# neeharperi/FutureDet

Hardware: AMD Instinct MI355X
Metric: sweeps/sec end-to-end (300k pts, 10-sweep voxel) (higher is better)
Workload: dtype f32

## Files before the change

futuredet_amd/backbones.py:

```python
import numpy as np
import torch
from torch import nn

from . import hip_ops, sparse as spconv
from .nn_utils import build_norm_layer
from .registry import BACKBONES
from .sparse import SparseConv3d, SubMConv3d


def conv3x3(in_planes, out_planes, stride=1, indice_key=None, bias=True):
    return spconv.SubMConv3d(in_planes, out_planes, kernel_size=3, stride=stride, padding=1, bias=bias,
                             indice_key=indice_key)


class SparseBasicBlock(spconv.SparseModule):
    expansion = 1

    def __init__(self, inplanes, planes, stride=1, norm_cfg=None, downsample=None, indice_key=None):
        super().__init__()
        if norm_cfg is None:
            norm_cfg = dict(type="BN1d", eps=1e-3, momentum=0.01)
        bias = norm_cfg is not None
        self.conv1 = conv3x3(inplanes, planes, stride, indice_key=indice_key, bias=bias)
        self.bn1 = build_norm_layer(norm_cfg, planes)[1]
        self.relu = nn.ReLU()
        self.conv2 = conv3x3(planes, planes, indice_key=indice_key, bias=bias)
        self.bn2 = build_norm_layer(norm_cfg, planes)[1]
        self.downsample = downsample
        self.stride = stride

    def forward(self, x):
        identity = x
        out = self.conv1(x)
        out.features = self.relu(self.bn1(out.features))
        out = self.conv2(out)
        out.features = self.bn2(out.features)
        if self.downsample is not None:
            identity = self.downsample(x)
        out.features = self.relu(out.features + identity.features)
        return out

    def forward_fused_bn(self, x, bn_act):
        out = self.conv1(x)
        out.features = bn_act(out.features, self.bn1, self.relu)
        out = self.conv2(out)
        identity = x if self.downsample is None else self.downsample(x)
        out.features = bn_act(out.features, self.bn2, self.relu, identity.features)
        return out


@BACKBONES.register_module
class SpMiddleResNetFHD(nn.Module):
    def __init__(self, num_input_features=128, norm_cfg=None, name="SpMiddleResNetFHD", **kwargs):
        super().__init__()
        self.name = name
        if norm_cfg is None:
            norm_cfg = dict(type="BN1d", eps=1e-3, momentum=0.01)
        S = spconv.SparseSequential
        self.conv_input = S(SubMConv3d(num_input_features, 16, 3, bias=False, indice_key="res0"),
                            build_norm_layer(norm_cfg, 16)[1], nn.ReLU(inplace=True))
        self.conv1 = S(SparseBasicBlock(16, 16, norm_cfg=norm_cfg, indice_key="res0"),
                       SparseBasicBlock(16, 16, norm_cfg=norm_cfg, indice_key="res0"))
        self.conv2 = S(SparseConv3d(16, 32, 3, 2, padding=1, bias=False), build_norm_layer(norm_cfg, 32)[1],
                       nn.ReLU(inplace=True), SparseBasicBlock(32, 32, norm_cfg=norm_cfg, indice_key="res1"),
                       SparseBasicBlock(32, 32, norm_cfg=norm_cfg, indice_key="res1"))
        self.conv3 = S(SparseConv3d(32, 64, 3, 2, padding=1, bias=False), build_norm_layer(norm_cfg, 64)[1],
                       nn.ReLU(inplace=True), SparseBasicBlock(64, 64, norm_cfg=norm_cfg, indice_key="res2"),
                       SparseBasicBlock(64, 64, norm_cfg=norm_cfg, indice_key="res2"))
        self.conv4 = S(SparseConv3d(64, 128, 3, 2, padding=[0, 1, 1], bias=False), build_norm_layer(norm_cfg, 128)[1],
                       nn.ReLU(inplace=True), SparseBasicBlock(128, 128, norm_cfg=norm_cfg, indice_key="res3"),
                       SparseBasicBlock(128, 128, norm_cfg=norm_cfg, indice_key="res3"))
        self.extra_conv = S(SparseConv3d(128, 128, (3, 1, 1), (2, 1, 1), bias=False), build_norm_layer(norm_cfg, 128)[1],
                            nn.ReLU())
        self.compute_dtype = torch.float32
        self.dense_channels_last = True
        self.dense_dtype = None
        self.profile_hook = None
        self.fused_bn = False
        self.train_dtype = torch.float32

    def _bn_act(self, features, bn, relu, residual=None):
        if self.fused_bn and spconv.batch_norm_fusable(features, bn):
            return spconv.batch_norm_act(features, bn, residual=residual, relu=True)
        if features.dtype == torch.bfloat16:
            out = bn(features.float())
            if residual is not None:
                out = out + residual.float()
            return spconv.relu_to_bf16(out)
        out = bn(features)
        if residual is not None:
            out = out + residual
        return relu(out)

    def _run_stage(self, seq, x):
        mods = list(seq._modules.values())
        i = 0
        while i < len(mods):
            m = mods[i]
            if isinstance(m, SparseBasicBlock):
                x = m.forward_fused_bn(x, self._bn_act)
            elif isinstance(m, spconv.SparseModule):
                x = m(x)
            elif x.features.shape[0] != 0:
                if isinstance(m, nn.BatchNorm1d) and i + 1 < len(mods) and isinstance(mods[i + 1], nn.ReLU):
                    x.features = self._bn_act(x.features, m, mods[i + 1])
                    i += 1
                else:
                    x.features = m(x.features)
            i += 1
        return x

    def forward_generic(self, voxel_features, coors, batch_size, input_shape):
        sparse_shape = np.array(input_shape[::-1]) + [1, 0, 0]
        ret = spconv.SparseConvTensor(voxel_features, coors.int(), sparse_shape, batch_size)
        stages = (self.conv_input, self.conv1, self.conv2, self.conv3, self.conv4, self.extra_conv)
        mixed = self.train_dtype == torch.bfloat16 and self.training and torch.is_grad_enabled()
        if mixed:
            ret.features = ret.features.to(torch.bfloat16)
        if mixed or (self.fused_bn and self.training and torch.is_grad_enabled()):
            run = [lambda x, seq=seq: self._run_stage(seq, x) for seq in stages]
        else:
            run = stages
        x = run[0](ret)
        x_conv1 = run[1](x)
        x_conv2 = run[2](x_conv1)
        x_conv3 = run[3](x_conv2)
        x_conv4 = run[4](x_conv3)
        ret = run[5](x_conv4).dense()
        if mixed:
            ret = ret.float()
        N, C, D, H, W = ret.shape
        ret = ret.view(N, C * D, H, W)
        return ret, {"conv1": x_conv1, "conv2": x_conv2, "conv3": x_conv3, "conv4": x_conv4}

    def _stages(self):
        return [(self.conv_input[0], self.conv_input[1], [self.conv1[0], self.conv1[1]], True),
                (self.conv2[0], self.conv2[1], [self.conv2[3], self.conv2[4]], False),
                (self.conv3[0], self.conv3[1], [self.conv3[3], self.conv3[4]], False),
                (self.conv4[0], self.conv4[1], [self.conv4[3], self.conv4[4]], False),
                (self.extra_conv[0], self.extra_conv[1], [], False)]

    def build_indexes(self, mark_fn, batch_size, input_shape, device, voxels=None, static=False, expected=None, row_caps=None):
        D, H, W = [int(v) for v in (np.array(input_shape[::-1]) + [1, 0, 0])]
        if voxels is not None:
            geoms = [self._stages()[lvl][0].geometry() for lvl in range(1, 5)]
            return hip_ops.build_pyramid(voxels[0], voxels[1], voxels[2], batch_size, (D, H, W), geoms, device, static=static,
                                         expected=expected, row_caps=row_caps)
        assert not static, "static indexes are built from the voxelizer's device output (voxels=...)"
        counts = torch.zeros((5,), dtype=torch.int32, device=device)
        idx = [hip_ops.SparseIndex(batch_size, D, H, W, device)]
        mark_fn(idx[0])
        idx[0].scan(counts[0:1])
        for lvl in range(1, 5):
            conv = self._stages()[lvl][0]
            ks, st, pd = conv.geometry()
            nxt = idx[-1].downsample(ks, st, pd)
            nxt.scan(counts[lvl:lvl + 1])
            idx.append(nxt)
        host = counts.cpu()
        for i, ix in enumerate(idx):
            ix.finalize(int(host[i]))
        return idx

    def run_fused(self, idx, feats0, dense_out=None, fork=False):
        dt = self.compute_dtype
        stages = self._stages()
        rb_cache = {}

        def rulebook(src, dst, conv):
            ks, st, pd = conv.geometry()
            key = (id(src), id(dst), tuple(ks), tuple(st), tuple(pd))
            if key not in rb_cache:
                rb_cache[key] = src.rulebook(dst, ks, st, pd)
            return rb_cache[key]

        def run(conv, bn, x, src, dst, relu, residual=None):
            wpk, bias, cin_p, cout_p = conv.packed_weight(dt, bn)
            assert x.shape[1] == cin_p, (x.shape, cin_p)
            nbr = rulebook(src, dst, conv)
            fn = lambda: hip_ops.spconv_apply(x, wpk, bias, nbr, dst.n, cout_p, residual=residual, relu=relu)
            if self.profile_hook is not None:
                s = 4 if dt == torch.float32 else 2
                K = nbr.shape[0]
                pairs = lambda: int((nbr[:, : dst.n] >= 0).sum().item())
                return self.profile_hook("spconv_%dx%d_K%d" % (cin_p, cout_p, K),
                                         dict(s=s, K=K, cin=cin_p, cout=cout_p, n_in=src.n, n_out=dst.n, pairs=pairs), fn)
            return fn()

        main, side = None, None
        if fork and feats0.is_cuda:
            main = torch.cuda.current_stream(feats0.device)
            pool = self.__dict__.setdefault("_side_streams", {})
            side = pool.get(main.cuda_stream)
            if side is None:
                side = pool[main.cuda_stream] = torch.cuda.Stream(device=feats0.device)
            side.wait_stream(main)
            with torch.cuda.stream(side):
                made = []
                for lvl, (conv, bn, blocks, is_subm_in) in enumerate(stages):
                    if lvl == 0:
                        continue
                    src_l, dst_l = (idx[lvl] if is_subm_in else idx[lvl - 1]), idx[lvl]
                    made.append(rulebook(src_l, dst_l, conv))
                    for blk in blocks:
                        nbr = rulebook(dst_l, dst_l, blk.conv1)
                        made.append(nbr)
                        cp = spconv.pad_channels(blk.conv1.out_channels)
                        if dt == torch.float32 and nbr.shape[0] == 27 and \
                                hip_ops._lib.load().fd_spconv_wants_balanced_ranges(cp, cp, 0):
                            r = hip_ops.ranges_for(nbr, cp, cp)
                            if r[0] is not None:
                                made.append(r[0])
                for t in made:
                    t.record_stream(main)
        x = feats0
        levels = {}
        for lvl, (conv, bn, blocks, is_subm_in) in enumerate(stages):
            src = idx[lvl] if is_subm_in else idx[lvl - 1]
            dst = idx[lvl]
            if lvl == 1 and side is not None:
                main.wait_stream(side)
            x = run(conv, bn, x, src, dst, relu=True)
            for blk in blocks:
                y = run(blk.conv1, blk.bn1, x, dst, dst, relu=True)
                x = run(blk.conv2, blk.bn2, y, dst, dst, relu=True, residual=x)
            levels[lvl] = (x, dst)
        bev = hip_ops.densify(x, idx[4], out_dtype=self.dense_dtype or dt, channels_last=self.dense_channels_last, out=dense_out)
        return bev, levels

    def forward_static_train(self, feats0, idx):
        if not self.fused_bn:
            raise ValueError("SpMiddleResNetFHD.forward_static_train needs fused_bn = True: torch's BatchNorm1d cannot take its row count "
                             "from the device (set backbone.fused_bn = True)")
        if not (self.training and torch.is_grad_enabled()):
            raise RuntimeError("SpMiddleResNetFHD.forward_static_train is the training path: call .train() and enable gradients")
        if self.train_dtype not in (torch.float32, torch.bfloat16):
            raise ValueError("SpMiddleResNetFHD: train_dtype must be torch.float32 or torch.bfloat16 (got %s)" % (self.train_dtype,))
        B = idx[0].B
        feats = feats0.to(self.train_dtype)
        rulebooks = {}

        def conv(m, x, src, dst):
            ks, st, pd = m.geometry()
            key = (id(src), id(dst), tuple(ks), tuple(st), tuple(pd))
            if key not in rulebooks:
                rulebooks[key] = src.rulebook(dst, ks, st, pd)
            return m._forward_autograd(x, dst, rulebooks[key])

        def bn_act(x, bn, dst, residual=None):
            if dst.n < 2 or not spconv.batch_norm_fusable(x.features, bn):
                raise hip_ops.FutureDetHipError("forward_static_train: BatchNorm over %s %s rows cannot run on the fused kernels"
                                                % (tuple(x.features.shape), x.features.dtype))
            x.features = spconv.batch_norm_act(x.features, bn, residual=residual, relu=True, n_dev=dst.n_dev if dst.static else None)
            return x

        x = spconv.SparseConvTensor(feats, None, idx[0].spatial_shape, B, _index=idx[0])
        for lvl, (head, bn, blocks, is_subm_in) in enumerate(self._stages()):
            src, dst = (idx[lvl] if is_subm_in else idx[lvl - 1]), idx[lvl]
            x = bn_act(conv(head, x, src, dst), bn, dst)
            for blk in blocks:
                y = bn_act(conv(blk.conv1, x, dst, dst), blk.bn1, dst)
                x = bn_act(conv(blk.conv2, y, dst, dst), blk.bn2, dst, residual=x.features)
        ret = x.dense()
        if ret.dtype != torch.float32:
            ret = ret.float()
        N, C, D, H, W = ret.shape
        return ret.view(N, C * D, H, W)

    def forward(self, voxel_features, coors, batch_size, input_shape):
        if self.training:
            if self.train_dtype not in (torch.float32, torch.bfloat16):
                raise ValueError("SpMiddleResNetFHD: train_dtype must be torch.float32 or torch.bfloat16 (got %s)" % (self.train_dtype,))
            if self.train_dtype == torch.float32 and self.compute_dtype != torch.float32 and torch.is_grad_enabled():
                raise NotImplementedError("SpMiddleResNetFHD: with train_dtype = torch.float32 training runs the fp32 sparse convolution only; "
                                          "compute_dtype = %s selects the inference path (set train_dtype = torch.bfloat16 for mixed-precision "
                                          "training, or compute_dtype = torch.float32)" % self.compute_dtype)
            return self.forward_generic(voxel_features, coors, batch_size, input_shape)
        coors = coors.int().contiguous()
        dev = voxel_features.device
        idx = self.build_indexes(lambda i0: i0.mark(coors), batch_size, input_shape, dev)
        row_of = idx[0].lookup(coors)
        feats0 = hip_ops.rows_permute(voxel_features.float().contiguous(), row_of,
                                      spconv.pad_channels(voxel_features.shape[1]), self.compute_dtype, n_rows=idx[0].n)
        bev, levels = self.run_fused(idx, feats0)
        multi = {}
        for name, lvl, c in (("conv1", 0, 16), ("conv2", 1, 32), ("conv3", 2, 64), ("conv4", 3, 128)):
            f, ix = levels[lvl]
            multi[name] = spconv.SparseConvTensor(f[:, :c], None, ix.spatial_shape, batch_size, _index=ix)
        return bev, multi


@BACKBONES.register_module
class PointPillarsScatter(nn.Module):

    def __init__(self, num_input_features=64, norm_cfg=None, name="PointPillarsScatter", **kwargs):
        super().__init__()
        self.name = "PointPillarsScatter"
        self.nchannels = num_input_features
        self.dense_channels_last = True

    def forward(self, voxel_features, coords, batch_size, input_shape, n_dev=None):
        self.nx = int(input_shape[0])
        self.ny = int(input_shape[1])
        coords = coords.int().contiguous()
        if n_dev is None and torch.is_grad_enabled() and voxel_features.requires_grad:
            return _ScatterFn.apply(voxel_features, coords, batch_size, self.ny, self.nx, self.dense_channels_last)
        return hip_ops.pillar_scatter(voxel_features, coords, n_dev, batch_size, self.ny, self.nx,
                                      channels_last=self.dense_channels_last)


    def forward_static(self, voxel_features, coords, counts, batch_size, input_shape):
        self.nx = int(input_shape[0])
        self.ny = int(input_shape[1])
        return _ScatterSegFn.apply(voxel_features, coords.int().contiguous(), counts, batch_size, self.ny, self.nx, self.dense_channels_last)


class _ScatterSegFn(torch.autograd.Function):

    @staticmethod
    def forward(ctx, feats, coords, counts, batch_size, ny, nx, channels_last):
        B = counts.shape[0]
        cap = feats.shape[0] // B
        ctx.coords, ctx.counts, ctx.cap = coords, counts, cap
        canvas = None
        for b in range(B):
            sl = slice(b * cap, (b + 1) * cap)
            canvas = hip_ops.pillar_scatter(feats[sl], coords[sl], counts[b:b + 1], batch_size, ny, nx, channels_last=channels_last,
                                            out=canvas, zero_first=(b == 0))
        return canvas

    @staticmethod
    def backward(ctx, dcanvas):
        coords, counts, cap = ctx.coords, ctx.counts, ctx.cap
        dcanvas = dcanvas.float()
        d = torch.cat([hip_ops.pillar_scatter_backward(dcanvas, coords[b * cap:(b + 1) * cap], n_dev=counts[b:b + 1])
                       for b in range(counts.shape[0])])
        ctx.coords = ctx.counts = None
        return d, None, None, None, None, None, None


class _ScatterFn(torch.autograd.Function):

    @staticmethod
    def forward(ctx, feats, coords, batch_size, ny, nx, channels_last):
        ctx.coords = coords
        return hip_ops.pillar_scatter(feats, coords, None, batch_size, ny, nx, channels_last=channels_last)

    @staticmethod
    def backward(ctx, dcanvas):
        d = hip_ops.pillar_scatter_backward(dcanvas.float(), ctx.coords)
        ctx.coords = None
        return d, None, None, None, None, None
```

futuredet_amd/csrc/fd_common.h:

```cpp
#pragma once
#include <hip/hip_runtime.h>
#include <stdint.h>
#include <stdio.h>

#include <atomic>

#include "../../include/futuredet_hip.h"

namespace fd {

void set_error(const char *fmt, ...);

struct SpconvCall {
    const void *in;
    int64_t n_in;
    const void *wpacked;
    const float *bias;
    const void *residual;
    int relu;
    const int *nbr;
    int64_t nbr_stride;
    const int *ranges;
    int n_ranges;
    int K, n_out;
    const int *n_out_dev;
    int64_t n_expected;
    int cin, cout, dtype;
    void *out;
    hipStream_t stream;
};

constexpr int kSpconvMaxTaps = 27;

struct WeightSection {
    size_t offset, bytes;
};
struct SpconvWeightLayout {
    WeightSection base, c32, pair, win;
    size_t total;
};
inline SpconvWeightLayout spconv_weight_layout(int K, int cin, int cout, int dtype) {
    const size_t elem = dtype == 0 ? 4 : 2, main_bytes = (size_t)K * cin * cout * elem;
    SpconvWeightLayout l{};
    size_t end = 0;
    auto section = [&](bool present, size_t bytes) {
        const WeightSection s{end, present ? bytes : 0};
        end += s.bytes;
        return s;
    };
    l.base = section(true, main_bytes);
    l.c32 = section(dtype == 0 && cin == 32 && cout == 32, main_bytes);
    l.pair = section(dtype == 1 && cin == 16, (size_t)((K + 1) / 2) * 32 * cout * elem);
    l.win = section(dtype == 1 && ((cin == 64 && cout == 64) || (cin == 128 && cout == 128)), main_bytes);
    l.total = end;
    return l;
}
inline SpconvWeightLayout spconv_weight_layout(const SpconvCall &c) { return spconv_weight_layout(c.K, c.cin, c.cout, c.dtype); }

int spconv_f32_res16_dispatch(const SpconvCall &c);
int spconv_f32_c32_dispatch(const SpconvCall &c);
int spconv_f32_compact_dispatch(const SpconvCall &c);
int spconv_bf16_win_dispatch(const SpconvCall &c);
int spconv_bf16_ws_dispatch(const SpconvCall &c);

int wino_pc_launch(const float *x, const void *wp, const float *bias, float *y, int B, int H, int W, int cin, int cout, int relu, int cout_total,
                   int co_off, int wide_items, hipStream_t stream);

__device__ __forceinline__ int device_count(int capacity, const int *count_dev) {
    if (!count_dev) return capacity;
    const int n = *count_dev;
    return n < capacity ? (n > 0 ? n : 0) : capacity;
}

inline int check_launch(const char *what) {
    hipError_t e = hipGetLastError();
    if (e != hipSuccess) {
        set_error("%s: %s", what, hipGetErrorString(e));
        return FD_ELAUNCH;
    }
    return FD_OK;
}

#define FD_REQUIRE(cond, ...)           \
    do {                                \
        if (!(cond)) {                  \
            fd::set_error(__VA_ARGS__); \
            return FD_EINVAL;           \
        }                               \
    } while (0)

inline hipStream_t as_stream(fd_stream_t s) { return reinterpret_cast<hipStream_t>(s); }

int fill_words(void *p, uint32_t value, size_t n_words, hipStream_t stream);
int fill_words3(void *p0, uint32_t v0, size_t n0, void *p1, uint32_t v1, size_t n1, void *p2, uint32_t v2, size_t n2, hipStream_t stream);

constexpr int kMaxDevices = 64;
int current_device();
int device_cu_count();
bool ensure_dynamic_lds(const void *kernel, size_t bytes, std::atomic<uint64_t> &done);
#define FD_TUNE_KNOBS(X)                                                                                                       \
    X(kTuneSpconvRG, "spconv_rg") X(kTuneSpconvV1, "spconv_v1") X(kTuneConvNT, "conv_nt") X(kTuneV2RangesPerCU, "v2_ranges_per_cu") \
    X(kTuneSpconvC32, "spconv_c32") X(kTuneBf16GP, "bf16_gp") X(kTuneBf16RG, "bf16_rg") X(kTuneBf16Depth, "bf16_depth")        \
    X(kTuneBf16NW, "bf16_nw") X(kTuneBf16Win, "bf16_win") X(kTuneF32ResRG, "f32_res_rg") X(kTuneConvStrip, "conv_strip")       \
    X(kTuneF32ResNW, "f32_res_nw")
#define FD_TUNE_ENUM(key, name) key,
enum TuneKey { FD_TUNE_KNOBS(FD_TUNE_ENUM) kTuneCount };
#undef FD_TUNE_ENUM
int tuning(TuneKey key);

inline size_t align_up(size_t v, size_t a) { return (v + a - 1) / a * a; }

struct IndexGeom {
    int B, D, H, W, Ht, Wt;
    __host__ __device__ int64_t num_cols() const { return (int64_t)B * Ht * Wt * 64; }
};
__host__ __device__ inline IndexGeom make_geom(int B, int D, int H, int W) {
    IndexGeom g;
    g.B = B; g.D = D; g.H = H; g.W = W;
    g.Ht = (H + 7) >> 3; g.Wt = (W + 7) >> 3;
    return g;
}
__host__ __device__ inline int64_t col_of(const IndexGeom &g, int b, int y, int x) {
    return ((((int64_t)b * g.Ht + (y >> 3)) * g.Wt + (x >> 3)) << 6) + ((y & 7) << 3) + (x & 7);
}
__device__ inline void col_to_byx(const IndexGeom &g, int64_t col, int &b, int &y, int &x) {
    int in = (int)(col & 63);
    int64_t t = col >> 6;
    int tx = (int)(t % g.Wt);
    t /= g.Wt;
    int ty = (int)(t % g.Ht);
    b = (int)(t / g.Ht);
    y = ty * 8 + (in >> 3);
    x = tx * 8 + (in & 7);
}

__device__ inline unsigned xcd_swizzle(unsigned bid, unsigned nblocks) {
    const unsigned nx = 8;
    unsigned per = nblocks / nx, rem = nblocks % nx;
    unsigned xcd = bid % nx, loc = bid / nx;
    unsigned start = xcd * per + (xcd < rem ? xcd : rem);
    return start + loc;
}

}
```

futuredet_amd/csrc/fd_spconv.hip:

```cpp
#include "fd_spconv_pack.h"

namespace {

typedef float f32x4 __attribute__((ext_vector_type(4)));
typedef short s16x4 __attribute__((ext_vector_type(4)));
typedef __bf16 bf16x8 __attribute__((ext_vector_type(8)));

__device__ inline unsigned short f2bf(float v) {
    unsigned u = __float_as_uint(v);
    u += 0x7fffu + ((u >> 16) & 1u);
    return (unsigned short)(u >> 16);
}
__device__ inline float bf2f(unsigned short h) { return __uint_as_float(((unsigned)h) << 16); }


template <int CIN, int COUT, int RG>
__global__ void __launch_bounds__(256) spconv_f32(const float *__restrict__ in, const float4 *__restrict__ wp,
                                                  const float *__restrict__ bias, const float *__restrict__ residual, int relu,
                                                  const int *__restrict__ nbr, int64_t nbr_stride, int K, int n_out,
                                                  const int *__restrict__ n_out_dev, float *__restrict__ out) {
    constexpr int ROWS_B = 64 * RG;
    constexpr int NB = COUT / 16, NC = CIN / 16;
    __shared__ int s_nbr[fd::kSpconvMaxTaps * ROWS_B];
    const int tile = blockIdx.x;
    const int row0 = tile * ROWS_B;
    n_out = fd::device_count(n_out, n_out_dev);
    if (row0 >= n_out) return;
    for (int t = threadIdx.x; t < K * ROWS_B; t += 256) {
        int k = t / ROWS_B, r = t - k * ROWS_B;
        int64_t o = (int64_t)row0 + r;
        s_nbr[t] = (o < n_out) ? nbr[(int64_t)k * nbr_stride + o] : -1;
    }
    __syncthreads();
    const int lane = threadIdx.x & 63, wave = __builtin_amdgcn_readfirstlane(threadIdx.x >> 6);
    const int lrow = lane & 15, lq = lane >> 4;
    const int wrow = wave * 16 * RG;
    if (row0 + wrow >= n_out) return;

    f32x4 acc[RG][NB];
#pragma unroll
    for (int g = 0; g < RG; ++g)
#pragma unroll
        for (int nb = 0; nb < NB; ++nb) acc[g][nb] = (f32x4){0.f, 0.f, 0.f, 0.f};

    for (int k = 0; k < K; ++k) {
        int idx[RG];
        bool any[RG];
        bool any_all = false;
#pragma unroll
        for (int g = 0; g < RG; ++g) {
            idx[g] = s_nbr[k * ROWS_B + wrow + g * 16 + lrow];
            any[g] = __ballot(idx[g] >= 0) != 0ull;
            any_all = any_all || any[g];
        }
        if (!any_all) continue;
        const float4 *wk = wp + (int64_t)k * NC * NB * 64 + lane;
#pragma unroll
        for (int c = 0; c < NC; ++c) {
            float4 a[RG];
#pragma unroll
            for (int g = 0; g < RG; ++g) {
                a[g] = make_float4(0.f, 0.f, 0.f, 0.f);
                if (idx[g] >= 0) a[g] = *reinterpret_cast<const float4 *>(in + (int64_t)idx[g] * CIN + c * 16 + lq * 4);
            }
#pragma unroll
            for (int nb = 0; nb < NB; ++nb) {
                const float4 b = wk[(c * NB + nb) * 64];
#pragma unroll
                for (int g = 0; g < RG; ++g) {
                    if (any[g]) {
                        acc[g][nb] = __builtin_amdgcn_mfma_f32_16x16x4f32(a[g].x, b.x, acc[g][nb], 0, 0, 0);
                        acc[g][nb] = __builtin_amdgcn_mfma_f32_16x16x4f32(a[g].y, b.y, acc[g][nb], 0, 0, 0);
                        acc[g][nb] = __builtin_amdgcn_mfma_f32_16x16x4f32(a[g].z, b.z, acc[g][nb], 0, 0, 0);
                        acc[g][nb] = __builtin_amdgcn_mfma_f32_16x16x4f32(a[g].w, b.w, acc[g][nb], 0, 0, 0);
                    }
                }
            }
        }
    }
#pragma unroll
    for (int g = 0; g < RG; ++g) {
#pragma unroll
        for (int nb = 0; nb < NB; ++nb) {
            const int col = nb * 16 + lrow;
            const float bv = bias ? bias[col] : 0.0f;
#pragma unroll
            for (int r = 0; r < 4; ++r) {
                const int row = row0 + wrow + g * 16 + lq * 4 + r;
                if (row < n_out) {
                    float v = acc[g][nb][r] + bv;
                    if (residual) v += residual[(int64_t)row * COUT + col];
                    if (relu) v = fmaxf(v, 0.0f);
                    out[(int64_t)row * COUT + col] = v;
                }
            }
        }
    }
}

template <int CIN, int COUT, int RG>
__global__ void __launch_bounds__(256) spconv_bf16(const unsigned short *__restrict__ in, const void *__restrict__ wp_,
                                                   const float *__restrict__ bias, const unsigned short *__restrict__ residual,
                                                   int relu, const int *__restrict__ nbr, int64_t nbr_stride, int K, int n_out,
                                                   const int *__restrict__ n_out_dev, unsigned short *__restrict__ out) {
    constexpr int ROWS_B = 64 * RG;
    constexpr int NB = COUT / 16;
    constexpr bool WIDE = CIN >= 32;
    constexpr int NC = WIDE ? CIN / 32 : 1;
    __shared__ int s_nbr[fd::kSpconvMaxTaps * ROWS_B];
    const int tile = blockIdx.x;
    const int row0 = tile * ROWS_B;
    n_out = fd::device_count(n_out, n_out_dev);
    if (row0 >= n_out) return;
    for (int t = threadIdx.x; t < K * ROWS_B; t += 256) {
        int k = t / ROWS_B, r = t - k * ROWS_B;
        int64_t o = (int64_t)row0 + r;
        s_nbr[t] = (o < n_out) ? nbr[(int64_t)k * nbr_stride + o] : -1;
    }
    __syncthreads();
    const int lane = threadIdx.x & 63, wave = __builtin_amdgcn_readfirstlane(threadIdx.x >> 6);
    const int lrow = lane & 15, lq = lane >> 4;
    const int wrow = wave * 16 * RG;
    if (row0 + wrow >= n_out) return;

    f32x4 acc[RG][NB];
#pragma unroll
    for (int g = 0; g < RG; ++g)
#pragma unroll
        for (int nb = 0; nb < NB; ++nb) acc[g][nb] = (f32x4){0.f, 0.f, 0.f, 0.f};

    for (int k = 0; k < K; ++k) {
        int idx[RG];
        bool any[RG];
        bool any_all = false;
#pragma unroll
        for (int g = 0; g < RG; ++g) {
            idx[g] = s_nbr[k * ROWS_B + wrow + g * 16 + lrow];
            any[g] = __ballot(idx[g] >= 0) != 0ull;
            any_all = any_all || any[g];
        }
        if (!any_all) continue;
        if constexpr (WIDE) {
            const bf16x8 *wk = reinterpret_cast<const bf16x8 *>(wp_) + (int64_t)k * NC * NB * 64 + lane;
#pragma unroll
            for (int c = 0; c < NC; ++c) {
                bf16x8 a[RG];
#pragma unroll
                for (int g = 0; g < RG; ++g) {
                    uint4 raw = make_uint4(0u, 0u, 0u, 0u);
                    if (idx[g] >= 0) raw = *reinterpret_cast<const uint4 *>(in + (int64_t)idx[g] * CIN + c * 32 + lq * 8);
                    a[g] = __builtin_bit_cast(bf16x8, raw);
                }
#pragma unroll
                for (int nb = 0; nb < NB; ++nb) {
                    const bf16x8 b = wk[(c * NB + nb) * 64];
#pragma unroll
                    for (int g = 0; g < RG; ++g)
                        if (any[g]) acc[g][nb] = __builtin_amdgcn_mfma_f32_16x16x32_bf16(a[g], b, acc[g][nb], 0, 0, 0);
                }
            }
        } else {
            const s16x4 *wk = reinterpret_cast<const s16x4 *>(wp_) + (int64_t)k * NB * 64 + lane;
            s16x4 a[RG];
#pragma unroll
            for (int g = 0; g < RG; ++g) {
                uint2 raw = make_uint2(0u, 0u);
                if (idx[g] >= 0) raw = *reinterpret_cast<const uint2 *>(in + (int64_t)idx[g] * CIN + lq * 4);
                a[g] = __builtin_bit_cast(s16x4, raw);
            }
#pragma unroll
            for (int nb = 0; nb < NB; ++nb) {
                const s16x4 b = wk[nb * 64];
#pragma unroll
                for (int g = 0; g < RG; ++g)
                    if (any[g]) acc[g][nb] = __builtin_amdgcn_mfma_f32_16x16x16bf16_1k(a[g], b, acc[g][nb], 0, 0, 0);
            }
        }
    }
#pragma unroll
    for (int g = 0; g < RG; ++g) {
#pragma unroll
        for (int nb = 0; nb < NB; ++nb) {
            const int col = nb * 16 + lrow;
            const float bv = bias ? bias[col] : 0.0f;
#pragma unroll
            for (int r = 0; r < 4; ++r) {
                const int row = row0 + wrow + g * 16 + lq * 4 + r;
                if (row < n_out) {
                    float v = acc[g][nb][r] + bv;
                    if (residual) v += bf2f(residual[(int64_t)row * COUT + col]);
                    if (relu) v = fmaxf(v, 0.0f);
                    out[(int64_t)row * COUT + col] = f2bf(v);
                }
            }
        }
    }
}

template <int CIN, int COUT, int RG>
void launch(const fd::SpconvCall &a) {
    const int rows_b = 64 * RG;
    dim3 grid((unsigned)((a.n_out + rows_b - 1) / rows_b));
    const void *wp = (const char *)a.wpacked + fd::spconv_weight_layout(a).base.offset;
    if (a.dtype == 0)
        hipLaunchKernelGGL((spconv_f32<CIN, COUT, RG>), grid, dim3(256), 0, a.stream, (const float *)a.in, (const float4 *)wp, a.bias,
                           (const float *)a.residual, a.relu, a.nbr, a.nbr_stride, a.K, a.n_out, a.n_out_dev, (float *)a.out);
    else
        hipLaunchKernelGGL((spconv_bf16<CIN, COUT, RG>), grid, dim3(256), 0, a.stream, (const unsigned short *)a.in, wp, a.bias,
                           (const unsigned short *)a.residual, a.relu, a.nbr, a.nbr_stride, a.K, a.n_out, a.n_out_dev, (unsigned short *)a.out);
}

template <int CIN, int COUT>
void launch_rg(const fd::SpconvCall &a, int rg) {
    if (rg >= 4) launch<CIN, COUT, 4>(a);
    else if (rg == 2) launch<CIN, COUT, 2>(a);
    else launch<CIN, COUT, 1>(a);
}

int pick_rg(int64_t n_out, int cin, int cout) {
    const int forced = fd::tuning(fd::kTuneSpconvRG);
    if (forced > 0) return forced;
    const int64_t waves2 = (n_out + 31) / 32;
    int rg = (cin * cout >= 128 * 128) ? 1 : 2;
    if (rg == 2 && waves2 < 256 * 4 * 2) rg = 1;
    return rg;
}

}

extern "C" size_t fd_spconv_packed_weight_bytes(int K, int cin, int cout, int dtype) {
    if (K <= 0 || cin <= 0 || cout <= 0) return 0;
    return fd::spconv_weight_layout(K, cin, cout, dtype).total;
}

extern "C" int fd_spconv_pack_weight(const float *w, int K, int cin, int cout, int dtype, void *dst) {
    if (const int rc = fd::spconv_pack_check("fd_spconv_pack_weight", w, dst, K, cin, cout, dtype, 0)) return rc;
    fd::spconv_pack_weight_host(w, K, cin, cout, dtype, dst);
    return FD_OK;
}

extern "C" int fd_spconv_apply(const void *in_feats, int64_t n_in, const void *wpacked, const float *bias, const void *residual, int relu,
                               const int32_t *nbr, int64_t nbr_stride, const int32_t *ranges, int n_ranges, int K, int64_t n_out,
                               const int32_t *n_out_dev, int64_t n_expected, int cin, int cout, int dtype, void *out_feats, fd_stream_t stream) {
    FD_REQUIRE(K >= 1 && K <= fd::kSpconvMaxTaps, "fd_spconv_apply: K must be in [1,27]");
    FD_REQUIRE(dtype == 0 || dtype == 1, "fd_spconv_apply: dtype must be 0 (f32) or 1 (bf16)");
    FD_REQUIRE(n_out >= 0 && n_out <= nbr_stride && n_out < (1ll << 31), "fd_spconv_apply: n_out out of range");
    FD_REQUIRE(n_ranges >= 0 && (ranges == nullptr || n_ranges >= 1), "fd_spconv_apply: ranges needs n_ranges >= 1");
    if (n_expected <= 0 || n_expected > n_out) n_expected = n_out;
    if (n_out == 0) return FD_OK;
    FD_REQUIRE(in_feats && wpacked && nbr && out_feats, "fd_spconv_apply: null argument");
    const fd::SpconvCall c{in_feats, n_in, wpacked, bias, residual, relu, nbr, nbr_stride, ranges, n_ranges, K, (int)n_out, n_out_dev, n_expected,
                           cin, cout, dtype, out_feats, fd::as_stream(stream)};
    if (dtype == 0 && !fd::tuning(fd::kTuneSpconvV1) && cin == 16 && fd::tuning(fd::kTuneF32ResRG) >= 0) {
        if (fd::spconv_f32_res16_dispatch(c)) return fd::check_launch("fd_spconv_apply(f32 resident)");
    }
    if (dtype == 0 && !fd::tuning(fd::kTuneSpconvV1) && fd::tuning(fd::kTuneSpconvC32) >= 0) {
        if (fd::spconv_f32_c32_dispatch(c)) return fd::check_launch("fd_spconv_apply(c32)");
    }
    if (dtype == 0 && !fd::tuning(fd::kTuneSpconvV1)) {
        if (fd::spconv_f32_compact_dispatch(c)) return fd::check_launch("fd_spconv_apply(compact)");
    }
    if (dtype == 1 && fd::tuning(fd::kTuneBf16GP) >= 0) {
        const bool subm_like = K == 27 && n_in == n_out;
        if (fd::tuning(fd::kTuneBf16Win) >= 0 && subm_like && fd::spconv_bf16_win_dispatch(c)) return fd::check_launch("fd_spconv_apply(bf16 window)");
        if (fd::spconv_bf16_ws_dispatch(c)) return fd::check_launch("fd_spconv_apply(bf16 ws)");
    }
    const int rg = pick_rg(n_expected, cin, cout);
    const int key = cin * 1000 + cout;
    switch (key) {
        case 16016: launch_rg<16, 16>(c, rg); break;
        case 16032: launch_rg<16, 32>(c, rg); break;
        case 32032: launch_rg<32, 32>(c, rg); break;
        case 32064: launch_rg<32, 64>(c, rg); break;
        case 64064: launch_rg<64, 64>(c, rg); break;
        case 64128: launch_rg<64, 128>(c, rg); break;
        case 128128: launch_rg<128, 128>(c, rg); break;
        default:
            fd::set_error("fd_spconv_apply: unsupported channels %d -> %d", cin, cout);
            return FD_EINVAL;
    }
    return fd::check_launch("fd_spconv_apply");
}
```

futuredet_amd/csrc/fd_spconv_c32.hip:

```cpp
#include "fd_spconv_chunk.h"

namespace {

namespace sk = fd::skeleton;
typedef float f32x16 __attribute__((ext_vector_type(16)));
typedef unsigned u32x4 __attribute__((ext_vector_type(4)));
constexpr int TM = 128, COUT = 32, TS = 4, WR = 1;
constexpr sk::Layout L = sk::layout(TM, COUT, TS, 32);
static_assert(((sk::kMaxTaps + TS - 1) / TS) * (TM / WR / 32) <= L.item_slot, "item list slot");

template <int CIN, int DEPTH>
__global__ void __launch_bounds__(256) spconv_f32_c32(const float *__restrict__ in, const float4 *__restrict__ wp, const float *__restrict__ bias,
                                                      const float *__restrict__ residual, int relu, const int *__restrict__ nbr, int64_t nbr_stride,
                                                      int K, int n_out, const int *__restrict__ n_out_dev, float *__restrict__ out, unsigned in_bytes,
                                                      const int *__restrict__ ranges, int rows_per_range) {
    constexpr int NCH = CIN / 8;
    constexpr int kPad = sk::pad_entry(TM);
    extern __shared__ __attribute__((aligned(16))) unsigned char smem[];
    int *s_list = reinterpret_cast<int *>(smem + L.list);
    unsigned short *s_items = reinterpret_cast<unsigned short *>(smem + L.items);
    unsigned char *s_cnt = smem + L.cnt;
    int *s_pad = reinterpret_cast<int *>(smem + L.pad);
    float *s_acc = reinterpret_cast<float *>(smem + L.acc);

    const int tid = threadIdx.x, lane = tid & 63, wave = __builtin_amdgcn_readfirstlane(tid >> 6);
    int r_begin, r_end, n_chunks, chunk_rows;
    sk::resolve_range(n_out, n_out_dev, ranges, rows_per_range, r_begin, r_end);
    if (r_begin >= r_end) return;
    sk::cut_chunks<TM>(r_begin, r_end, n_chunks, chunk_rows);
    int pre[sk::kSliceRegs<TM>];
    sk::fetch_slice<TM>(pre, nbr, nbr_stride, K, r_begin);

    const int ln = lane & 31, lh = lane >> 5;
    const int ts = wave, wr = 0;
    unsigned char *acc_bytes = reinterpret_cast<unsigned char *>(s_acc + ts * L.acc_copy);
    const __amdgpu_buffer_rsrc_t rsrc = __builtin_amdgcn_make_buffer_rsrc(const_cast<float *>(in), 0, (int)in_bytes, 0x00020000);
    unsigned short *items = s_items + wave * L.item_slot;

    for (int chunk = 0; chunk < n_chunks; ++chunk) {
        int row0, n_rows;
        if (!sk::chunk_span(r_begin, r_end, chunk_rows, chunk, row0, n_rows)) break;
        sk::stage_chunk<TM, COUT, TS, 32>(pre, s_list, s_pad, s_acc, bias, residual, K, row0, n_rows);
        __syncthreads();
        sk::compact_taps<TM, WR>(s_list, s_cnt, K);
        __syncthreads();
        if (chunk + 1 < n_chunks) sk::fetch_slice<TM>(pre, nbr, nbr_stride, K, row0 + chunk_rows);
        const int n_items = sk::build_items<TS, 32>(s_cnt, items, K, ts, wr);

        int k_r[DEPTH], row_r[DEPTH];
        u32x4 a_r[DEPTH][NCH];
        auto stage_a0 = [&](int it) -> int { return sk::stage_a0(items, n_items, it); };
        auto stage_a1 = [&](int it, int code_v, int &kk, int &e) { sk::stage_a1<TM, WR, 32>(s_list, s_pad, n_items, wr, ln, it, code_v, kk, e); };
        auto gather_offset = [&](int e) -> unsigned { return sk::entry_row_bytes<CIN>(e) + (unsigned)(lh * 16); };
        auto gather_step = [&](unsigned voff, int c) { return __builtin_amdgcn_raw_buffer_load_b128(rsrc, voff + c * 32, 0, 0); };
        float4 b[NCH];
        auto load_b = [&](int k) {
            const float4 *wk = wp + (int64_t)k * NCH * 64 + lane;
#pragma unroll
            for (int c = 0; c < NCH; ++c) b[c] = wk[c * 64];
        };
        int k_s, e_s, code_s;
#pragma unroll
        for (int d = 0; d < DEPTH - 1; ++d) {
            stage_a1(d, stage_a0(d), k_s, e_s);
            const unsigned vo = gather_offset(e_s);
#pragma unroll
            for (int c = 0; c < NCH; ++c) a_r[d][c] = gather_step(vo, c);
            k_r[d] = k_s;
            row_r[d] = e_s;
        }
        k_r[DEPTH - 1] = -1;
        row_r[DEPTH - 1] = kPad;
        stage_a1(DEPTH - 1, stage_a0(DEPTH - 1), k_s, e_s);
        code_s = stage_a0(DEPTH);
        if (n_items > 0) load_b(k_r[0]);

        for (int i0 = 0; i0 < n_items; i0 += DEPTH) {
#pragma unroll
            for (int d = 0; d < DEPTH; ++d) {
                const unsigned arow = sk::entry_local_row(row_r[d]);
                unsigned aoff[4];
#pragma unroll
                for (int q = 0; q < 4; ++q) aoff[q] = sk::acc_slot_bytes<COUT>(arow, (unsigned)(2 * q + lh));
                f32x16 acc;
#pragma unroll
                for (int q = 0; q < 4; ++q) {
                    const float4 v = *reinterpret_cast<const float4 *>(acc_bytes + aoff[q]);
                    acc[4 * q + 0] = v.x; acc[4 * q + 1] = v.y; acc[4 * q + 2] = v.z; acc[4 * q + 3] = v.w;
                }
                const int dn = (d + DEPTH - 1) % DEPTH;
                {
                    const int it = i0 + d + DEPTH - 1;
                    const unsigned vo = gather_offset(e_s);
                    k_r[dn] = k_s;
                    row_r[dn] = e_s;
#pragma unroll
                    for (int c = 0; c < NCH; ++c) a_r[dn][c] = gather_step(vo, c);
                    stage_a1(it + 1, code_s, k_s, e_s);
                    code_s = stage_a0(it + 2);
                }
                const int knext = k_r[(d + 1) % DEPTH];
                const bool reload = knext >= 0 && knext != k_r[d];
                __builtin_amdgcn_sched_barrier(0);
#pragma unroll
                for (int c = 0; c < NCH; ++c) {
                    const float4 av = __builtin_bit_cast(float4, a_r[d][c]);
                    acc = __builtin_amdgcn_mfma_f32_32x32x2f32(b[c].x, av.x, acc, 0, 0, 0);
                    acc = __builtin_amdgcn_mfma_f32_32x32x2f32(b[c].y, av.y, acc, 0, 0, 0);
                    acc = __builtin_amdgcn_mfma_f32_32x32x2f32(b[c].z, av.z, acc, 0, 0, 0);
                    acc = __builtin_amdgcn_mfma_f32_32x32x2f32(b[c].w, av.w, acc, 0, 0, 0);
                    if (reload) b[c] = (wp + (int64_t)knext * NCH * 64 + lane)[c * 64];
                }
#pragma unroll
                for (int q = 0; q < 4; ++q)
                    *reinterpret_cast<float4 *>(acc_bytes + aoff[q]) = make_float4(acc[4 * q + 0], acc[4 * q + 1], acc[4 * q + 2], acc[4 * q + 3]);
                __builtin_amdgcn_sched_barrier(0);
            }
        }
        __syncthreads();
        sk::epilogue<TM, COUT, TS>(s_acc, bias, residual, relu, out, row0, n_rows);
        __syncthreads();
    }
}

template <int CIN, int DEPTH>
int launch_c32(const fd::SpconvCall &c) {
    const unsigned in_bytes = (unsigned)(c.n_in * CIN * 4);
    int n_ranges = c.n_ranges, rows_per = 0;
    if (!c.ranges) sk::equal_rows_split(c.n_out, TM, c.n_out_dev != nullptr, n_ranges, rows_per);
    static std::atomic<uint64_t> lds_set{0};
    if (!fd::ensure_dynamic_lds(reinterpret_cast<const void *>(spconv_f32_c32<CIN, DEPTH>), (size_t)L.bytes, lds_set)) return 0;
    const void *wp = (const char *)c.wpacked + fd::spconv_weight_layout(c).c32.offset;
    hipLaunchKernelGGL((spconv_f32_c32<CIN, DEPTH>), dim3((unsigned)n_ranges), dim3(256), (size_t)L.bytes, c.stream, (const float *)c.in, (const float4 *)wp,
                       c.bias, (const float *)c.residual, c.relu, c.nbr, c.nbr_stride, c.K, c.n_out, c.n_out_dev, (float *)c.out, in_bytes, c.ranges, rows_per);
    return 1;
}

}

namespace fd {
int spconv_f32_c32_dispatch(const SpconvCall &c) {
    if (c.cout != 32 || c.cin != 32) return 0;
    if (!sk::entries_fit(c.n_in, c.cin)) return 0;
    return launch_c32<32, 3>(c);
}
}
```

futuredet_amd/csrc/fd_spconv_chunk.h:

```cpp
#pragma once
#include "fd_common.h"

namespace fd {
namespace skeleton {

constexpr int kMaxTaps = 27;

constexpr int pad_entry(int tm) { return (int)(0xffffff00u | (unsigned)tm); }
__device__ __forceinline__ int pack_entry(int in_row, int local_row) { return (in_row << 8) | local_row; }
__device__ __forceinline__ unsigned entry_local_row(int e) { return (unsigned)e & 255u; }
template <int CIN>
__device__ __forceinline__ unsigned entry_row_bytes(int e) {
    static_assert(CIN == 16 || CIN == 32 || CIN == 64 || CIN == 128, "shift per CIN");
    const unsigned hi = (unsigned)e & 0xffffff00u;
    return CIN >= 64 ? hi << (CIN == 128 ? 1 : 0) : hi >> (CIN == 32 ? 1 : 2);
}
inline bool entries_fit(int64_t n_in_bound, int cin) { return n_in_bound < (1ll << 23) && n_in_bound * cin * 4 < (1ll << 31); }

struct Layout {
    int list;
    int items;
    int item_slot;
    int cnt;
    int pad;
    int acc;
    int acc_copy;
    int bytes;
};
constexpr int acc_copy_floats(int tm, int cout) { return (tm + 1) * cout; }
constexpr Layout layout(int tm, int cout, int ts, int item) {
    Layout l{};
    l.list = 0;
    l.items = l.list + (int)sizeof(int) * kMaxTaps * tm;
    l.item_slot = item == 16 ? kMaxTaps * (tm / 16) : 32;
    l.cnt = l.items + (int)sizeof(unsigned short) * 4 * l.item_slot;
    l.pad = l.cnt + 112;
    l.acc = l.pad + (int)sizeof(int) * item;
    l.acc_copy = acc_copy_floats(tm, cout);
    l.bytes = l.acc + (int)sizeof(float) * ts * l.acc_copy;
    return l;
}

template <int COUT>
__device__ __forceinline__ unsigned acc_swizzle(unsigned row) {
    static_assert(COUT == 16 || COUT == 32 || COUT == 64 || COUT == 128, "whole bank rows");
    constexpr int kSwzShift = COUT >= 64 ? 0 : COUT == 32 ? 1 : 2;
    constexpr unsigned kSwzMask = COUT >= 64 ? 15u : COUT == 32 ? 7u : 3u;
    return (row >> kSwzShift) & kSwzMask;
}
template <int COUT>
__device__ __forceinline__ int acc_slot(int row, int col) {
    return row * (COUT / 4) + (col ^ (int)acc_swizzle<COUT>((unsigned)row));
}
template <int COUT>
__device__ __forceinline__ unsigned acc_slot_bytes(unsigned row, unsigned col) {
    return row * (COUT * 4) + ((col ^ acc_swizzle<COUT>(row)) << 4);
}

__device__ __forceinline__ void resolve_range(int n_out, const int *n_out_dev, const int *ranges, int rows_per_range,
                                              int &r_begin, int &r_end) {
    if (n_out_dev) n_out = fd::device_count(n_out, n_out_dev);
    if (ranges) {
        r_begin = ranges[blockIdx.x];
        r_end = ranges[blockIdx.x + 1];
    } else {
        if (n_out_dev) rows_per_range = (((n_out + (int)gridDim.x - 1) / (int)gridDim.x) + 15) & ~15;
        const int64_t b = (int64_t)blockIdx.x * rows_per_range;
        r_begin = (int)(b < n_out ? b : n_out);
        r_end = (int)(b + rows_per_range < n_out ? b + rows_per_range : n_out);
    }
    if (r_end > n_out) r_end = n_out;
}
template <int TM>
__device__ __forceinline__ void cut_chunks(int r_begin, int r_end, int &n_chunks, int &chunk_rows) {
    n_chunks = (r_end - r_begin + TM - 1) / TM;
    chunk_rows = (((r_end - r_begin + n_chunks - 1) / n_chunks) + 15) & ~15;
}
__device__ __forceinline__ bool chunk_span(int r_begin, int r_end, int chunk_rows, int chunk, int &row0, int &n_rows) {
    row0 = r_begin + chunk * chunk_rows;
    n_rows = (r_end - row0) < chunk_rows ? (r_end - row0) : chunk_rows;
    return n_rows > 0;
}
inline void equal_rows_split(int n_out, int tm, bool device_count, int &n_ranges, int &rows_per) {
    if (n_ranges <= 0) n_ranges = (n_out + tm - 1) / tm;
    rows_per = (((n_out + n_ranges - 1) / n_ranges) + 15) & ~15;
    if (!device_count) n_ranges = (n_out + rows_per - 1) / rows_per;
}

template <int TM>
constexpr int kSliceRegs = (kMaxTaps * TM + 255) / 256;

template <int TM>
__device__ __forceinline__ void fetch_slice(int (&pre)[kSliceRegs<TM>], const int *nbr, int64_t nbr_stride, int K, int row0) {
    const int tid = threadIdx.x;
#pragma unroll
    for (int i = 0; i < kSliceRegs<TM>; ++i) {
        const int t = tid + i * 256;
        int k = t / TM;
        const int r = t - k * TM;
        k = k < K ? k : K - 1;
        int64_t o = (int64_t)row0 + r;
        o = o < nbr_stride ? o : nbr_stride - 1;
        pre[i] = nbr[(int64_t)k * nbr_stride + o];
    }
}

template <int COUT>
constexpr bool kInitAcc = COUT <= 64;

template <int TM, int COUT, int TS>
__device__ __forceinline__ void init_acc(float *s_acc, const float *bias, const float *residual, int row0, int n_rows) {
    const int tid = threadIdx.x;
    if constexpr (kInitAcc<COUT>) {
        constexpr int C4i = COUT / 4, NINIT = TM * C4i / 256;
        static_assert(TM * C4i % 256 == 0, "whole passes");
        float4 iv[NINIT];
#pragma unroll
        for (int i = 0; i < NINIT; ++i) {
            const int t = tid + i * 256, c4 = t % C4i;
            iv[i] = bias ? reinterpret_cast<const float4 *>(bias)[c4] : make_float4(0.f, 0.f, 0.f, 0.f);
        }
        if (residual) {
            float4 rv[NINIT];
#pragma unroll
            for (int i = 0; i < NINIT; ++i) {
                const int t = tid + i * 256, r = t / C4i, c4 = t - r * C4i;
                const int rr = r < n_rows ? r : n_rows - 1;
                rv[i] = reinterpret_cast<const float4 *>(residual + (int64_t)(row0 + rr) * COUT)[c4];
            }
#pragma unroll
            for (int i = 0; i < NINIT; ++i) { iv[i].x += rv[i].x; iv[i].y += rv[i].y; iv[i].z += rv[i].z; iv[i].w += rv[i].w; }
        }
#pragma unroll
        for (int i = 0; i < NINIT; ++i) {
            const int t = tid + i * 256, r = t / C4i, c4 = t - r * C4i;
            reinterpret_cast<float4 *>(s_acc)[acc_slot<COUT>(r, c4)] = r < n_rows ? iv[i] : make_float4(0.f, 0.f, 0.f, 0.f);
        }
        for (int t = TM * C4i + tid; t < TS * acc_copy_floats(TM, COUT) / 4; t += 256) reinterpret_cast<float4 *>(s_acc)[t] = make_float4(0.f, 0.f, 0.f, 0.f);
    } else {
        for (int t = tid; t < TS * acc_copy_floats(TM, COUT) / 4; t += 256) reinterpret_cast<float4 *>(s_acc)[t] = make_float4(0.f, 0.f, 0.f, 0.f);
    }
}

template <int TM, int COUT, int TS, int ITEM>
__device__ __forceinline__ void stage_chunk(const int (&pre)[kSliceRegs<TM>], int *s_list, int *s_pad, float *s_acc, const float *bias,
                                            const float *residual, int K, int row0, int n_rows) {
    const int tid = threadIdx.x;
    static_assert(256 % TM == 0, "a thread stages the same local row in every pass");
    const bool in_chunk = tid % TM < n_rows;
#pragma unroll
    for (int i = 0; i < kSliceRegs<TM>; ++i) {
        const int t = tid + i * 256;
        if (t < K * TM) s_list[t] = in_chunk ? pre[i] : -1;
    }
    init_acc<TM, COUT, TS>(s_acc, bias, residual, row0, n_rows);
    if (tid < ITEM) s_pad[tid] = pad_entry(TM);
}

template <int TM, int WR>
__device__ __forceinline__ void compact_taps(int *s_list, unsigned char *s_cnt, int K) {
    const int lane = threadIdx.x & 63, wave = __builtin_amdgcn_readfirstlane(threadIdx.x >> 6);
    constexpr int RW = TM / WR, NH = (RW + 63) / 64;
    for (int k = wave; k < K; k += 4) {
#pragma unroll
        for (int wr = 0; wr < WR; ++wr) {
            const int base = k * TM + wr * RW;
            int count = 0;
            int v[NH];
#pragma unroll
            for (int h = 0; h < NH; ++h) {
                const int r = h * 64 + lane;
                v[h] = (r < RW) ? s_list[base + r] : -1;
            }
#pragma unroll
            for (int h = 0; h < NH; ++h) {
                const int r = h * 64 + lane;
                if (r < RW) s_list[base + r] = pad_entry(TM);
            }
#pragma unroll
            for (int h = 0; h < NH; ++h) {
                const int r = h * 64 + lane;
                const unsigned long long m = __ballot(v[h] >= 0);
                const int pos = count + __popcll(m & ((1ull << lane) - 1ull));
                if (v[h] >= 0) s_list[base + pos] = pack_entry(v[h], wr * RW + r);
                count += __popcll(m);
            }
            if (lane == 0) s_cnt[k * 4 + wr] = (unsigned char)count;
        }
    }
}

template <int TS, int ITEM>
__device__ __forceinline__ int build_items(const unsigned char *s_cnt, unsigned short *items, int K, int ts, int wr) {
    const int lane = threadIdx.x & 63;
    const int ng = (lane < K && (lane % TS) == ts) ? ((int)s_cnt[lane * 4 + wr] + ITEM - 1) / ITEM : 0;
    int inc = ng;
#pragma unroll
    for (int off = 1; off < 64; off <<= 1) {
        const int u = __shfl_up(inc, off);
        if (lane >= off) inc += u;
    }
    const int n_items = __builtin_amdgcn_readfirstlane(__shfl(inc, 63));
    for (int g = 0; g < ng; ++g) items[inc - ng + g] = (unsigned short)((lane << 3) | g);
    __builtin_amdgcn_fence(__ATOMIC_RELEASE, "workgroup");
    __builtin_amdgcn_wave_barrier();
    __builtin_amdgcn_fence(__ATOMIC_ACQUIRE, "workgroup");
    return n_items;
}

__device__ __forceinline__ int stage_a0(const unsigned short *items, int n_items, int it) { return (int)items[it < n_items ? it : 0]; }
template <int TM, int WR, int ITEM>
__device__ __forceinline__ void stage_a1(const int *s_list, const int *s_pad, int n_items, int wr, int lp, int it, int code_v, int &kk, int &e) {
    const bool v = it < n_items;
    const int code = __builtin_amdgcn_readfirstlane(code_v);
    const int ks = v ? (code >> 3) : 0;
    kk = v ? ks : -1;
    const int *lst = v ? s_list + ks * TM + wr * (TM / WR) + (code & 7) * ITEM : s_pad;
    e = lst[lp];
}

template <int TM, int COUT, int TS>
__device__ __forceinline__ void epilogue(float *s_acc, const float *bias, const float *residual, int relu,
                                         float *out, int row0, int n_rows) {
    const int tid = threadIdx.x;
    constexpr int C4 = COUT / 4;
    for (int t = tid; t < n_rows * C4; t += 256) {
        const int r = t / C4, c4 = t - r * C4;
        const int row = row0 + r;
        const int slot = acc_slot<COUT>(r, c4);
        float4 v = reinterpret_cast<const float4 *>(s_acc)[slot];
#pragma unroll
        for (int q = 1; q < TS; ++q) {
            const float4 v2 = reinterpret_cast<const float4 *>(s_acc + q * acc_copy_floats(TM, COUT))[slot];
            v.x += v2.x; v.y += v2.y; v.z += v2.z; v.w += v2.w;
        }
        if constexpr (!kInitAcc<COUT>) {
            if (bias) {
                const float4 bv = reinterpret_cast<const float4 *>(bias)[c4];
                v.x += bv.x; v.y += bv.y; v.z += bv.z; v.w += bv.w;
            }
            if (residual) {
                const float4 rv = reinterpret_cast<const float4 *>(residual + (int64_t)row * COUT)[c4];
                v.x += rv.x; v.y += rv.y; v.z += rv.z; v.w += rv.w;
            }
        }
        if (relu) { v.x = fmaxf(v.x, 0.f); v.y = fmaxf(v.y, 0.f); v.z = fmaxf(v.z, 0.f); v.w = fmaxf(v.w, 0.f); }
        reinterpret_cast<float4 *>(out + (int64_t)row * COUT)[c4] = v;
    }
}

}
}
```

futuredet_amd/csrc/fd_spconv_v2.hip:

```cpp
#include "fd_spconv_chunk.h"

namespace {

namespace sk = fd::skeleton;
typedef float f32x4 __attribute__((ext_vector_type(4)));
typedef unsigned u32x4 __attribute__((ext_vector_type(4)));
typedef int i32x4 __attribute__((ext_vector_type(4)));

#ifdef FD_V2_TRACE
__device__ unsigned long long *g_trace;
#define FD_T(i)                                                                                  \
    do {                                                                                         \
        if (threadIdx.x == 0 && g_trace) g_trace[(size_t)blockIdx.x * 16 + (i)] = __builtin_readcyclecounter(); \
    } while (0)
#define FD_TV(i, v)                                                                    \
    do {                                                                               \
        if (threadIdx.x == 0 && g_trace) g_trace[(size_t)blockIdx.x * 16 + (i)] = (v); \
    } while (0)
#else
#define FD_T(i)
#define FD_TV(i, v)
#endif


constexpr int tap_splits(int cout) { return (cout == 32 || cout == 64) ? 2 : 1; }

template <int CIN, int COUT, int TM, int DEPTH>
__global__ void __launch_bounds__(256) spconv_f32_compact(const float *__restrict__ in, const float4 *__restrict__ wp,
                                                          const float *__restrict__ bias, const float *__restrict__ residual, int relu,
                                                          const int *__restrict__ nbr, int64_t nbr_stride, int K, int n_out,
                                                          const int *__restrict__ n_out_dev, float *__restrict__ out, unsigned in_bytes,
                                                          const int *__restrict__ ranges, int rows_per_range) {
    constexpr int NB = COUT / 16, NC = CIN / 16;
    constexpr int WC = NB == 8 ? 4 : (NB >= 2 ? 2 : 1);
    constexpr int NBW = NB / WC;
    constexpr int TS = tap_splits(COUT);
    constexpr int WR = 4 / (WC * TS);
    constexpr int NACC = NBW;
    static_assert((TM == 128 || TM == 64) && TM / WR >= 16, "local row uses 8 bits (0..TM, TM = scratch row)");
    constexpr int kPad = sk::pad_entry(TM);
    constexpr sk::Layout L = sk::layout(TM, COUT, TS, 16);
    extern __shared__ __attribute__((aligned(16))) unsigned char smem[];
    int *s_list = reinterpret_cast<int *>(smem + L.list);
    unsigned short *s_items = reinterpret_cast<unsigned short *>(smem + L.items);
    unsigned char *s_cnt = smem + L.cnt;
    int *s_pad = reinterpret_cast<int *>(smem + L.pad);
    float *s_acc = reinterpret_cast<float *>(smem + L.acc);

    const int tid = threadIdx.x, lane = tid & 63, wave = __builtin_amdgcn_readfirstlane(tid >> 6);
    int r_begin, r_end, n_chunks, chunk_rows;
    sk::resolve_range(n_out, n_out_dev, ranges, rows_per_range, r_begin, r_end);
    if (r_begin >= r_end) return;
    FD_T(0);
    sk::cut_chunks<TM>(r_begin, r_end, n_chunks, chunk_rows);
    int pre[sk::kSliceRegs<TM>];
    sk::fetch_slice<TM>(pre, nbr, nbr_stride, K, r_begin);

    const int lrow = lane & 15, lq = lane >> 4;
    const int wc = wave % WC, wr = TS == 1 ? wave / WC : 0, ts = TS == 1 ? 0 : wave / WC;
    const int cb = wc * NBW * 16;
    unsigned char *acc_bytes = reinterpret_cast<unsigned char *>(s_acc + ts * L.acc_copy);
    const unsigned slot0 = (unsigned)(cb >> 2) + (unsigned)lq;
    const __amdgpu_buffer_rsrc_t rsrc = __builtin_amdgcn_make_buffer_rsrc(const_cast<float *>(in), 0, (int)in_bytes, 0x00020000);
    unsigned short *items = s_items + wave * L.item_slot;

    for (int chunk = 0; chunk < n_chunks; ++chunk) {
    int row0, n_rows;
    if (!sk::chunk_span(r_begin, r_end, chunk_rows, chunk, row0, n_rows)) break;
    sk::stage_chunk<TM, COUT, TS, 16>(pre, s_list, s_pad, s_acc, bias, residual, K, row0, n_rows);
    __syncthreads();
    if (chunk == 0) FD_T(1);
    sk::compact_taps<TM, WR>(s_list, s_cnt, K);
    __syncthreads();
    if (chunk == 0) FD_T(2);
    if (chunk + 1 < n_chunks) sk::fetch_slice<TM>(pre, nbr, nbr_stride, K, row0 + chunk_rows);
    const int n_items = sk::build_items<TS, 16>(s_cnt, items, K, ts, wr);

    int k_r[DEPTH];
    int row_r[DEPTH];
    u32x4 a_r[DEPTH][NC];
    auto stage_a0 = [&](int it) -> int { return sk::stage_a0(items, n_items, it); };
    auto stage_a1 = [&](int it, int code_v, int &kk, int &e) { sk::stage_a1<TM, WR, 16>(s_list, s_pad, n_items, wr, lrow, it, code_v, kk, e); };
    auto gather_offset = [&](int e) -> unsigned { return sk::entry_row_bytes<CIN>(e) + (unsigned)(lq * 16); };
    auto gather_chunk = [&](unsigned voff, int c) { return __builtin_amdgcn_raw_buffer_load_b128(rsrc, voff + c * 64, 0, 0); };
    auto load_b = [&](int k, float4(&dst)[NC][NBW]) {
        const float4 *wk = wp + ((int64_t)k * NC * NB + wc * NBW) * 64 + lane;
#pragma unroll
        for (int c = 0; c < NC; ++c)
#pragma unroll
            for (int nw = 0; nw < NBW; ++nw) dst[c][nw] = wk[(c * NB + nw) * 64];
    };
    float4 b[NC][NBW];
    static_assert(DEPTH >= 2, "the slot freed by the previous item is refilled during the current item's MFMAs");
    int k_s, e_s, code_s;
#pragma unroll
    for (int d = 0; d < DEPTH - 1; ++d) {
        stage_a1(d, stage_a0(d), k_s, e_s);
        const unsigned vo = gather_offset(e_s);
#pragma unroll
        for (int c = 0; c < NC; ++c) a_r[d][c] = gather_chunk(vo, c);
        k_r[d] = k_s;
        row_r[d] = e_s;
    }
    k_r[DEPTH - 1] = -1;
    row_r[DEPTH - 1] = kPad;
    stage_a1(DEPTH - 1, stage_a0(DEPTH - 1), k_s, e_s);
    code_s = stage_a0(DEPTH);
    if (n_items > 0) load_b(k_r[0], b);
    if (chunk == 0) { FD_T(3); FD_TV(8, (unsigned long long)n_items); FD_TV(9, (unsigned long long)n_chunks); FD_TV(10, (unsigned long long)n_rows);
                      FD_TV(11, (unsigned long long)__builtin_amdgcn_s_getreg(4 | (31 << 11))); FD_TV(12, (unsigned long long)__builtin_amdgcn_s_getreg(20 | (31 << 11))); }
    FD_TV(13, (unsigned long long)(g_trace ? g_trace[(size_t)blockIdx.x * 16 + 13] : 0) + (unsigned long long)n_items);

    auto mfma_chunk = [&](const u32x4 &a4, const float4(&bc)[NBW], f32x4(&acc)[NACC]) {
        const float4 av = __builtin_bit_cast(float4, a4);
#pragma unroll
        for (int nw = 0; nw < NBW; ++nw) acc[nw] = __builtin_amdgcn_mfma_f32_16x16x4f32(bc[nw].x, av.x, acc[nw], 0, 0, 0);
#pragma unroll
        for (int nw = 0; nw < NBW; ++nw) acc[nw] = __builtin_amdgcn_mfma_f32_16x16x4f32(bc[nw].y, av.y, acc[nw], 0, 0, 0);
#pragma unroll
        for (int nw = 0; nw < NBW; ++nw) acc[nw] = __builtin_amdgcn_mfma_f32_16x16x4f32(bc[nw].z, av.z, acc[nw], 0, 0, 0);
#pragma unroll
        for (int nw = 0; nw < NBW; ++nw) acc[nw] = __builtin_amdgcn_mfma_f32_16x16x4f32(bc[nw].w, av.w, acc[nw], 0, 0, 0);
    };

    for (int i0 = 0; i0 < n_items; i0 += DEPTH) {
#pragma unroll
        for (int d = 0; d < DEPTH; ++d) {
            const unsigned arow = sk::entry_local_row(row_r[d]);
            unsigned aoff[NBW];
#pragma unroll
            for (int nw = 0; nw < NBW; ++nw) aoff[nw] = sk::acc_slot_bytes<COUT>(arow, slot0 + 4u * nw);
            f32x4 acc[NACC];
#pragma unroll
            for (int nw = 0; nw < NBW; ++nw) acc[nw] = *reinterpret_cast<const f32x4 *>(acc_bytes + aoff[nw]);
            const int dn = (d + DEPTH - 1) % DEPTH;
            unsigned vo;
            {
                const int it = i0 + d + DEPTH - 1;
                vo = gather_offset(e_s);
                k_r[dn] = k_s;
                row_r[dn] = e_s;
                stage_a1(it + 1, code_s, k_s, e_s);
                code_s = stage_a0(it + 2);
            }
            const int knext = k_r[(d + 1) % DEPTH];
            const bool reload = knext >= 0 && knext != k_r[d];
            constexpr bool kSpread = NC * 4 * NBW >= 16;
            if constexpr (!kSpread) {
#pragma unroll
                for (int c = 0; c < NC; ++c) a_r[dn][c] = gather_chunk(vo, c);
            }
            __builtin_amdgcn_sched_barrier(0);
            if (reload) {
                const float4 *wk = wp + ((int64_t)knext * NC * NB + wc * NBW) * 64 + lane;
#pragma unroll
                for (int c = 0; c < NC; ++c) {
                    mfma_chunk(a_r[d][c], b[c], acc);
                    if constexpr (kSpread) a_r[dn][c] = gather_chunk(vo, c);
#pragma unroll
                    for (int nw = 0; nw < NBW; ++nw) b[c][nw] = wk[(c * NB + nw) * 64];
                    __builtin_amdgcn_sched_group_barrier(0x008, 4 * NBW, 0);
                    __builtin_amdgcn_sched_group_barrier(0x020, (kSpread ? 1 : 0) + NBW, 0);
                }
            } else {
#pragma unroll
                for (int c = 0; c < NC; ++c) {
                    mfma_chunk(a_r[d][c], b[c], acc);
                    if constexpr (kSpread) {
                        a_r[dn][c] = gather_chunk(vo, c);
                        __builtin_amdgcn_sched_group_barrier(0x008, 4 * NBW, 0);
                        __builtin_amdgcn_sched_group_barrier(0x020, 1, 0);
                    }
                }
            }
#pragma unroll
            for (int nw = 0; nw < NBW; ++nw) *reinterpret_cast<f32x4 *>(acc_bytes + aoff[nw]) = acc[nw];
            __builtin_amdgcn_sched_barrier(0);
        }
    }
    if (chunk == 0) FD_T(4);
    __syncthreads();
    if (chunk == 0) FD_T(5);
    sk::epilogue<TM, COUT, TS>(s_acc, bias, residual, relu, out, row0, n_rows);
    __syncthreads();
    if (chunk == 0) FD_T(6);
    }
    FD_T(7);
}

inline size_t lds_request(int cin, int cout, int tm) {
    const size_t lds = (size_t)sk::layout(tm, cout, tap_splits(cout), 16).bytes;
    return (cin == 64 && cout == 64 && tm == 128 && lds < 56 * 1024) ? (size_t)56 * 1024 : lds;
}

template <int CIN, int COUT, int TM, int DEPTH>
int launch_compact(const fd::SpconvCall &c) {
    const size_t lds_req = lds_request(CIN, COUT, TM);
    static std::atomic<uint64_t> lds_set{0};
    auto kern = spconv_f32_compact<CIN, COUT, TM, DEPTH>;
    if (!fd::ensure_dynamic_lds(reinterpret_cast<const void *>(kern), lds_req, lds_set)) return 0;
    const unsigned in_bytes = (unsigned)(c.n_in * CIN * 4);
    int n_ranges = c.n_ranges, rows_per = 0;
    if (!c.ranges) sk::equal_rows_split(c.n_out, TM, c.n_out_dev != nullptr, n_ranges, rows_per);
    const void *wp = (const char *)c.wpacked + fd::spconv_weight_layout(c).base.offset;
    hipLaunchKernelGGL(kern, dim3((unsigned)n_ranges), dim3(256), lds_req, c.stream, (const float *)c.in, (const float4 *)wp, c.bias,
                       (const float *)c.residual, c.relu, c.nbr, c.nbr_stride, c.K, c.n_out, c.n_out_dev, (float *)c.out, in_bytes, c.ranges, rows_per);
    return 1;
}

constexpr int kWorkRows = 8;
constexpr int kRowCost = 24;
__global__ void __launch_bounds__(256) block_work_kernel(const int *__restrict__ nbr, int64_t nbr_stride, int K, int n_out,
                                                         const int *__restrict__ n_out_dev, unsigned row_cost, unsigned *__restrict__ work) {
    n_out = fd::device_count(n_out, n_out_dev);
    const int n_blocks = (n_out + kWorkRows - 1) / kWorkRows;
    const int lane = threadIdx.x & 63;
    const int64_t wave = (int64_t)blockIdx.x * 4 + (threadIdx.x >> 6);
    const int64_t o = wave * 64 + lane;
    if (wave * 8 >= n_blocks) return;
    unsigned w = row_cost;
    for (int k = 0; k < K; ++k) {
        const bool v = o < n_out && nbr[(int64_t)k * nbr_stride + o] >= 0;
        const unsigned long long m = __ballot(v);
        const unsigned byte = (unsigned)(m >> (8 * (lane & 7))) & 0xffu;
        w += (unsigned)__popc(byte) * 2u + (byte ? 1u : 0u);
    }
    if (lane < 8 && wave * 8 + lane < n_blocks) work[wave * 8 + lane] = w;
}

__global__ void __launch_bounds__(1024) range_split_kernel(const unsigned *__restrict__ work, int n_out, const int *__restrict__ n_out_dev,
                                                           int n_ranges, int *__restrict__ ranges) {
    n_out = fd::device_count(n_out, n_out_dev);
    const int n_blocks = (n_out + kWorkRows - 1) / kWorkRows;
    __shared__ unsigned long long s_seg[16];
    __shared__ unsigned long long s_total;
    const int tid = threadIdx.x, lane = tid & 63, wave = tid >> 6;
    if (n_blocks == 0) {
        for (int j = tid; j <= n_ranges; j += 1024) ranges[j] = 0;
        return;
    }
    const int seg = (((n_blocks + 15) / 16) + 63) & ~63;
    const int b_lo = wave * seg, b_hi = min(n_blocks, b_lo + seg);
    constexpr int kU = 16;
    unsigned long long sum = 0;
    for (int c0 = b_lo; c0 < b_hi; c0 += 64 * kU) {
        unsigned wv[kU];
#pragma unroll
        for (int u = 0; u < kU; ++u) {
            const int bb = c0 + 64 * u + lane;
            wv[u] = work[bb < b_hi ? bb : b_hi - 1];
        }
#pragma unroll
        for (int u = 0; u < kU; ++u) sum += (c0 + 64 * u + lane < b_hi) ? wv[u] : 0u;
    }
#pragma unroll
    for (int o = 32; o > 0; o >>= 1) sum += __shfl_xor(sum, o);
    if (lane == 0) s_seg[wave] = sum;
    __syncthreads();
    if (tid == 0) {
        unsigned long long run = 0;
        for (int w = 0; w < 16; ++w) { const unsigned long long v = s_seg[w]; s_seg[w] = run; run += v; }
        s_total = run;
    }
    __syncthreads();
    const unsigned long long total = s_total > 0 ? s_total : 1ull;
    const double scale = (double)n_ranges / (2.0 * (double)total);
    auto range_of = [&](unsigned long long ex, unsigned w) -> int {
        const int r = (int)((double)(2ull * ex + w) * scale);
        return r < n_ranges ? r : n_ranges - 1;
    };
    unsigned long long run = s_seg[wave];
    int prev = -1;
    if (b_lo > 0 && b_lo < n_blocks) {
        const unsigned wp = work[b_lo - 1];
        prev = range_of(run - wp, wp);
    }
    constexpr int kB = 8;
    __shared__ unsigned s_buf[16][64 * (kB + 1)];
    unsigned *buf = s_buf[wave];
    for (int c0 = b_lo; c0 < b_hi; c0 += 64 * kB) {
#pragma unroll
        for (int u = 0; u < kB; ++u) {
            const int e = 64 * u + lane, bb = c0 + e;
            buf[(e / kB) * (kB + 1) + e % kB] = bb < b_hi ? work[bb] : 0u;
        }
        __builtin_amdgcn_fence(__ATOMIC_RELEASE, "workgroup");
        __builtin_amdgcn_wave_barrier();
        __builtin_amdgcn_fence(__ATOMIC_ACQUIRE, "workgroup");
        unsigned w[kB];
        unsigned tot = 0;
#pragma unroll
        for (int i = 0; i < kB; ++i) {
            w[i] = buf[lane * (kB + 1) + i];
            tot += w[i];
        }
        unsigned inc = tot;
#pragma unroll
        for (int o = 1; o < 64; o <<= 1) {
            const unsigned u = __shfl_up(inc, o);
            if (lane >= o) inc += u;
        }
        unsigned long long ex = run + (inc - tot);
        const int first = c0 + lane * kB;
        int last_rg = prev;
        {
            unsigned long long e2 = ex;
#pragma unroll
            for (int i = 0; i < kB; ++i) {
                if (first + i < b_hi) last_rg = range_of(e2, w[i]);
                e2 += w[i];
            }
        }
        int before = __shfl_up(last_rg, 1);
        if (lane == 0) before = prev;
        if (first >= b_hi) last_rg = before;
#pragma unroll
        for (int i = 0; i < kB; ++i) {
            const int bb = first + i;
            if (bb < b_hi) {
                const int rg = range_of(ex, w[i]);
                for (int j = before + 1; j <= rg; ++j) ranges[j] = bb * kWorkRows;
                before = rg;
                if (bb == n_blocks - 1)
                    for (int j = rg + 1; j <= n_ranges; ++j) ranges[j] = n_out;
            }
            ex += w[i];
        }
        const int n_valid = min(64 * kB, b_hi - c0);
        prev = __shfl(last_rg, (n_valid - 1) / kB);
        run += __shfl(inc, 63);
        __builtin_amdgcn_wave_barrier();
    }
}

}

#ifdef FD_V2_TRACE
extern "C" int fd_debug_set_trace(void *p) { return hipMemcpyToSymbol(HIP_SYMBOL(g_trace), &p, sizeof(p)) == hipSuccess ? 0 : -1; }
#endif

extern "C" int fd_spconv_num_ranges(int64_t n_out, int cin, int cout, int dtype) {
    if (n_out <= 0 || dtype != 0) return 0;
    const int n_cu = fd::device_cu_count();
    const int64_t tiles = (n_out + 127) / 128;
    const int mult = fd::tuning(fd::kTuneV2RangesPerCU);
    int64_t per_cu;
    if (mult) per_cu = mult;
    else if (cout >= 64) per_cu = (int64_t)((160 * 1024) / lds_request(cin, cout, 128));
    else per_cu = (tiles + n_cu - 1) / n_cu;
    if (per_cu < 1) per_cu = 1;
    return (int)(per_cu * n_cu);
}

extern "C" int fd_spconv_wants_balanced_ranges(int cin, int cout, int dtype) { return dtype == 0 && cout >= 64; }

extern "C" size_t fd_spconv_ranges_workspace_bytes(int64_t n_out) {
    return fd::align_up(sizeof(unsigned) * (size_t)((n_out + kWorkRows - 1) / kWorkRows + 8), 256);
}

extern "C" int fd_spconv_ranges(const int32_t *nbr, int64_t nbr_stride, int K, int64_t n_out, const int32_t *n_out_dev, int n_ranges,
                                int32_t *ranges, void *workspace, size_t workspace_bytes, fd_stream_t stream_) {
    FD_REQUIRE(nbr && ranges && workspace, "fd_spconv_ranges: null argument");
    FD_REQUIRE(n_ranges >= 1 && n_out >= 0 && n_out <= nbr_stride && n_out < (1ll << 31), "fd_spconv_ranges: bad sizes");
    FD_REQUIRE(workspace_bytes >= fd_spconv_ranges_workspace_bytes(n_out), "fd_spconv_ranges: workspace too small");
    hipStream_t stream = fd::as_stream(stream_);
    const int n_blocks = (int)((n_out + kWorkRows - 1) / kWorkRows);
    unsigned *work = (unsigned *)workspace;
    if (n_blocks > 0)
        hipLaunchKernelGGL(block_work_kernel, dim3((unsigned)((n_blocks + 31) / 32)), dim3(256), 0, stream, nbr, nbr_stride, K, (int)n_out, n_out_dev,
                           (unsigned)kRowCost, work);
    hipLaunchKernelGGL(range_split_kernel, dim3(1), dim3(1024), 0, stream, work, (int)n_out, n_out_dev, n_ranges, ranges);
    return fd::check_launch("fd_spconv_ranges");
}

namespace fd {
int spconv_f32_compact_dispatch(const SpconvCall &c) {
    if (!sk::entries_fit(c.n_in, c.cin)) return 0;
    switch (c.cin * 1000 + c.cout) {
        case 16016: return launch_compact<16, 16, 128, 4>(c);
        case 16032: return launch_compact<16, 32, 128, 4>(c);
        case 32032: return launch_compact<32, 32, 128, 4>(c);
        case 32064: return launch_compact<32, 64, 128, 4>(c);
        case 64064: return launch_compact<64, 64, 128, 3>(c);
        case 64128: return launch_compact<64, 128, 128, 3>(c);
        case 128128: return launch_compact<128, 128, 128, 2>(c);
        case 32016: return launch_compact<32, 16, 128, 4>(c);
        case 64032: return launch_compact<64, 32, 128, 4>(c);
        case 128064: return launch_compact<128, 64, 128, 2>(c);
    }
    return 0;
}
}
```

futuredet_amd/hip_ops.py:

```python
import ctypes
import threading

import numpy as np
import torch

from . import lib as _lib
from .lib import DecodeCfg, FutureDetHipError, MapView, check


_raw_stream = getattr(torch._C, "_cuda_getCurrentRawStream", None)


def _stream():
    if _raw_stream is not None:
        return ctypes.c_void_p(_raw_stream(torch.cuda.current_device()))
    return ctypes.c_void_p(torch.cuda.current_stream().cuda_stream)


def _dev(t, name, dtype=None):
    if not isinstance(t, torch.Tensor) or not t.is_cuda:
        raise FutureDetHipError("%s must be a tensor on the HIP device (got %s); this path has no CPU implementation"
                                % (name, "cpu tensor" if isinstance(t, torch.Tensor) else type(t)))
    if dtype is not None and t.dtype != dtype:
        raise FutureDetHipError("%s must be %s, got %s" % (name, dtype, t.dtype))
    if not t.is_contiguous():
        raise FutureDetHipError("%s must be contiguous" % name)
    return t


def _p(t):
    return ctypes.c_void_p(t.data_ptr()) if t is not None else None


class _Workspace(object):

    def __init__(self):
        self._bufs = {}
        self._scope = threading.local()

    def scope(self, token):
        ws = self

        class _Scope(object):
            def __enter__(self_):
                self_.prev = getattr(ws._scope, "token", None)
                ws._scope.token = token

            def __exit__(self_, *exc):
                ws._scope.token = self_.prev

        return _Scope()

    def release(self, token):
        for key in [k for k in self._bufs if k[2] == ("scope", token)]:
            del self._bufs[key]

    def get(self, tag, nbytes, device):
        token = getattr(self._scope, "token", None)
        key = (tag, device.index, ("scope", token) if token is not None else _stream().value)
        buf = self._bufs.get(key)
        if buf is None or buf.numel() < nbytes:
            buf = torch.empty(max(int(nbytes), 256), dtype=torch.uint8, device=device)
            self._bufs[key] = buf
        return buf


workspace = _Workspace()
_DT = {torch.float32: 0, torch.bfloat16: 1}


def set_tuning(name, value):
    check(_lib.load().fd_tuning_set(name.encode(), int(value)), "fd_tuning_set")


def voxelize(points, voxel_size, coors_range, max_points, max_voxels, batch_idx=0, want_voxels=True, want_mean=False,
             mean_stride=None, coor_cols=3, out=None, n_points_dev=None):
    L = _lib.load()
    points = _dev(points, "points", torch.float32)
    n, ndim = points.shape
    dev = points.device
    rng = (ctypes.c_float * 6)(*[float(np.float32(v)) for v in coors_range])
    vs = (ctypes.c_float * 3)(*[float(np.float32(v)) for v in voxel_size])
    out = dict(out or {})
    if want_voxels and "voxels" not in out:
        out["voxels"] = torch.empty((max_voxels, max_points, ndim), dtype=torch.float32, device=dev)
    if want_mean and "mean" not in out:
        out["mean"] = torch.empty((max_voxels, mean_stride or ndim), dtype=torch.float32, device=dev)
    if "coors" not in out:
        out["coors"] = torch.empty((max_voxels, coor_cols), dtype=torch.int32, device=dev)
    if "num_points" not in out:
        out["num_points"] = torch.empty((max_voxels,), dtype=torch.int32, device=dev)
    if "num_voxels" not in out:
        out["num_voxels"] = torch.zeros((1,), dtype=torch.int32, device=dev)
    mean = out.get("mean") if want_mean else None
    voxels = out.get("voxels") if want_voxels else None
    ws_bytes = L.fd_voxelize_workspace_bytes(n, max_voxels)
    ws = workspace.get("voxelize", ws_bytes, dev)
    check(L.fd_voxelize(_p(points), n, _p(n_points_dev), ndim, rng, vs, int(max_points), int(max_voxels), int(batch_idx), _p(voxels), _p(mean),
                        int(mean.shape[1]) if mean is not None else 0, _p(out["coors"]), int(out["coors"].shape[1]),
                        _p(out["num_points"]), _p(out["num_voxels"]), _p(ws), ws.numel(), _stream()), "fd_voxelize")
    return out


class SparseIndex(object):

    def __init__(self, B, D, H, W, device, words=None, prefix=None):
        L = _lib.load()
        self.B, self.D, self.H, self.W = int(B), int(D), int(H), int(W)
        self.ncols = L.fd_index_num_cols(self.B, self.H, self.W)
        self.words = torch.zeros((self.ncols,), dtype=torch.int64, device=device) if words is None else words
        self.prefix = torch.empty((self.ncols,), dtype=torch.int32, device=device) if prefix is None else prefix
        self.n_dev = None
        self.n = None
        self.coords = None
        self.device = device
        self.static = False
        self.n_expected = 0

    @property
    def spatial_shape(self):
        return [self.D, self.H, self.W]

    def mark(self, coords, n_dev=None, n_max=None):
        L = _lib.load()
        coords = _dev(coords, "coords", torch.int32)
        n_max = coords.shape[0] if n_max is None else n_max
        check(L.fd_index_mark(_p(coords), _p(n_dev), n_max, self.B, self.D, self.H, self.W, _p(self.words), _stream()),
              "fd_index_mark")

    def scan(self, n_dev):
        L = _lib.load()
        ws = workspace.get("index_scan", L.fd_index_workspace_bytes(self.ncols), self.device)
        self.n_dev = n_dev
        check(L.fd_index_scan(_p(self.words), self.ncols, _p(self.prefix), _p(n_dev), _p(ws), ws.numel(), _stream()),
              "fd_index_scan")

    def downsample(self, ksize, stride, pad):
        L = _lib.load()
        od = [(i + 2 * p - (k - 1) - 1) // s + 1 for i, k, s, p in zip(self.spatial_shape, ksize, stride, pad)]
        out = SparseIndex(self.B, od[0], od[1], od[2], self.device)
        check(L.fd_index_downsample(_p(self.words), self.B, self.D, self.H, self.W, (ctypes.c_int * 3)(*ksize),
                                    (ctypes.c_int * 3)(*stride), (ctypes.c_int * 3)(*pad), _p(out.words), _stream()),
              "fd_index_downsample")
        return out

    def finalize(self, n):
        L = _lib.load()
        self.n = int(n)
        self.coords = torch.empty((max(self.n, 1), 4), dtype=torch.int32, device=self.device)[: self.n]
        if self.n:
            check(L.fd_index_coords(_p(self.words), _p(self.prefix), self.B, self.D, self.H, self.W, _p(self.coords),
                                    _stream()), "fd_index_coords")

    def lookup(self, coords, n_dev=None):
        L = _lib.load()
        coords = _dev(coords, "coords", torch.int32)
        row_of = torch.empty((coords.shape[0],), dtype=torch.int32, device=self.device)
        check(L.fd_index_lookup(_p(self.words), _p(self.prefix), self.B, self.D, self.H, self.W, _p(coords), _p(n_dev),
                                coords.shape[0], _p(row_of), _stream()), "fd_index_lookup")
        return row_of

    def rulebook(self, out_index, ksize, stride, pad):
        L = _lib.load()
        assert out_index.n is not None
        K = int(ksize[0] * ksize[1] * ksize[2])
        nstride = max(64, (out_index.n + 63) // 64 * 64)
        nbr = torch.empty((K, nstride), dtype=torch.int32, device=self.device)
        static = getattr(out_index, "static", False)
        if out_index.n == 0:
            nbr.fill_(-1)
            return nbr
        check(L.fd_rulebook(_p(self.words), _p(self.prefix), self.B, self.D, self.H, self.W, _p(out_index.coords), out_index.n,
                            _p(out_index.n_dev), nstride, 0 if static else 1, (ctypes.c_int * 3)(*ksize), (ctypes.c_int * 3)(*stride),
                            (ctypes.c_int * 3)(*pad), _p(nbr), _stream()), "fd_rulebook")
        nbr.n_out = out_index.n
        nbr.n_dev = out_index.n_dev if static else None
        nbr.n_expected = out_index.n_expected if static else 0
        src_static = getattr(self, "static", False)
        nbr.n_in_dev = self.n_dev if src_static else None
        nbr.n_in_expected = self.n_expected if src_static else 0
        return nbr


class _PyramidPlan(object):

    def __init__(self, B, shape0, geoms, device):
        L = _lib.load()
        self.B, self.geoms, self.device = int(B), geoms, device
        self.shapes = [tuple(int(v) for v in shape0)]
        for ks, st, pd in geoms:
            self.shapes.append(tuple((i + 2 * p - (k - 1) - 1) // s + 1 for i, k, s, p in zip(self.shapes[-1], ks, st, pd)))
        self.ncols = [L.fd_index_num_cols(self.B, sh[1], sh[2]) for sh in self.shapes]
        self.ws_bytes = L.fd_index_workspace_bytes(sum(self.ncols) + 2048 * len(self.ncols))

    def row_caps(self, cap0):
        caps = [min(int(cap0), self.B * int(np.prod(self.shapes[0])))]
        for (ks, st, pd), sh in zip(self.geoms, self.shapes[1:]):
            fan = int(np.prod([-(-k // s) for k, s in zip(ks, st)]))
            caps.append(min(caps[-1] * fan, self.B * int(np.prod(sh))))
        return caps


_pyramid_plans = {}


def build_pyramid(coors, nvox, n_max, B, shape0, geoms, device, static=False, expected=None, row_caps=None):
    L = _lib.load()
    key = (int(B), tuple(int(v) for v in shape0), tuple((tuple(k), tuple(s), tuple(p)) for k, s, p in geoms), str(device))
    plan = _pyramid_plans.get(key)
    if plan is None:
        plan = _pyramid_plans[key] = _PyramidPlan(B, shape0, geoms, device)
    shapes, ncols = plan.shapes, plan.ncols
    words_all = torch.empty((sum(ncols),), dtype=torch.int64, device=device)
    prefix_all = torch.empty((sum(ncols),), dtype=torch.int32, device=device)
    counts = torch.empty((len(shapes),), dtype=torch.int32, device=device)
    idx, off = [], 0
    levels = (_lib.IndexLevel * len(shapes))()
    wp, pp = words_all.data_ptr(), prefix_all.data_ptr()
    for l, (sh, nc) in enumerate(zip(shapes, ncols)):
        ix = SparseIndex.__new__(SparseIndex)
        ix.B, ix.D, ix.H, ix.W, ix.ncols, ix.device = plan.B, sh[0], sh[1], sh[2], nc, device
        ix.words, ix.prefix = words_all[off:off + nc], prefix_all[off:off + nc]
        ix.n_dev, ix.n, ix.coords = counts[l:l + 1], None, None
        ix.level_counts = counts
        ix.static, ix.n_expected = False, 0
        lv = levels[l]
        lv.D, lv.H, lv.W = sh
        if l:
            ks, st, pd = geoms[l - 1]
            lv.ksize[:], lv.stride[:], lv.pad[:] = list(ks), list(st), list(pd)
        lv.words, lv.prefix, lv.coords = wp + 8 * off, pp + 4 * off, None
        idx.append(ix)
        off += nc
    ws = workspace.get("index_scan", plan.ws_bytes, device)

    def size_coords(host):
        total = sum(host)
        coords_all = torch.empty((max(total, 1), 4), dtype=torch.int32, device=device)
        o = 0
        for l, ix in enumerate(idx):
            ix.n = int(host[l])
            ix.coords = coords_all[o:o + ix.n]
            levels[l].coords = (coords_all.data_ptr() + 16 * o) if ix.n else None
            levels[l].coords_rows = ix.n
            o += ix.n

    if static:
        host = plan.row_caps(int(B) * int(n_max))
        if row_caps is not None:
            host = [min(int(a), int(b)) for a, b in zip(host, row_caps)]
        for l, ix in enumerate(idx):
            ix.static = True
            ix.n_expected = int(expected[l]) if expected is not None else 0
        size_coords(host)
        fused = all(int(h) > 0 for h in host)
        check(L.fd_index_pyramid(_p(coors), _p(nvox), int(n_max), plan.B, len(shapes), levels, _p(counts), _p(ws), ws.numel(), _stream()),
              "fd_index_pyramid")
        if not fused:
            check(L.fd_index_pyramid_coords(plan.B, len(shapes), levels, _stream()), "fd_index_pyramid_coords")
        return idx
    check(L.fd_index_pyramid(_p(coors), _p(nvox), int(n_max), plan.B, len(shapes), levels, _p(counts), _p(ws), ws.numel(), _stream()),
          "fd_index_pyramid")
    size_coords(counts.tolist())
    check(L.fd_index_pyramid_coords(plan.B, len(shapes), levels, _stream()), "fd_index_pyramid_coords")
    return idx


def ranges_for(nbr, cin, cout):
    cached = getattr(nbr, "ranges", None)
    if cached is not None:
        return cached
    L = _lib.load()
    n_out = getattr(nbr, "n_out", None)
    if not n_out:
        return None, 0
    K, nstride = nbr.shape
    n = int(L.fd_spconv_num_ranges(getattr(nbr, "n_expected", 0) or n_out, cin, cout, 0))
    if n <= 0:
        return None, 0
    ranges = torch.empty((n + 1,), dtype=torch.int32, device=nbr.device)
    ws = workspace.get("spconv_ranges", L.fd_spconv_ranges_workspace_bytes(n_out), nbr.device)
    check(L.fd_spconv_ranges(_p(nbr), nstride, K, n_out, _p(getattr(nbr, "n_dev", None)), n, _p(ranges), _p(ws), ws.numel(), _stream()),
          "fd_spconv_ranges")
    nbr.ranges = (ranges, n)
    return nbr.ranges


def rows_permute(src, row_of, c_dst, dtype=torch.float32, n_rows=None, n_dev=None):
    L = _lib.load()
    src = _dev(src, "src", torch.float32)
    row_of = _dev(row_of, "row_of", torch.int32)
    n_rows = src.shape[0] if n_rows is None else n_rows
    dst = torch.zeros((max(n_rows, 1), c_dst), dtype=dtype, device=src.device)[:n_rows]
    if src.shape[0]:
        check(L.fd_rows_permute(_p(src), src.shape[1], _p(row_of), _p(n_dev), src.shape[0], _p(dst), c_dst,
                                _DT[dtype], _stream()), "fd_rows_permute")
    return dst


def rows_place(index, coords, src, c_dst, dtype=torch.float32, n_dev=None, out=None):
    L = _lib.load()
    coords = _dev(coords, "coords", torch.int32)
    src = _dev(src, "src", torch.float32)
    if out is None:
        out = torch.zeros((max(index.n, 1), c_dst), dtype=dtype, device=src.device)[: index.n]
    _dev(out, "out", dtype)
    if coords.dim() != 2 or coords.shape[1] != 4:
        raise FutureDetHipError("rows_place: coords must be [n, 4] (b, z, y, x), got %s" % (tuple(coords.shape),))
    if src.dim() != 2 or src.shape[0] < coords.shape[0]:
        raise FutureDetHipError("rows_place: src must be [n, c_src] with a row per coordinate")
    if out.dim() != 2 or out.shape[1] != c_dst or index.n is None or out.shape[0] < index.n:
        raise FutureDetHipError("rows_place: out must be [rows >= index.n, %d] (finalised index), got %s" % (c_dst, tuple(out.shape)))
    check(L.fd_rows_place(_p(index.words), _p(index.prefix), index.B, index.D, index.H, index.W, _p(coords), _p(n_dev),
                          coords.shape[0], _p(src), src.shape[1], _p(out), c_dst, _DT[dtype], _stream()), "fd_rows_place")
    return out


def pack_spconv_weight(w_kio, dtype=torch.float32):
    L = _lib.load()
    dev = w_kio.device
    w = w_kio.detach().to("cpu", torch.float32).contiguous()
    K, cin, cout = w.shape
    nbytes = L.fd_spconv_packed_weight_bytes(K, cin, cout, _DT[dtype])
    host = torch.empty((nbytes,), dtype=torch.uint8)
    check(L.fd_spconv_pack_weight(ctypes.c_void_p(w.data_ptr()), K, cin, cout, _DT[dtype], ctypes.c_void_p(host.data_ptr())),
          "fd_spconv_pack_weight")
    return host.to(dev)


PACK_PLAIN, PACK_TRANSPOSED, PACK_FLIPPED_TRANSPOSED = 0, 1, 2
_PACK_DEVICE = {torch.float32: "fd_spconv_pack_weight_device", torch.bfloat16: "fd_spconv_pack_weight_device_bf16"}
_WGRAD = {torch.float32: ("fd_spconv_wgrad", "fd_spconv_wgrad_workspace_bytes", "spconv_wgrad"),
          torch.bfloat16: ("fd_spconv_wgrad_bf16", "fd_spconv_wgrad_bf16_workspace_bytes", "spconv_wgrad_bf16")}


def pack_spconv_weight_device(w_kio, mode=PACK_PLAIN, dtype=torch.float32):
    L = _lib.load()
    if dtype not in _DT:
        raise FutureDetHipError("pack_spconv_weight_device: dtype must be float32 or bfloat16 (got %s)" % (dtype,))
    w = _dev(w_kio.detach(), "w_kio", torch.float32)
    K, cin, cout = w.shape
    ci, co = (cout, cin) if mode else (cin, cout)
    out = torch.empty((L.fd_spconv_packed_weight_bytes(K, ci, co, _DT[dtype]),), dtype=torch.uint8, device=w.device)
    name = _PACK_DEVICE[dtype]
    check(getattr(L, name)(_p(w), K, cin, cout, int(mode), _p(out), _stream()), name)
    return out


def spconv_wgrad(feats, dy, nbr, n_out):
    L = _lib.load()
    if feats.dtype != dy.dtype or feats.dtype not in _DT:
        raise FutureDetHipError("spconv_wgrad: feats and dy must both be float32 or both bfloat16 (got %s and %s)" % (feats.dtype, dy.dtype))
    feats = _dev(feats, "feats")
    dy = _dev(dy, "dy")
    K, nstride = nbr.shape
    cin, cout = feats.shape[1], dy.shape[1]
    assert dy.shape[0] >= n_out
    dw = torch.empty((K, cin, cout), dtype=torch.float32, device=feats.device)
    name, ws_bytes, tag = _WGRAD[feats.dtype]
    ws = workspace.get(tag, getattr(L, ws_bytes)(K, n_out, cin, cout), feats.device)
    check(getattr(L, name)(_p(feats), feats.shape[0], _p(dy), _p(_dev(nbr, "nbr", torch.int32)), nstride, K, n_out,
                           _p(getattr(nbr, "n_dev", None)), cin, cout, _p(dw), _p(ws), ws.numel(), _stream()), name)
    return dw


def assign_targets(boxes, counts, classes, trajectory, cfg, out):
    L = _lib.load()
    boxes = _dev(boxes, "boxes", torch.float32)
    B = boxes.shape[0]
    assert tuple(boxes.shape) == (B, cfg.T, cfg.n_max, 12), (tuple(boxes.shape), cfg.T, cfg.n_max)
    assert tuple(counts.shape) == (B, cfg.T) and tuple(classes.shape) == (B, cfg.T, cfg.n_max)
    assert (trajectory is None) == (cfg.n_sets == 1)
    if trajectory is not None:
        assert tuple(trajectory.shape) == (B, cfg.T, cfg.n_max)
        trajectory = _dev(trajectory, "trajectory", torch.int32)
    U = cfg.n_tasks + (2 if cfg.n_sets == 3 else 0)
    ws = workspace.get("targets", L.fd_targets_workspace_bytes(B, cfg.T, U, cfg.max_objs), boxes.device)
    check(L.fd_assign_targets(_p(boxes), _p(_dev(counts, "counts", torch.int32)), _p(_dev(classes, "classes", torch.int32)), _p(trajectory), B,
                              ctypes.byref(cfg), _p(_dev(out["hm"], "hm", torch.float32)), _p(_dev(out["ind"], "ind", torch.int64)),
                              _p(_dev(out["mask"], "mask", torch.uint8)), _p(_dev(out["cat"], "cat", torch.int64)),
                              _p(_dev(out["anno_box"], "anno_box", torch.float32)), _p(_dev(out["gt_boxes_and_cls"], "gt_boxes_and_cls", torch.float32)),
                              _p(_dev(out["status"], "status", torch.int32)), _p(ws), ws.numel(), _stream()), "fd_assign_targets")
    return out


def rulebook_transpose(nbr, n_out, n_in):
    L = _lib.load()
    K, nstride = nbr.shape
    istride = max(64, (n_in + 63) // 64 * 64)
    inv = torch.empty((K, istride), dtype=torch.int32, device=nbr.device)
    check(L.fd_rulebook_transpose(_p(_dev(nbr, "nbr", torch.int32)), nstride, K, n_out, _p(getattr(nbr, "n_dev", None)), n_in, _p(inv),
                                  istride, _stream()), "fd_rulebook_transpose")
    return inv


def dense_gather(grad, index, c):
    L = _lib.load()
    if not (isinstance(grad, torch.Tensor) and grad.is_cuda and grad.dtype == torch.float32):
        raise FutureDetHipError("dense_gather: grad must be a float32 tensor on the HIP device")
    n = int(index.n)
    feats = torch.empty((max(n, 1), c), dtype=torch.float32, device=grad.device)[:n]
    sb, sc, sy, sx = grad.stride()
    check(L.fd_dense_gather(_p(grad), sb, sc, sy, sx, index.D, _p(index.coords), n, _p(index.n_dev if index.static else None), c,
                            _p(feats), _stream()), "fd_dense_gather")
    return feats


def spconv_apply(feats, wpacked, bias, nbr, n_out, cout, residual=None, relu=False, out=None, balanced=None):
    L = _lib.load()
    feats = _dev(feats, "feats")
    dt = _DT[feats.dtype]
    cin = feats.shape[1]
    out_dtype, out_cols = feats.dtype, cout
    K, nstride = nbr.shape
    if out is None:
        out = torch.empty((max(n_out, 1), out_cols), dtype=out_dtype, device=feats.device)[:n_out]
    if residual is not None:
        _dev(residual, "residual", out_dtype)
    ranges, n_ranges = None, 0
    n_dev, n_expected = getattr(nbr, "n_dev", None), getattr(nbr, "n_expected", 0)
    if dt == 0 and n_out > 0:
        if balanced is None:
            balanced = K == 27 and cin == cout and bool(L.fd_spconv_wants_balanced_ranges(cin, cout, 0))
        if balanced == "tiles":
            n_ranges = 0
        elif balanced:
            ranges, n_ranges = ranges_for(nbr, cin, cout)
        else:
            n_ranges = int(L.fd_spconv_num_ranges(n_expected or n_out, cin, cout, 0))
    check(L.fd_spconv_apply(_p(feats), feats.shape[0], _p(_dev(wpacked, "wpacked")), _p(bias), _p(residual), int(bool(relu)),
                            _p(_dev(nbr, "nbr", torch.int32)), nstride, _p(ranges), n_ranges, K, n_out, _p(n_dev), int(n_expected or 0),
                            cin, cout, dt, _p(out), _stream()),
          "fd_spconv_apply")
    return out


def densify(feats, index, out_dtype=None, channels_last=False, out=None):
    L = _lib.load()
    feats = _dev(feats, "feats")
    C = feats.shape[1]
    shape = (index.B, C * index.D, index.H, index.W)
    if out is None:
        out_dtype = out_dtype or feats.dtype
        out = torch.empty(shape, dtype=out_dtype, device=feats.device,
                          memory_format=torch.channels_last if channels_last else torch.contiguous_format)
    else:
        assert tuple(out.shape) == shape and out.is_cuda
        out_dtype = out.dtype
    sb, sc, sy, sx = out.stride()
    check(L.fd_densify(_p(feats), C, _DT[feats.dtype], _p(index.words), _p(index.prefix), index.B, index.D, index.H,
                       index.W, _p(out), _DT[out_dtype], sb, sc, sy, sx, int(feats.shape[0]), _stream()), "fd_densify")
    return out


def pack_conv2d_weight(w_oihw):
    L = _lib.load()
    dev = w_oihw.device
    w = w_oihw.detach().to("cpu", torch.float32).contiguous()
    cout, cin, ks, _ = w.shape
    nbytes = L.fd_conv2d_packed_weight_bytes(cout, cin, ks)
    if nbytes == 0:
        raise FutureDetHipError("fd_conv2d: unsupported weight shape %s" % (tuple(w.shape),))
    host = torch.empty((nbytes,), dtype=torch.uint8)
    check(L.fd_conv2d_pack_weight(ctypes.c_void_p(w.data_ptr()), cout, cin, ks, ctypes.c_void_p(host.data_ptr())),
          "fd_conv2d_pack_weight")
    return host.to(dev)


def conv2d_nhwc_bf16(x, wpk, bias, cout, ks, stride=1, relu=True, out=None, co_off=0, osy=1, osx=1, ooy=0, oox=0):
    L = _lib.load()
    x = _dev(x, "x", torch.bfloat16)
    B, H, W, cin = x.shape
    pad = 1 if ks == 3 else 0
    Ho, Wo = (H + 2 * pad - ks) // stride + 1, (W + 2 * pad - ks) // stride + 1
    if out is None:
        out = torch.empty((B, Ho * osy, Wo * osx, cout), dtype=torch.bfloat16, device=x.device)
    _dev(out, "out", torch.bfloat16)
    check(L.fd_conv2d_nhwc_bf16(_p(x), B, H, W, cin, _p(wpk), _p(bias), cout, ks, stride, pad, int(bool(relu)), _p(out),
                                out.shape[3], co_off, osy, osx, ooy, oox, _stream()), "fd_conv2d_nhwc_bf16")
    return out


def pack_conv2d_weight_device(w, transposed=False):
    L = _lib.load()
    w = _dev(w.detach(), "w", torch.float32)
    if w.dim() != 4 or w.shape[2] != w.shape[3]:
        raise FutureDetHipError("pack_conv2d_weight_device: need a [Cout, Cin, k, k] weight (got %s)" % (tuple(w.shape),))
    cout, cin, ks, _ = w.shape
    if transposed and cout % 32:
        raise FutureDetHipError("pack_conv2d_weight_device: the transposed weights need Cout %% 32 == 0 (got %s)" % (tuple(w.shape),))
    nbytes = L.fd_conv2d_packed_weight_bytes(cin, cout, ks) if transposed else L.fd_conv2d_packed_weight_bytes(cout, cin, ks)
    if nbytes == 0:
        raise FutureDetHipError("fd_conv2d: unsupported weight shape %s" % (tuple(w.shape),))
    out = torch.empty((nbytes,), dtype=torch.uint8, device=w.device)
    check(L.fd_conv2d_pack_weight_dev(_p(w), cout, cin, ks, int(bool(transposed)), _p(out), _stream()), "fd_conv2d_pack_weight_dev")
    return out


def conv2d_wgrad_bf16_chunk():
    return int(_lib.load().fd_conv2d_wgrad_bf16_chunk())


def conv2d_wgrad_bf16(x_nhwc, dy_nhwc, ks):
    L = _lib.load()
    x = _dev(x_nhwc, "x_nhwc", torch.bfloat16)
    dy = _dev(dy_nhwc, "dy_nhwc", torch.bfloat16)
    if x.dim() != 4 or dy.dim() != 4 or x.shape[:3] != dy.shape[:3]:
        raise FutureDetHipError("conv2d_wgrad_bf16: x [B,H,W,Cin] and dy [B,H,W,Cout] must cover the same pixels (got %s and %s)"
                                % (tuple(x.shape), tuple(dy.shape)))
    B, H, W, cin = x.shape
    cout = dy.shape[3]
    nbytes = L.fd_conv2d_wgrad_bf16_workspace_bytes(B, H, W, cin, cout, ks)
    if nbytes == 0:
        raise FutureDetHipError("conv2d_wgrad_bf16: unsupported problem %s -> %d channels, ks %s" % (tuple(x.shape), cout, ks))
    ws = torch.empty((nbytes,), dtype=torch.uint8, device=x.device)
    dw = torch.empty((cout, cin, ks, ks), dtype=torch.float32, device=x.device)
    check(L.fd_conv2d_wgrad_bf16(_p(x), _p(dy), B, H, W, cin, cout, ks, _p(ws), ws.numel(), _p(dw), _stream()), "fd_conv2d_wgrad_bf16")
    return dw


def _map4(t, name):
    t = _dev(t, name, torch.bfloat16)
    if t.dim() != 4:
        raise FutureDetHipError("%s must be a [B, H, W, C] map (got %s)" % (name, tuple(t.shape)))
    return t


def _out_map(out, shape, like, name):
    if out is None:
        return torch.empty(shape, dtype=torch.bfloat16, device=like.device)
    _dev(out, name, torch.bfloat16)
    if tuple(out.shape) != tuple(shape):
        raise FutureDetHipError("%s must be %s (got %s)" % (name, tuple(shape), tuple(out.shape)))
    return out


def conv2d_s2_dgrad_bf16(dy_nhwc, wpk_t, H, W, cin, out=None):
    L = _lib.load()
    dy = _map4(dy_nhwc, "dy_nhwc")
    B, Ho, Wo, cout = dy.shape
    if H < 1 or W < 1 or (Ho, Wo) != ((H - 1) // 2 + 1, (W - 1) // 2 + 1):
        raise FutureDetHipError("conv2d_s2_dgrad_bf16: dy %s is not the stride-2 map of %d x %d" % (tuple(dy.shape), H, W))
    _dev(wpk_t, "wpk_t", torch.uint8)
    if wpk_t.numel() != L.fd_conv2d_packed_weight_bytes(cin, cout, 3) or wpk_t.numel() == 0:
        raise FutureDetHipError("conv2d_s2_dgrad_bf16: wpk_t is not the transposed pack of a [%d, %d, 3, 3] weight" % (cout, cin))
    out = _out_map(out, (B, H, W, cin), dy, "out")
    check(L.fd_conv2d_s2_dgrad_bf16(_p(dy), B, H, W, cin, cout, _p(wpk_t), _p(out), _stream()), "fd_conv2d_s2_dgrad_bf16")
    return out


def conv2d_wgrad_s2_bf16(x_nhwc, dy_nhwc):
    L = _lib.load()
    x, dy = _map4(x_nhwc, "x_nhwc"), _map4(dy_nhwc, "dy_nhwc")
    B, H, W, cin = x.shape
    cout = dy.shape[3]
    if tuple(dy.shape[:3]) != (B, (H - 1) // 2 + 1, (W - 1) // 2 + 1):
        raise FutureDetHipError("conv2d_wgrad_s2_bf16: dy %s is not the stride-2 map of x %s" % (tuple(dy.shape), tuple(x.shape)))
    nbytes = L.fd_conv2d_wgrad_s2_bf16_workspace_bytes(B, H, W, cin, cout)
    if nbytes == 0:
        raise FutureDetHipError("conv2d_wgrad_s2_bf16: unsupported problem %s -> %d channels" % (tuple(x.shape), cout))
    ws = torch.empty((nbytes,), dtype=torch.uint8, device=x.device)
    dw = torch.empty((cout, cin, 3, 3), dtype=torch.float32, device=x.device)
    check(L.fd_conv2d_wgrad_s2_bf16(_p(x), _p(dy), B, H, W, cin, cout, _p(ws), ws.numel(), _p(dw), _stream()), "fd_conv2d_wgrad_s2_bf16")
    return dw


PACK_UP2, PACK_DOWN2 = 0, 1


def pack_conv2d_weight_2x2_device(w, kind, fine_major=False):
    L = _lib.load()
    w = _dev(w.detach(), "w", torch.float32)
    if w.dim() != 4 or tuple(w.shape[2:]) != (2, 2) or kind not in (PACK_UP2, PACK_DOWN2):
        raise FutureDetHipError("pack_conv2d_weight_2x2_device: need a [Ccoarse, Cfine, 2, 2] weight and kind PACK_UP2 or PACK_DOWN2 (got %s, %r)"
                                % (tuple(w.shape), kind))
    cc, cf = (w.shape[1], w.shape[0]) if fine_major else (w.shape[0], w.shape[1])
    nbytes = L.fd_conv2d_packed_weight_2x2_bytes(cc, cf, kind)
    if nbytes == 0:
        raise FutureDetHipError("pack_conv2d_weight_2x2_device: unsupported weight shape %s for kind %d" % (tuple(w.shape), kind))
    out = torch.empty((nbytes,), dtype=torch.uint8, device=w.device)
    check(L.fd_conv2d_pack_weight_2x2_dev(_p(w), cc, cf, kind, int(bool(fine_major)), _p(out), _stream()), "fd_conv2d_pack_weight_2x2_dev")
    return out


def conv2d_up2_bf16(x_nhwc, wpk4, c_fine, out=None):
    x = _map4(x_nhwc, "x_nhwc")
    B, H, W, cc = x.shape
    _dev(wpk4, "wpk4", torch.uint8)
    per = _lib.load().fd_conv2d_packed_weight_bytes(c_fine, cc, 1)
    if per == 0 or wpk4.numel() != 4 * per:
        raise FutureDetHipError("conv2d_up2_bf16: wpk4 is not the PACK_UP2 pack of a [%d, %d, 2, 2] weight" % (cc, c_fine))
    out = _out_map(out, (B, 2 * H, 2 * W, c_fine), x, "out")
    for tap in range(4):
        conv2d_nhwc_bf16(x, wpk4[tap * per:(tap + 1) * per], None, c_fine, 1, stride=1, relu=False, out=out, osy=2, osx=2, ooy=tap >> 1, oox=tap & 1)
    return out


def conv2d_down2_bf16(x_nhwc, wpk, c_coarse, out=None):
    L = _lib.load()
    x = _map4(x_nhwc, "x_nhwc")
    B, H, W, cf = x.shape
    _dev(wpk, "wpk", torch.uint8)
    if wpk.numel() != L.fd_conv2d_packed_weight_2x2_bytes(c_coarse, cf, PACK_DOWN2) or wpk.numel() == 0:
        raise FutureDetHipError("conv2d_down2_bf16: wpk is not the PACK_DOWN2 pack of a [%d, %d, 2, 2] weight" % (c_coarse, cf))
    out = _out_map(out, (B, H // 2, W // 2, c_coarse), x, "out")
    check(L.fd_conv2d_down2_bf16(_p(x), B, H, W, cf, _p(wpk), c_coarse, _p(out), _stream()), "fd_conv2d_down2_bf16")
    return out


def conv2d_wgrad_2x2_bf16(coarse_nhwc, fine_nhwc, fine_major=False):
    L = _lib.load()
    co, fi = _map4(coarse_nhwc, "coarse_nhwc"), _map4(fine_nhwc, "fine_nhwc")
    B, H, W, cf = fi.shape
    cc = co.shape[3]
    if tuple(co.shape[:3]) != (B, H // 2, W // 2):
        raise FutureDetHipError("conv2d_wgrad_2x2_bf16: coarse %s is not the 2 x 2 / stride 2 map of fine %s" % (tuple(co.shape), tuple(fi.shape)))
    nbytes = L.fd_conv2d_wgrad_2x2_bf16_workspace_bytes(B, H, W, cc, cf)
    if nbytes == 0:
        raise FutureDetHipError("conv2d_wgrad_2x2_bf16: unsupported problem %s, %s" % (tuple(co.shape), tuple(fi.shape)))
    ws = torch.empty((nbytes,), dtype=torch.uint8, device=fi.device)
    dw = torch.empty((cf, cc, 2, 2) if fine_major else (cc, cf, 2, 2), dtype=torch.float32, device=fi.device)
    check(L.fd_conv2d_wgrad_2x2_bf16(_p(co), _p(fi), B, H, W, cc, cf, int(bool(fine_major)), _p(ws), ws.numel(), _p(dw), _stream()),
          "fd_conv2d_wgrad_2x2_bf16")
    return dw


def head_tail_max_groups():
    return int(_lib.load().fd_head_tail_bf16_max_groups())


def head_tail_wgrad_chunk():
    return int(_lib.load().fd_head_tail_wgrad_bf16_chunk())


def _head_tail_group(what, x, c0, w, bias, y):
    x = _dev(x, what + ": x", torch.bfloat16)
    w = _dev(w, what + ": weight", torch.float32)
    y = _dev(y, what + ": y", torch.float32)
    if bias is not None:
        bias = _dev(bias, what + ": bias", torch.float32)
    if x.dim() != 4 or w.dim() != 4 or tuple(w.shape[2:]) != (3, 3) or y.dim() != 4:
        raise FutureDetHipError("%s: needs x [B, H, W, C], a [k, cin, 3, 3] weight and y [B, k, H, W] (got %s, %s, %s)"
                                % (what, tuple(x.shape), tuple(w.shape), tuple(y.shape)))
    k, cin = int(w.shape[0]), int(w.shape[1])
    B, H, W, C = x.shape
    if tuple(y.shape) != (B, k, H, W) or (bias is not None and tuple(bias.shape) != (k,)):
        raise FutureDetHipError("%s: y must be [%d, %d, %d, %d] and the bias [%d] (got %s, %s)"
                                % (what, B, k, H, W, k, tuple(y.shape), None if bias is None else tuple(bias.shape)))
    if c0 < 0 or c0 % 8 or c0 + cin > C:
        raise FutureDetHipError("%s: channels %d .. %d are no 16-byte aligned slice of the %d channels of x" % (what, c0, c0 + cin - 1, C))
    rec = _lib.HeadTailGroup(x.data_ptr() + 2 * c0, w.data_ptr(), bias.data_ptr() if bias is not None else None, y.data_ptr(), C, cin, k)
    return rec, (B, H, W)


def _head_tail_launch(what, entry, records, with_workspace=False):
    L = _lib.load()
    shapes = set(s for _, s in records)
    if len(shapes) != 1:
        raise FutureDetHipError("%s: needs at least one group, all over the same B x H x W pixels (got %s)" % (what, sorted(shapes)))
    B, H, W = shapes.pop()
    step = head_tail_max_groups()
    for i in range(0, len(records), step):
        part = [r for r, _ in records[i:i + step]]
        arr = (_lib.HeadTailGroup * len(part))(*part)
        if with_workspace:
            nbytes = L.fd_head_tail_wgrad_bf16_workspace_bytes(B, H, W, sum(r.cin for r in part))
            if nbytes == 0:
                raise FutureDetHipError("%s: unsupported problem %d x %d x %d, cin %s" % (what, B, H, W, [r.cin for r in part]))
            ws = workspace.get("head_tail_wgrad", nbytes, torch.device("cuda", torch.cuda.current_device()))
            check(getattr(L, entry)(arr, len(part), B, H, W, _p(ws), ws.numel(), _stream()), entry)
        else:
            check(getattr(L, entry)(arr, len(part), B, H, W, _stream()), entry)


def head_tail_forward(groups):
    recs, ys = [], []
    for x, c0, w, bias in groups:
        x = _dev(x, "head_tail_forward: x", torch.bfloat16)
        w = _dev(w, "head_tail_forward: weight", torch.float32)
        if x.dim() != 4 or w.dim() != 4:
            raise FutureDetHipError("head_tail_forward: needs x [B, H, W, C] and a [k, cin, 3, 3] weight (got %s, %s)" % (tuple(x.shape), tuple(w.shape)))
        if bias is None:
            raise FutureDetHipError("head_tail_forward: every group needs a bias")
        y = torch.empty((x.shape[0], w.shape[0], x.shape[1], x.shape[2]), dtype=torch.float32, device=x.device)
        recs.append(_head_tail_group("head_tail_forward", x, c0, w, bias, y))
        ys.append(y)
    _head_tail_launch("head_tail_forward", "fd_head_tail_forward_bf16", recs)
    return ys


def head_tail_dgrad(groups):
    recs = [_head_tail_group("head_tail_dgrad", dx, c0, w, None, dy) for dx, c0, w, dy in groups]
    _head_tail_launch("head_tail_dgrad", "fd_head_tail_dgrad_bf16", recs)


def head_tail_wgrad(groups):
    recs, out = [], []
    for x, c0, cin, dy in groups:
        dy = _dev(dy, "head_tail_wgrad: dy", torch.float32)
        if dy.dim() != 4:
            raise FutureDetHipError("head_tail_wgrad: dy must be [B, k, H, W] (got %s)" % (tuple(dy.shape),))
        dw = torch.empty((dy.shape[1], cin, 3, 3), dtype=torch.float32, device=dy.device)
        db = torch.empty((dy.shape[1],), dtype=torch.float32, device=dy.device)
        recs.append(_head_tail_group("head_tail_wgrad", x, c0, dw, db, dy))
        out.append((dw, db))
    _head_tail_launch("head_tail_wgrad", "fd_head_tail_wgrad_bf16", recs, with_workspace=True)
    return out


def pack_conv2d_weight_f32(w_oihw):
    L = _lib.load()
    dev = w_oihw.device
    w = w_oihw.detach().to("cpu", torch.float32).contiguous()
    cout, cin, ks, _ = w.shape
    nbytes = L.fd_conv2d_f32_packed_weight_bytes(cout, cin, ks)
    if nbytes == 0:
        raise FutureDetHipError("fd_conv2d_f32: unsupported weight shape %s" % (tuple(w.shape),))
    host = torch.empty((nbytes,), dtype=torch.uint8)
    check(L.fd_conv2d_f32_pack_weight(ctypes.c_void_p(w.data_ptr()), cout, cin, ks, ctypes.c_void_p(host.data_ptr())),
          "fd_conv2d_f32_pack_weight")
    return host.to(dev)


def conv2d_nhwc_f32(x, wpk, bias, cout, ks, stride=1, relu=True, out=None, co_off=0, osy=1, osx=1, ooy=0, oox=0, tile=0):
    L = _lib.load()
    x = _dev(x, "x", torch.float32)
    B, H, W, cin = x.shape
    pad = 1 if ks == 3 else 0
    Ho, Wo = (H + 2 * pad - ks) // stride + 1, (W + 2 * pad - ks) // stride + 1
    if out is None:
        out = torch.empty((B, Ho * osy, Wo * osx, cout), dtype=torch.float32, device=x.device)
    _dev(out, "out", torch.float32)
# ... 1067 lines not shown
```

futuredet_amd/lib.py:

```python
import ctypes
import os

_HERE = os.path.dirname(os.path.abspath(__file__))
LIB_PATH = os.environ.get("FD_LIB_PATH") or os.path.join(_HERE, "libfuturedet_hip.so")
_lib = None

c_void_p = ctypes.c_void_p
c_int = ctypes.c_int
c_i64 = ctypes.c_int64
c_size_t = ctypes.c_size_t
c_float = ctypes.c_float


class MapView(ctypes.Structure):
    _fields_ = [("data", ctypes.c_void_p), ("group_stride", ctypes.c_int64), ("channel_stride", ctypes.c_int64), ("cell_stride", ctypes.c_int64),
                ("dtype", ctypes.c_int)]


ABI_VERSION = 8


class DecodeCfg(ctypes.Structure):
    _fields_ = [("H", c_int), ("W", c_int), ("out_size_factor", c_float), ("voxel_x", c_float), ("voxel_y", c_float),
                ("pc_x", c_float), ("pc_y", c_float), ("score_threshold", c_float), ("center_range", c_float * 6),
                ("nms_iou_threshold", c_float), ("nms_pre_max", c_int), ("nms_post_max", c_int), ("hm_channels", c_int),
                ("nms_kind", c_int), ("n_radius", c_int), ("circle_radius", c_float * 16)]


class IndexLevel(ctypes.Structure):
    _fields_ = [("D", ctypes.c_int32), ("H", ctypes.c_int32), ("W", ctypes.c_int32), ("ksize", ctypes.c_int32 * 3),
                ("stride", ctypes.c_int32 * 3), ("pad", ctypes.c_int32 * 3), ("words", c_void_p), ("prefix", c_void_p),
                ("coords", c_void_p), ("coords_rows", ctypes.c_int64)]


class ForecastBuffers(ctypes.Structure):
    _fields_ = [(n, c_void_p) for n in ("center", "quat", "velocity", "size", "fwd_idx", "fwd_ok", "bwd_idx", "bwd_ok", "match_idx", "cv_centers",
                                        "status", "traj_kind", "traj_src", "traj_first", "traj_group", "n_traj")]


class TargetsCfg(ctypes.Structure):
    _fields_ = [("H", c_int), ("W", c_int), ("T", c_int), ("n_max", c_int), ("max_objs", c_int), ("n_sets", c_int), ("n_tasks", c_int),
                ("task_classes", c_int * 16), ("radius_mult", c_int), ("min_radius", c_int), ("out_size_factor", c_float), ("voxel_x", c_float),
                ("voxel_y", c_float), ("pc_x", c_float), ("pc_y", c_float), ("gaussian_overlap", ctypes.c_double)]


class OptimTable(ctypes.Structure):
    _fields_ = [(n, c_void_p) for n in ("params", "numel", "offset", "flags", "step", "coef", "chunks", "partials", "norm", "grad", "exp_avg",
                                        "exp_avg_sq")] + [("total", c_i64), ("n_tensors", ctypes.c_int32), ("n_chunks", ctypes.c_int32),
                                                          ("chunk", ctypes.c_int32)]


class LossCfg(ctypes.Structure):
    _fields_ = [(n, ctypes.c_int32) for n in ("B", "H", "W", "M", "n_tasks", "dense", "T", "D", "row_stride")] + [
        ("col", ctypes.c_int32 * 14), ("code_weights", ctypes.c_double * 14), ("code_weights_forecast", ctypes.c_double * 14),
        ("weight", ctypes.c_double)]


class LossTask(ctypes.Structure):
    _fields_ = [("hm", c_void_p), ("hm_target", c_void_p), ("ind", c_void_p), ("cat", c_void_p), ("mask", c_void_p * 7), ("maps", c_void_p * 7),
                ("anno_box", c_void_p * 7), ("C", ctypes.c_int32), ("sig", c_void_p), ("d_hm", c_void_p), ("d_maps", c_void_p * 7)]


class HeadTailGroup(ctypes.Structure):
    _fields_ = [("x", c_void_p), ("w", c_void_p), ("bias", c_void_p), ("y", c_void_p), ("x_stride", c_i64), ("cin", c_int), ("k", c_int)]


class DenseBnNhwcGroup(ctypes.Structure):
    _fields_ = [("gamma", c_void_p), ("beta", c_void_p), ("running_mean", c_void_p), ("running_var", c_void_p), ("num_batches_tracked", c_void_p),
                ("c", c_int), ("eps", c_float), ("momentum", ctypes.c_double)]


class AugmentRecord(ctypes.Structure):
    _fields_ = [("flip_a", ctypes.c_int32), ("flip_b", ctypes.c_int32), ("c", c_float), ("s", c_float), ("rot", c_float), ("scale", c_float),
                ("tx", ctypes.c_double), ("ty", ctypes.c_double), ("tz", ctypes.c_double)]


SIGNATURES = {
    "fd_abi_version": (c_int, []),
    "fd_last_error": (ctypes.c_char_p, []),
    "fd_tuning_set": (c_int, [ctypes.c_char_p, c_int]),
    "fd_voxelize_workspace_bytes": (c_size_t, [c_i64, c_i64]),
    "fd_voxelize": (c_int, [c_void_p, c_i64, c_void_p, c_int, c_void_p, c_void_p, c_int, c_i64, c_int, c_void_p, c_void_p, c_int,
                            c_void_p, c_int, c_void_p, c_void_p, c_void_p, c_size_t, c_void_p]),
    "fd_index_num_cols": (c_i64, [c_int, c_int, c_int]),
    "fd_index_workspace_bytes": (c_size_t, [c_i64]),
    "fd_index_mark": (c_int, [c_void_p, c_void_p, c_i64, c_int, c_int, c_int, c_int, c_void_p, c_void_p]),
    "fd_index_downsample": (c_int, [c_void_p, c_int, c_int, c_int, c_int, c_void_p, c_void_p, c_void_p, c_void_p, c_void_p]),
    "fd_index_scan": (c_int, [c_void_p, c_i64, c_void_p, c_void_p, c_void_p, c_size_t, c_void_p]),
    "fd_index_coords": (c_int, [c_void_p, c_void_p, c_int, c_int, c_int, c_int, c_void_p, c_void_p]),
    "fd_index_lookup": (c_int, [c_void_p, c_void_p, c_int, c_int, c_int, c_int, c_void_p, c_void_p, c_i64, c_void_p, c_void_p]),
    "fd_rows_permute": (c_int, [c_void_p, c_int, c_void_p, c_void_p, c_i64, c_void_p, c_int, c_int, c_void_p]),
    "fd_rulebook": (c_int, [c_void_p, c_void_p, c_int, c_int, c_int, c_int, c_void_p, c_i64, c_void_p, c_i64, c_int, c_void_p, c_void_p,
                            c_void_p, c_void_p, c_void_p]),
    "fd_spconv_packed_weight_bytes": (c_size_t, [c_int, c_int, c_int, c_int]),
    "fd_spconv_pack_weight": (c_int, [c_void_p, c_int, c_int, c_int, c_int, c_void_p]),
    "fd_spconv_apply": (c_int, [c_void_p, c_i64, c_void_p, c_void_p, c_void_p, c_int, c_void_p, c_i64, c_void_p, c_int, c_int, c_i64,
                                c_void_p, c_i64, c_int, c_int, c_int, c_void_p, c_void_p]),
    "fd_spconv_num_ranges": (c_int, [c_i64, c_int, c_int, c_int]),
    "fd_spconv_wants_balanced_ranges": (c_int, [c_int, c_int, c_int]),
    "fd_spconv_ranges_workspace_bytes": (c_size_t, [c_i64]),
    "fd_spconv_ranges": (c_int, [c_void_p, c_i64, c_int, c_i64, c_void_p, c_int, c_void_p, c_void_p, c_size_t, c_void_p]),
    "fd_densify": (c_int, [c_void_p, c_int, c_int, c_void_p, c_void_p, c_int, c_int, c_int, c_int, c_void_p, c_int, c_i64,
                           c_i64, c_i64, c_i64, c_i64, c_void_p]),
    "fd_conv2d_packed_weight_bytes": (c_size_t, [c_int, c_int, c_int]),
    "fd_conv2d_pack_weight": (c_int, [c_void_p, c_int, c_int, c_int, c_void_p]),
    "fd_conv2d_nhwc_bf16": (c_int, [c_void_p, c_int, c_int, c_int, c_int, c_void_p, c_void_p, c_int, c_int, c_int, c_int, c_int,
                                    c_void_p, c_int, c_int, c_int, c_int, c_int, c_int, c_void_p]),
    "fd_conv2d_f32_packed_weight_bytes": (c_size_t, [c_int, c_int, c_int]),
    "fd_conv2d_f32_pack_weight": (c_int, [c_void_p, c_int, c_int, c_int, c_void_p]),
    "fd_conv2d_f32_num_tiles": (c_int, []),
    "fd_conv2d_nhwc_f32": (c_int, [c_void_p, c_int, c_int, c_int, c_int, c_void_p, c_void_p, c_int, c_int, c_int, c_int, c_int,
                                   c_void_p, c_int, c_int, c_int, c_int, c_int, c_int, c_int, c_void_p]),
    "fd_conv2d_shuffle_nhwc_f32": (c_int, [c_void_p, c_int, c_int, c_int, c_int, c_void_p, c_void_p, c_int, c_int, c_int, c_void_p, c_int, c_int, c_int,
                                           c_void_p]),
    "fd_conv2d_grouped_nhwc_f32": (c_int, [c_void_p, c_int, c_int, c_int, c_int, c_int, c_void_p, c_void_p, c_void_p, c_int, c_void_p, c_int, c_int,
                                           c_int, c_void_p]),
    "fd_conv2d_wino_f32_num_tiles": (c_int, []),
    "fd_conv2d_wino_f32_packed_weight_bytes": (c_size_t, [c_int, c_int]),
    "fd_conv2d_wino_f32_pack_weight": (c_int, [c_void_p, c_int, c_int, c_void_p]),
    "fd_conv2d_wino_nhwc_f32": (c_int, [c_void_p, c_int, c_int, c_int, c_int, c_void_p, c_void_p, c_int, c_int, c_void_p, c_int, c_int, c_int,
                                        c_void_p]),
    "fd_decode_workspace_bytes": (c_size_t, [c_int, ctypes.POINTER(DecodeCfg)]),
    "fd_centerpoint_decode": (c_int, [c_void_p, c_i64, c_void_p, c_i64, c_void_p, c_i64, c_void_p, c_i64, c_void_p, c_i64,
                                      c_int, ctypes.POINTER(DecodeCfg), c_void_p, c_void_p, c_void_p, c_void_p, c_void_p,
                                      c_size_t, c_void_p]),
    "fd_centerpoint_decode_maps": (c_int, [ctypes.POINTER(MapView)] * 5 + [c_int, ctypes.POINTER(DecodeCfg), c_void_p, c_void_p, c_void_p, c_void_p,
                                           c_void_p, c_size_t, c_void_p]),
    "fd_centerpoint_decode_packed": (c_int, [ctypes.POINTER(MapView)] * 6 + [c_int, c_int, ctypes.POINTER(DecodeCfg), c_int, c_void_p, c_void_p, c_void_p,
                                             c_void_p, c_void_p, c_void_p, c_void_p, c_void_p, c_void_p, c_void_p, c_size_t, c_void_p]),
    "fd_assemble_detections": (c_int, [c_void_p, c_void_p, c_void_p, c_void_p, ctypes.POINTER(MapView), c_int, c_int, c_int, c_void_p, c_void_p,
                                       c_void_p, c_void_p, c_void_p, c_void_p]),
    "fd_nms_workspace_bytes": (c_size_t, [c_int]),
    "fd_rotated_nms": (c_int, [c_void_p, c_int, c_float, c_void_p, c_void_p, c_void_p, c_size_t, c_void_p]),
    "fd_boxes_iou_bev": (c_int, [c_void_p, c_int, c_void_p, c_int, c_void_p, c_void_p]),
    "fd_pillar_encode": (c_int, [c_void_p, c_void_p, c_void_p, c_void_p, c_i64, c_int, c_int, c_int, c_float, c_float, c_float,
                                 c_float, c_void_p, c_void_p, c_void_p, c_int, c_void_p, c_void_p, c_void_p, c_int, c_int,
                                 c_void_p, c_int, c_void_p]),
    "fd_pillar_scatter": (c_int, [c_void_p, c_int, c_int, c_int, c_void_p, c_void_p, c_i64, c_int, c_int, c_int, c_void_p, c_int,
                                  c_i64, c_i64, c_i64, c_i64, c_int, c_void_p]),
    "fd_forecast_chains": (c_int, [c_void_p, c_void_p, c_void_p, c_void_p, c_int, c_int, ctypes.c_double, c_void_p, c_void_p,
                                   c_void_p, c_void_p, c_void_p, c_void_p, c_void_p, c_void_p]),
    "fd_det_to_global_boxes": (c_int, [c_void_p, c_int, c_void_p, c_void_p, c_void_p, c_void_p, c_void_p, c_void_p, c_void_p, c_void_p, c_void_p]),
    "fd_forecast_groups": (c_int, [c_void_p, c_int, ctypes.c_double, c_void_p, c_void_p]),
    "fd_forecast_from_detections": (c_int, [c_void_p, c_void_p, c_int, c_int, c_int, c_int, c_void_p, c_void_p, ctypes.c_double, ctypes.c_double,
                                            ctypes.POINTER(ForecastBuffers), c_void_p]),
    "fd_nearest_rows": (c_int, [c_void_p, c_int, c_void_p, c_int, c_int, c_void_p, c_void_p]),
    "fd_index_pyramid": (c_int, [c_void_p, c_void_p, c_i64, c_int, c_int, ctypes.POINTER(IndexLevel), c_void_p, c_void_p, c_size_t,
                                 c_void_p]),
    "fd_index_pyramid_coords": (c_int, [c_int, c_int, ctypes.POINTER(IndexLevel), c_void_p]),
    "fd_rows_place": (c_int, [c_void_p, c_void_p, c_int, c_int, c_int, c_int, c_void_p, c_void_p, c_i64, c_void_p, c_int, c_void_p,
                              c_int, c_int, c_void_p]),
    "fd_sweep_assemble_workspace_bytes": (c_size_t, [c_i64]),
    "fd_sweep_assemble": (c_int, [c_void_p, c_int, c_int, c_i64, c_void_p, c_int, c_float, c_void_p, c_void_p, c_void_p,
                                  c_size_t, c_void_p]),
    "fd_deform_adapt_packed_weight_bytes": (c_size_t, [c_int]),
    "fd_deform_adapt_pack_weight": (c_int, [c_void_p, c_void_p, c_int, c_void_p]),
    "fd_deform_adapt_nhwc": (c_int, [c_void_p, c_int, c_int, c_int, c_int, c_int, c_void_p, c_void_p, c_void_p, c_void_p, c_void_p, c_void_p]),
    "fd_deform_adapt_backward_workspace_bytes": (c_size_t, [c_int, c_int, c_int]),
    "fd_deform_adapt_backward": (c_int, [c_void_p, c_void_p, c_void_p, c_void_p, c_void_p, c_void_p, c_int, c_int, c_int, c_int, c_void_p, c_void_p,
                                         c_void_p, c_void_p, c_size_t, c_void_p]),
    "fd_deform_adapt_pack_weight_device": (c_int, [c_void_p, c_void_p, c_void_p, c_void_p]),
    "fd_spconv_wgrad_workspace_bytes": (c_size_t, [c_int, c_i64, c_int, c_int]),
    "fd_spconv_wgrad": (c_int, [c_void_p, c_i64, c_void_p, c_void_p, c_i64, c_int, c_i64, c_void_p, c_int, c_int, c_void_p, c_void_p, c_size_t,
                                c_void_p]),
    "fd_rulebook_transpose": (c_int, [c_void_p, c_i64, c_int, c_i64, c_void_p, c_i64, c_void_p, c_i64, c_void_p]),
    "fd_spconv_pack_weight_device": (c_int, [c_void_p, c_int, c_int, c_int, c_int, c_void_p, c_void_p]),
    "fd_spconv_wgrad_bf16_workspace_bytes": (c_size_t, [c_int, c_i64, c_int, c_int]),
    "fd_spconv_wgrad_bf16": (c_int, [c_void_p, c_i64, c_void_p, c_void_p, c_i64, c_int, c_i64, c_void_p, c_int, c_int, c_void_p, c_void_p, c_size_t,
                                     c_void_p]),
    "fd_spconv_pack_weight_device_bf16": (c_int, [c_void_p, c_int, c_int, c_int, c_int, c_void_p, c_void_p]),
    "fd_conv2d_pack_weight_dev": (c_int, [c_void_p, c_int, c_int, c_int, c_int, c_void_p, c_void_p]),
    "fd_conv2d_wgrad_bf16_chunk": (c_int, []),
    "fd_conv2d_wgrad_bf16_workspace_bytes": (c_size_t, [c_int, c_int, c_int, c_int, c_int, c_int]),
    "fd_conv2d_wgrad_bf16": (c_int, [c_void_p, c_void_p, c_int, c_int, c_int, c_int, c_int, c_int, c_void_p, c_size_t, c_void_p, c_void_p]),
    "fd_conv2d_s2_dgrad_bf16": (c_int, [c_void_p, c_int, c_int, c_int, c_int, c_int, c_void_p, c_void_p, c_void_p]),
    "fd_conv2d_wgrad_s2_bf16_workspace_bytes": (c_size_t, [c_int, c_int, c_int, c_int, c_int]),
    "fd_conv2d_wgrad_s2_bf16": (c_int, [c_void_p, c_void_p, c_int, c_int, c_int, c_int, c_int, c_void_p, c_size_t, c_void_p, c_void_p]),
    "fd_conv2d_down2_bf16": (c_int, [c_void_p, c_int, c_int, c_int, c_int, c_void_p, c_int, c_void_p, c_void_p]),
    "fd_conv2d_packed_weight_2x2_bytes": (c_size_t, [c_int, c_int, c_int]),
    "fd_conv2d_pack_weight_2x2_dev": (c_int, [c_void_p, c_int, c_int, c_int, c_int, c_void_p, c_void_p]),
    "fd_conv2d_wgrad_2x2_bf16_workspace_bytes": (c_size_t, [c_int, c_int, c_int, c_int, c_int]),
    "fd_conv2d_wgrad_2x2_bf16": (c_int, [c_void_p, c_void_p, c_int, c_int, c_int, c_int, c_int, c_int, c_void_p, c_size_t, c_void_p, c_void_p]),
    "fd_head_tail_bf16_max_groups": (c_int, []),
    "fd_head_tail_wgrad_bf16_chunk": (c_int, []),
    "fd_head_tail_wgrad_bf16_workspace_bytes": (c_size_t, [c_int, c_int, c_int, c_int]),
    "fd_head_tail_forward_bf16": (c_int, [ctypes.POINTER(HeadTailGroup), c_int, c_int, c_int, c_int, c_void_p]),
    "fd_head_tail_dgrad_bf16": (c_int, [ctypes.POINTER(HeadTailGroup), c_int, c_int, c_int, c_int, c_void_p]),
    "fd_head_tail_wgrad_bf16": (c_int, [ctypes.POINTER(HeadTailGroup), c_int, c_int, c_int, c_int, c_void_p, c_size_t, c_void_p]),
    "fd_dense_gather": (c_int, [c_void_p, c_i64, c_i64, c_i64, c_i64, c_int, c_void_p, c_i64, c_void_p, c_int, c_void_p, c_void_p]),
    "fd_pillar_train_workspace_bytes": (c_size_t, [c_i64, c_int]),
    "fd_pillar_train_forward": (c_int, [c_void_p, c_void_p, c_void_p, c_i64, c_int, c_int, c_int, c_float, c_float, c_float, c_float,
                                        c_void_p, c_void_p, c_void_p, c_int, c_float, c_void_p, c_void_p, c_void_p, c_int, c_float,
                                        c_void_p, c_void_p, c_void_p, c_void_p, c_void_p, c_void_p, c_size_t, c_void_p]),
    "fd_pillar_train_backward": (c_int, [c_void_p, c_void_p, c_void_p, c_i64, c_int, c_int, c_int, c_float, c_float, c_float, c_float,
                                         c_void_p, c_void_p, c_void_p, c_int, c_void_p, c_void_p, c_void_p, c_int, c_void_p,
                                         c_void_p, c_void_p, c_void_p, c_void_p, c_void_p, c_void_p, c_void_p, c_size_t, c_void_p]),
    "fd_pillar_train_forward_dev": (c_int, [c_void_p, c_void_p, c_void_p, c_void_p, c_int, c_i64, c_int, c_int, c_int, c_float, c_float,
                                            c_float, c_float, c_void_p, c_void_p, c_void_p, c_int, c_float, c_void_p, c_void_p, c_void_p,
                                            c_int, c_float, c_void_p, c_void_p, c_void_p, c_void_p, c_void_p, c_void_p, c_size_t, c_void_p]),
    "fd_pillar_train_backward_dev": (c_int, [c_void_p, c_void_p, c_void_p, c_void_p, c_int, c_i64, c_int, c_int, c_int, c_float, c_float,
                                             c_float, c_float, c_void_p, c_void_p, c_void_p, c_int, c_void_p, c_void_p, c_void_p, c_int,
                                             c_void_p, c_void_p, c_void_p, c_void_p, c_void_p, c_void_p, c_void_p, c_void_p, c_size_t,
                                             c_void_p]),
    "fd_pillar_train_running_stats_dev": (c_int, [c_void_p, c_void_p, c_int, ctypes.c_double, c_void_p, c_int, c_i64, c_int, c_void_p,
                                                  c_void_p, c_void_p, c_void_p]),
    "fd_targets_workspace_bytes": (c_size_t, [c_int, c_int, c_int, c_int]),
    "fd_assign_targets": (c_int, [c_void_p, c_void_p, c_void_p, c_void_p, c_int, ctypes.POINTER(TargetsCfg), c_void_p, c_void_p, c_void_p, c_void_p,
                                  c_void_p, c_void_p, c_void_p, c_void_p, c_size_t, c_void_p]),
    "fd_optim_chunk": (c_int, []),
    "fd_optim_zero_grad": (c_int, [ctypes.POINTER(OptimTable), c_void_p]),
    "fd_optim_adam_step": (c_int, [ctypes.POINTER(OptimTable)] + [ctypes.c_double] * 6 + [c_void_p]),
    "fd_optim_adam_step_dev": (c_int, [ctypes.POINTER(OptimTable), c_void_p, c_int, c_void_p, c_void_p]),
    "fd_rows_colsum_chunk": (c_int, []),
    "fd_rows_colsum_workspace_bytes": (c_size_t, [c_i64, c_int]),
    "fd_rows_colsum": (c_int, [c_void_p, c_i64, c_void_p, c_int, c_int, c_void_p, c_void_p, c_size_t, c_void_p]),
    "fd_levels_overflow": (c_int, [c_void_p, c_void_p, c_int, c_void_p, c_void_p]),
    "fd_augment_points": (c_int, [c_void_p, c_i64, c_int, c_void_p, c_void_p, c_void_p, c_void_p]),
    "fd_augment_boxes": (c_int, [c_void_p, c_void_p, c_void_p, c_void_p, c_int, c_int, c_int, c_void_p]),
    "fd_loss_chunk": (c_int, []),
    "fd_centerhead_loss_terms": (c_size_t, [ctypes.POINTER(LossCfg)]),
    "fd_centerhead_loss_workspace_bytes": (c_size_t, [ctypes.POINTER(LossCfg), c_int]),
    "fd_centerhead_loss_forward": (c_int, [ctypes.POINTER(LossCfg), ctypes.POINTER(LossTask), c_void_p, c_void_p, c_size_t, c_void_p]),
    "fd_centerhead_loss_backward": (c_int, [ctypes.POINTER(LossCfg), ctypes.POINTER(LossTask), c_void_p, c_void_p, c_void_p, c_size_t, c_void_p]),
    "fd_sparse_bn_chunk": (c_int, []),
    "fd_sparse_bn_workspace_bytes": (c_size_t, [c_i64, c_int]),
    "fd_sparse_bn_train_forward": (c_int, [c_void_p, c_void_p, c_void_p, c_void_p, c_i64, c_void_p, c_int, c_int, c_float, ctypes.c_double,
                                           c_void_p, c_void_p, c_void_p, c_void_p, c_void_p, c_void_p, c_size_t, c_void_p]),
    "fd_sparse_bn_train_backward": (c_int, [c_void_p, c_void_p, c_void_p, c_void_p, c_void_p, c_i64, c_void_p, c_int, c_int,
                                            c_void_p, c_void_p, c_void_p, c_void_p, c_void_p, c_size_t, c_void_p]),
    "fd_dense_bn_chunk": (c_int, []),
    "fd_dense_bn_workspace_bytes": (c_size_t, [c_i64, c_int, c_i64]),
    "fd_dense_bn_train_forward": (c_int, [c_void_p, c_void_p, c_void_p, c_i64, c_int, c_i64, c_int, c_float, ctypes.c_double,
                                          c_void_p, c_void_p, c_void_p, c_void_p, c_void_p, c_void_p, c_size_t, c_void_p]),
    "fd_dense_bn_train_backward": (c_int, [c_void_p, c_void_p, c_void_p, c_void_p, c_void_p, c_i64, c_int, c_i64, c_int,
                                           c_void_p, c_void_p, c_void_p, c_void_p, c_size_t, c_void_p]),
    "fd_dense_bn_nhwc_chunk": (c_int, []),
    "fd_dense_bn_nhwc_stat_groups": (c_int, []),
    "fd_dense_bn_nhwc_apply_blocks": (c_int, []),
    "fd_dense_bn_nhwc_workspace_bytes": (c_size_t, [c_i64, c_int]),
    "fd_dense_bn_nhwc_train_forward_bf16": (c_int, [c_void_p, ctypes.POINTER(DenseBnNhwcGroup), c_int, c_i64, c_int, c_int, c_void_p, c_void_p,
                                                    c_void_p, c_size_t, c_void_p]),
    "fd_dense_bn_nhwc_train_backward_bf16": (c_int, [c_void_p, c_void_p, c_void_p, c_void_p, ctypes.POINTER(DenseBnNhwcGroup), c_int, c_i64, c_int,
                                                     c_int, c_void_p, c_void_p, c_void_p, c_void_p, c_size_t, c_void_p]),
}
for _name in ("fd_sparse_bn_train_forward", "fd_sparse_bn_train_backward"):
    SIGNATURES[_name + "_bf16"] = SIGNATURES[_name]



class FutureDetHipError(RuntimeError):
    pass


def load():
    global _lib
    if _lib is None:
        if not os.path.isfile(LIB_PATH):
            raise FutureDetHipError(
                "libfuturedet_hip.so is not built (%s). Run `python -c 'import __graft_entry__ as g; g.build()'` "
                "or `python futuredet_amd/build.py`; there is no CPU fallback for this path." % LIB_PATH)
        L = ctypes.CDLL(LIB_PATH)
        for name, (res, args) in SIGNATURES.items():
            fn = getattr(L, name)
            fn.restype = res
            fn.argtypes = args
        if L.fd_abi_version() != ABI_VERSION:
            raise FutureDetHipError("%s reports ABI %d, these bindings are written for %d: rebuild it (python futuredet_amd/build.py --force)"
                                    % (LIB_PATH, L.fd_abi_version(), ABI_VERSION))
        _lib = L
    return _lib


def check(status, what):
    if status != 0:
        msg = load().fd_last_error()
        raise FutureDetHipError("%s failed (%d): %s" % (what, status, msg.decode() if msg else "?"))
```

futuredet_amd/sparse.py:

```python
import math

import numpy as np
import torch
from torch import nn

from . import hip_ops

CH_ALIGN = 16


def _triple(v):
    if isinstance(v, (list, tuple, np.ndarray)):
        assert len(v) == 3
        return [int(x) for x in v]
    return [int(v)] * 3


def pad_channels(c):
    return max(CH_ALIGN, (c + CH_ALIGN - 1) // CH_ALIGN * CH_ALIGN)


class SparseConvTensor(object):
    def __init__(self, features, indices, spatial_shape, batch_size, grid=None, _index=None):
        self.spatial_shape = [int(v) for v in spatial_shape]
        self.batch_size = int(batch_size)
        self.indice_dict = {}
        self.grid = grid
        if _index is not None:
            self.index = _index
            self.features = features
            return
        indices = indices.int().contiguous()
        D, H, W = self.spatial_shape
        idx = hip_ops.SparseIndex(self.batch_size, D, H, W, features.device)
        n_dev = torch.zeros((1,), dtype=torch.int32, device=features.device)
        idx.mark(indices)
        idx.scan(n_dev)
        idx.finalize(int(n_dev.cpu()[0]))
        row_of = idx.lookup(indices)
        self.index = idx
        self._true_channels = features.shape[1]
        src = features.float().contiguous()
        if torch.is_grad_enabled() and src.requires_grad:
            self.features = _RowsPermute.apply(src, row_of, idx.n)
        else:
            self.features = hip_ops.rows_permute(src, row_of, features.shape[1], torch.float32, n_rows=idx.n)

    @property
    def indices(self):
        return self.index.coords

    def find_indice_pair(self, key):
        return self.indice_dict.get(key) if key is not None else None

    def dense(self, channels_first=True):
        feats = self.features.contiguous()
        if torch.is_grad_enabled() and feats.requires_grad:
            out = _Densify.apply(feats, self.index)
        else:
            out = hip_ops.densify(feats, self.index)
        B, C, D = self.batch_size, feats.shape[1], self.index.D
        out = out.view(B, C, D, self.index.H, self.index.W)
        if not channels_first:
            out = out.permute(0, 2, 3, 4, 1).contiguous()
        return out


class SparseModule(nn.Module):
    pass


class _RowsPermute(torch.autograd.Function):

    @staticmethod
    def forward(ctx, src, row_of, n_rows):
        ctx.save_for_backward(row_of)
        return hip_ops.rows_permute(src, row_of, src.shape[1], torch.float32, n_rows=n_rows)

    @staticmethod
    def backward(ctx, grad):
        (row_of,) = ctx.saved_tensors
        keep = row_of >= 0
        g = grad[row_of.long().clamp(min=0)]
        return g * keep[:, None].to(g.dtype), None, None


class _Densify(torch.autograd.Function):

    @staticmethod
    def forward(ctx, feats, index):
        ctx.index, ctx.dtype = index, feats.dtype
        return hip_ops.densify(feats, index)

    @staticmethod
    def backward(ctx, grad):
        g = hip_ops.dense_gather(grad.float(), ctx.index, grad.shape[1] // ctx.index.D)
        return (g if ctx.dtype == torch.float32 else g.to(ctx.dtype)), None


class _ReluToBf16(torch.autograd.Function):

    @staticmethod
    def forward(ctx, x):
        y = torch.relu(x).to(torch.bfloat16)
        ctx.save_for_backward(y)
        return y

    @staticmethod
    def backward(ctx, dy):
        (y,) = ctx.saved_tensors
        return dy.float() * (y > 0)


def relu_to_bf16(x):
    return _ReluToBf16.apply(x)


class _SparseConvFunction(torch.autograd.Function):

    @staticmethod
    def forward(ctx, feats, weight, bias, nbr, n_out, subm):
        wpk = hip_ops.pack_spconv_weight_device(weight, hip_ops.PACK_PLAIN, feats.dtype)
        out = hip_ops.spconv_apply(feats, wpk, bias, nbr, n_out, weight.shape[2])
        ctx.save_for_backward(feats, weight)
        ctx.nbr, ctx.n_out, ctx.subm, ctx.has_bias = nbr, n_out, subm, bias is not None
        return out

    @staticmethod
    def backward(ctx, dy):
        feats, weight = ctx.saved_tensors
        nbr, n_out = ctx.nbr, ctx.n_out
        n_in, cin_p = feats.shape
        dt = feats.dtype
        dy = dy.to(dt).contiguous()
        dx = dw = db = None
        if ctx.needs_input_grad[0]:
            if ctx.subm:
                wt = hip_ops.pack_spconv_weight_device(weight, hip_ops.PACK_FLIPPED_TRANSPOSED, dt)
                dx = hip_ops.spconv_apply(dy, wt, None, nbr, n_in, cin_p)
            else:
                inv = getattr(nbr, "inv", None)
                if inv is None:
                    inv = nbr.inv = hip_ops.rulebook_transpose(nbr, n_out, n_in)
                    if getattr(nbr, "n_in_dev", None) is not None:
                        inv.n_dev, inv.n_expected = nbr.n_in_dev, nbr.n_in_expected
                wt = hip_ops.pack_spconv_weight_device(weight, hip_ops.PACK_TRANSPOSED, dt)
                dx = hip_ops.spconv_apply(dy, wt, None, inv, n_in, cin_p)
        if ctx.needs_input_grad[1]:
            dw = hip_ops.spconv_wgrad(feats, dy, nbr, n_out)
        if ctx.has_bias and ctx.needs_input_grad[2]:
            if getattr(nbr, "n_dev", None) is not None:
                db = hip_ops.rows_colsum(dy[:n_out], nbr.n_dev)
            else:
                db = dy[:n_out].sum(0) if dt == torch.float32 else dy[:n_out].float().sum(0)
        return dx, dw, db, None, None, None


class _SparseBatchNormFunction(torch.autograd.Function):

    @staticmethod
    def forward(ctx, x, gamma, beta, residual, bn, relu, n_dev=None):
        y, saved = hip_ops.sparse_bn_train_forward(x, gamma, beta, bn.running_mean, bn.running_var, bn.num_batches_tracked, bn.eps,
                                                   bn.momentum, residual=residual, relu=relu, n_dev=n_dev)
        for buf in (bn.running_mean, bn.running_var, bn.num_batches_tracked):
            torch.autograd.graph.increment_version(buf)
        ctx.save_for_backward(x, y, gamma, saved)
        ctx.relu, ctx.n_dev = relu, n_dev
        return y

    @staticmethod
    @torch.autograd.function.once_differentiable
    def backward(ctx, dy):
        x, y, gamma, saved = ctx.saved_tensors
        want_res = ctx.needs_input_grad[3]
        dx, dres, dgamma, dbeta = hip_ops.sparse_bn_train_backward(dy.to(x.dtype).contiguous(), x, y, gamma, saved, relu=ctx.relu,
                                                                   want_residual=want_res, n_dev=ctx.n_dev)
        return dx, dgamma, dbeta, dres, None, None, None


def batch_norm_fusable(features, bn):
    return (isinstance(bn, nn.BatchNorm1d) and bn.training and torch.is_grad_enabled() and bn.affine and bn.track_running_stats
            and bn.momentum is not None and bn.running_mean is not None and features.is_cuda and features.dtype in (torch.float32, torch.bfloat16)
            and bn.weight.dtype == torch.float32 and bn.weight.device == features.device and features.dim() == 2
            and features.shape[0] >= 2 and hip_ops.sparse_bn_channels_ok(features.shape[1]))


def batch_norm_act(features, bn, residual=None, relu=True, n_dev=None):
    if not batch_norm_fusable(features, bn):
        raise hip_ops.FutureDetHipError("batch_norm_act: needs a training-mode affine BatchNorm1d with running statistics and a momentum, "
                                        "gradients enabled and fp32 or bf16 device features [n >= 2, C], C a multiple of 16 up to 128 (got %s %s)"
                                        % (tuple(features.shape), features.dtype))
    if residual is not None:
        residual = residual.to(features.dtype).contiguous()
    if n_dev is None:
        return _SparseBatchNormFunction.apply(features.contiguous(), bn.weight, bn.bias, residual, bn, bool(relu))
    return _SparseBatchNormFunction.apply(features.contiguous(), bn.weight, bn.bias, residual, bn, bool(relu), n_dev)


class SparseConvolution(SparseModule):
    def __init__(self, ndim, in_channels, out_channels, kernel_size=3, stride=1, padding=0, dilation=1, groups=1,
                 bias=True, subm=False, indice_key=None):
        super().__init__()
        assert ndim == 3 and groups == 1 and _triple(dilation) == [1, 1, 1]
        self.in_channels, self.out_channels = in_channels, out_channels
        self.kernel_size = _triple(kernel_size)
        self.stride = _triple(stride)
        self.padding = _triple(padding)
        self.subm = subm
        self.indice_key = indice_key
        self.weight = nn.Parameter(torch.Tensor(*self.kernel_size, in_channels, out_channels))
        if bias:
            self.bias = nn.Parameter(torch.Tensor(out_channels))
        else:
            self.register_parameter("bias", None)
        self.reset_parameters()
        self._packed = {}
        self.register_load_state_dict_post_hook(lambda m, keys: m._packed.clear())

    def reset_parameters(self):
        nn.init.kaiming_uniform_(self.weight, a=math.sqrt(5))
        if self.bias is not None:
            fan_in = self.in_channels * int(np.prod(self.kernel_size))
            bound = 1 / math.sqrt(fan_in)
            nn.init.uniform_(self.bias, -bound, bound)

    def geometry(self):
        if self.subm:
            return self.kernel_size, [1, 1, 1], [k // 2 for k in self.kernel_size]
        return self.kernel_size, self.stride, self.padding

    def packed_weight(self, dtype, bn=None):
        key = (dtype, id(bn), self.weight.device)
        ver = self.weight._version + (self.bias._version if self.bias is not None else 0)
        if bn is not None:
            ver += bn.weight._version + bn.bias._version + bn.running_mean._version + bn.running_var._version
        hit = self._packed.get(key)
        if hit is not None and hit[0] == ver:
            return hit[1]
        K = int(np.prod(self.kernel_size))
        w = self.weight.detach().float().reshape(K, self.in_channels, self.out_channels)
        b = self.bias.detach().float() if self.bias is not None else None
        if bn is not None:
            from .nn_utils import fold_bn

            w, b = fold_bn(w, b, bn, 2)
        cin_p, cout_p = pad_channels(self.in_channels), pad_channels(self.out_channels)
        wp = torch.zeros((K, cin_p, cout_p), dtype=torch.float32, device=w.device)
        wp[:, : self.in_channels, : self.out_channels] = w
        bp = None
        if b is not None:
            bp = torch.zeros((cout_p,), dtype=torch.float32, device=w.device)
            bp[: self.out_channels] = b
            bp = bp.contiguous()
        packed = (hip_ops.pack_spconv_weight(wp, dtype), bp, cin_p, cout_p)
        self._packed[key] = (ver, packed)
        return packed

    def rulebook_for(self, x):
        data = x.find_indice_pair(self.indice_key)
        if data is not None:
            return data
        ks, st, pd = self.geometry()
        if self.subm:
            out_index = x.index
        else:
            out_index = x.index.downsample(ks, st, pd)
            n_dev = torch.zeros((1,), dtype=torch.int32, device=x.features.device)
            out_index.scan(n_dev)
            out_index.finalize(int(n_dev.cpu()[0]))
        nbr = x.index.rulebook(out_index, ks, st, pd)
        data = (out_index, nbr)
        if self.indice_key is not None:
            x.indice_dict[self.indice_key] = data
        return data

    def forward(self, x):
        assert isinstance(x, SparseConvTensor)
        out_index, nbr = self.rulebook_for(x)
        params = [self.weight] + ([self.bias] if self.bias is not None else [])
        if torch.is_grad_enabled() and (x.features.requires_grad or (self.training and any(p.requires_grad for p in params))):
            return self._forward_autograd(x, out_index, nbr)
        feats = x.features
        if feats.dtype not in (torch.float32, torch.bfloat16):
            raise NotImplementedError("sparse convolution takes fp32 or bf16 features (features are %s)" % feats.dtype)
        wpk, bias, cin_p, cout_p = self.packed_weight(feats.dtype)
        if feats.shape[1] != cin_p:
            feats = torch.nn.functional.pad(feats, (0, cin_p - feats.shape[1]))
        out = hip_ops.spconv_apply(feats.contiguous(), wpk, bias, nbr, out_index.n, cout_p)
        if cout_p != self.out_channels:
            out = out[:, : self.out_channels].contiguous()
        y = SparseConvTensor(out, None, out_index.spatial_shape, x.batch_size, grid=x.grid, _index=out_index)
        y.indice_dict = x.indice_dict
        return y


    def _forward_autograd(self, x, out_index, nbr):
        if x.features.dtype not in (torch.float32, torch.bfloat16):
            raise NotImplementedError("sparse convolution training takes fp32 or bf16 features (features are %s)" % x.features.dtype)
        K = int(np.prod(self.kernel_size))
        cin_p, cout_p = pad_channels(self.in_channels), pad_channels(self.out_channels)
        F = torch.nn.functional
        w = F.pad(self.weight.float().reshape(K, self.in_channels, self.out_channels),
                  (0, cout_p - self.out_channels, 0, cin_p - self.in_channels)).contiguous()
        b = F.pad(self.bias.float(), (0, cout_p - self.out_channels)).contiguous() if self.bias is not None else None
        feats = x.features
        if feats.shape[1] != cin_p:
            feats = F.pad(feats, (0, cin_p - feats.shape[1]))
        out = _SparseConvFunction.apply(feats.contiguous(), w, b, nbr, out_index.n, self.subm)
        if cout_p != self.out_channels:
            out = out[:, : self.out_channels]
        y = SparseConvTensor(out, None, out_index.spatial_shape, x.batch_size, grid=x.grid, _index=out_index)
        y.indice_dict = x.indice_dict
        return y


class SparseConv3d(SparseConvolution):
    def __init__(self, in_channels, out_channels, kernel_size, stride=1, padding=0, dilation=1, groups=1, bias=True,
                 indice_key=None):
        super().__init__(3, in_channels, out_channels, kernel_size, stride, padding, dilation, groups, bias,
                         indice_key=indice_key)


class SubMConv3d(SparseConvolution):
    def __init__(self, in_channels, out_channels, kernel_size, stride=1, padding=0, dilation=1, groups=1, bias=True,
                 indice_key=None):
        super().__init__(3, in_channels, out_channels, kernel_size, stride, padding, dilation, groups, bias, subm=True,
                         indice_key=indice_key)


class SparseSequential(SparseModule):

    def __init__(self, *args, **kwargs):
        super().__init__()
        for i, m in enumerate(args):
            self.add_module(str(i), m)
        for k, m in kwargs.items():
            self.add_module(k, m)

    def __getitem__(self, idx):
        return list(self._modules.values())[idx]

    def __len__(self):
        return len(self._modules)

    def add(self, module, name=None):
        self.add_module(str(len(self._modules)) if name is None else name, module)

    def forward(self, x):
        for m in self._modules.values():
            if isinstance(m, SparseModule):
                x = m(x)
            elif isinstance(x, SparseConvTensor):
                if x.features.shape[0] != 0:
                    x.features = m(x.features)
            else:
                x = m(x)
        return x
```

include/futuredet_hip.h:

```cpp
#ifndef FUTUREDET_HIP_H
#define FUTUREDET_HIP_H

#include <stddef.h>
#include <stdint.h>

#ifdef __cplusplus
extern "C" {
#endif

#define FD_OK 0
#define FD_EINVAL (-1)
#define FD_EWORKSPACE (-2)
#define FD_ELAUNCH (-3)

typedef void *fd_stream_t;

int fd_abi_version(void);
const char *fd_last_error(void);
int fd_tuning_set(const char *name, int value);

size_t fd_voxelize_workspace_bytes(int64_t n_points, int64_t max_voxels);
int fd_voxelize(const float *points, int64_t n_points, const int32_t *n_points_dev, int ndim, const float *range6_host,
                const float *voxel_size3_host, int max_points, int64_t max_voxels, int batch_idx,
                float *out_voxels, float *out_mean, int mean_stride, int32_t *out_coors, int coor_cols,
                int32_t *out_num_points, int32_t *out_num_voxels, void *workspace, size_t workspace_bytes,
                fd_stream_t stream);

int64_t fd_index_num_cols(int B, int H, int W);
size_t fd_index_workspace_bytes(int64_t num_cols);
int fd_index_mark(const int32_t *coords , const int32_t *n_dev ,
                  int64_t n_max, int B, int D, int H, int W, uint64_t *words, fd_stream_t stream);
int fd_index_downsample(const uint64_t *in_words, int B, int D, int H, int W, const int *ksize3,
                        const int *stride3, const int *pad3, uint64_t *out_words, fd_stream_t stream);
int fd_index_scan(const uint64_t *words, int64_t num_cols, int32_t *prefix, int32_t *n_active_dev,
                  void *workspace, size_t workspace_bytes, fd_stream_t stream);
int fd_index_coords(const uint64_t *words, const int32_t *prefix, int B, int D, int H, int W,
                    int32_t *coords , fd_stream_t stream);
int fd_index_lookup(const uint64_t *words, const int32_t *prefix, int B, int D, int H, int W,
                    const int32_t *coords_in, const int32_t *n_dev, int64_t n_max, int32_t *row_of,
                    fd_stream_t stream);
int fd_rows_permute(const float *src, int c_src, const int32_t *row_of, const int32_t *n_dev, int64_t n_max,
                    void *dst, int c_dst, int dst_bf16, fd_stream_t stream);
int fd_rulebook(const uint64_t *in_words, const int32_t *in_prefix, int B, int Din, int Hin, int Win,
                const int32_t *out_coords, int64_t out_rows, const int32_t *n_out_dev, int64_t nbr_stride, int fill_tail, const int *ksize3,
                const int *stride3, const int *pad3, int32_t *nbr, fd_stream_t stream);

size_t fd_spconv_packed_weight_bytes(int K, int cin, int cout, int dtype);
int fd_spconv_pack_weight(const float *w_kio_host, int K, int cin, int cout, int dtype, void *wpacked_host);
int fd_spconv_apply(const void *in_feats, int64_t n_in, const void *wpacked, const float *bias, const void *residual,
                    int relu, const int32_t *nbr, int64_t nbr_stride, const int32_t *ranges ,
                    int n_ranges, int K, int64_t n_out, const int32_t *n_out_dev ,
                    int64_t n_expected ,
                    int cin, int cout, int dtype, void *out_feats, fd_stream_t stream);
int fd_spconv_num_ranges(int64_t n_out, int cin, int cout, int dtype);
int fd_spconv_wants_balanced_ranges(int cin, int cout, int dtype);
size_t fd_spconv_ranges_workspace_bytes(int64_t n_out);
int fd_spconv_ranges(const int32_t *nbr, int64_t nbr_stride, int K, int64_t n_out, const int32_t *n_out_dev, int n_ranges,
                     int32_t *ranges , void *workspace, size_t workspace_bytes, fd_stream_t stream);

int fd_densify(const void *feats, int c, int dtype, const uint64_t *words, const int32_t *prefix, int B, int D,
               int H, int W, void *out, int out_dtype, int64_t stride_b, int64_t stride_c, int64_t stride_y,
               int64_t stride_x, int64_t n_rows ,
               fd_stream_t stream);

size_t fd_conv2d_packed_weight_bytes(int cout, int cin, int ks);
int fd_conv2d_pack_weight(const float *w_oihw_host, int cout, int cin, int ks, void *wpacked_host);
int fd_conv2d_nhwc_bf16(const void *x, int B, int H, int W, int cin, const void *wpacked, const float *bias, int cout,
                        int ks, int stride, int pad, int relu, void *y, int cout_total, int co_off, int osy, int osx,
                        int ooy, int oox, fd_stream_t stream);
size_t fd_conv2d_f32_packed_weight_bytes(int cout, int cin, int ks);
int fd_conv2d_f32_pack_weight(const float *w_oihw_host, int cout, int cin, int ks, void *wpacked_host);
int fd_conv2d_f32_num_tiles(void);
int fd_conv2d_nhwc_f32(const float *x, int B, int H, int W, int cin, const void *wpacked, const float *bias, int cout, int ks,
                       int stride, int pad, int relu, float *y, int cout_total, int co_off, int osy, int osx, int ooy, int oox,
                       int tile , fd_stream_t stream);
int fd_conv2d_shuffle_nhwc_f32(const float *x, int B, int H, int W, int cin, const void *wpacked, const float *bias, int cout_sub, int k,
                               int relu, float *y, int cout_total, int co_off, int tile, fd_stream_t stream);
int fd_conv2d_grouped_nhwc_f32(const float *x, int B, int H, int W, int groups, int cin_g, const void *wpacked, const float *bias,
                               const int *counts_host, int relu, float *y, int cout_total, int co_off, int tile, fd_stream_t stream);
int fd_conv2d_wino_f32_num_tiles(void);
size_t fd_conv2d_wino_f32_packed_weight_bytes(int cout, int cin);
int fd_conv2d_wino_f32_pack_weight(const float *w_oihw_host, int cout, int cin, void *wpacked_host);
int fd_conv2d_wino_nhwc_f32(const float *x, int B, int H, int W, int cin, const void *wpacked, const float *bias, int cout, int relu,
                            float *y, int cout_total, int co_off, int tile , fd_stream_t stream);

typedef struct fd_decode_cfg {
    int H, W;
    float out_size_factor, voxel_x, voxel_y, pc_x, pc_y;
    float score_threshold;
    float center_range[6];
    float nms_iou_threshold;
    int nms_pre_max, nms_post_max;
    int hm_channels;
    int nms_kind;
    int n_radius;
    float circle_radius[16];
} fd_decode_cfg;

typedef struct fd_map_view {
    const void *data;
    int64_t group_stride, channel_stride, cell_stride;
    int dtype;
} fd_map_view;

size_t fd_decode_workspace_bytes(int G, const fd_decode_cfg *cfg);
int fd_centerpoint_decode_maps(const fd_map_view *hm, const fd_map_view *reg, const fd_map_view *height, const fd_map_view *dim,
                               const fd_map_view *rot, int G, const fd_decode_cfg *cfg_host, float *out_boxes7, float *out_scores,
                               int32_t *out_cell, int32_t *out_count, void *workspace, size_t workspace_bytes, fd_stream_t stream);
int fd_assemble_detections(const float *boxes7, const float *scores, const int32_t *cell, const int32_t *count, const fd_map_view *vel,
                           int B, int post_max, int S, const int32_t *step_group, const int32_t *step_vel_channel,
                           const int32_t *step_label, float *packed, int32_t *counts_out, fd_stream_t stream);
int fd_centerpoint_decode_packed(const fd_map_view *hm, const fd_map_view *reg, const fd_map_view *height, const fd_map_view *dim,
                                 const fd_map_view *rot, const fd_map_view *vel, int G, int B, const fd_decode_cfg *cfg_host, int S,
                                 const int32_t *step_group, const int32_t *step_vel_channel, const int32_t *step_label, float *out_boxes7,
                                 float *out_scores, int32_t *out_cell, int32_t *out_count, float *packed, int32_t *counts_out, void *workspace,
                                 size_t workspace_bytes, fd_stream_t stream);
int fd_centerpoint_decode(const float *hm, int64_t hm_gstride, const float *reg, int64_t reg_gstride,
                          const float *height, int64_t height_gstride, const float *dim, int64_t dim_gstride,
                          const float *rot, int64_t rot_gstride, int G, const fd_decode_cfg *cfg_host,
                          float *out_boxes7, float *out_scores, int32_t *out_cell, int32_t *out_count,
                          void *workspace, size_t workspace_bytes, fd_stream_t stream);

size_t fd_nms_workspace_bytes(int n);
int fd_rotated_nms(const float *boxes7, int n, float thresh, int64_t *keep, int32_t *out_count,
                   void *workspace, size_t workspace_bytes, fd_stream_t stream);
int fd_boxes_iou_bev(const float *a7, int na, const float *b7, int nb, float *out, fd_stream_t stream);

#define FD_SWEEP_HAS_TRANSFORM 1
#define FD_SWEEP_REMOVE_CLOSE 2
typedef struct fd_sweep_desc {
    double m[16];
    int64_t row_begin, row_end;
    float time;
    int32_t flags;
} fd_sweep_desc;
size_t fd_sweep_assemble_workspace_bytes(int64_t n_rows);
int fd_sweep_assemble(const float *raw, int raw_cols, int keep_cols, int64_t n_rows, const fd_sweep_desc *sweeps_dev,
                      int n_sweeps, float min_distance, float *out_points, int32_t *out_count, void *workspace,
                      size_t workspace_bytes, fd_stream_t stream);

int fd_pillar_encode(const float *voxels, const int32_t *num_points, const int32_t *coors4, const int32_t *n_dev,
                     int64_t m_max, int max_points, int ndim, int with_distance, float vx, float vy, float x_offset,
                     float y_offset, const float *w1, const float *scale1, const float *shift1, int units1,
                     const float *w2, const float *scale2, const float *shift2, int units2, int out_dtype, void *out,
                     int out_stride, fd_stream_t stream);

int fd_pillar_scatter(const void *feats, int c, int feat_stride, int dtype, const int32_t *coors4, const int32_t *n_dev,
                      int64_t m_max, int B, int H, int W, void *out, int out_dtype, int64_t stride_b, int64_t stride_c,
                      int64_t stride_y, int64_t stride_x, int zero_first, fd_stream_t stream);


int fd_forecast_chains(const double *centers, const double *velocity, const int32_t *counts, const double *time_dev, int T,
                       int n_max, double reject_thresh, int32_t *fwd_idx, int32_t *fwd_ok, int32_t *bwd_idx, int32_t *bwd_ok,
                       int32_t *match_idx, double *cv_centers, int32_t *status, fd_stream_t stream);

int fd_det_to_global_boxes(const float *box3d9, int n, const double *cs_rotation4_host, const double *cs_translation3_host,
                           const double *pose_rotation4_host, const double *pose_translation3_host, double *center,
                           double *quat, double *velocity, float *size, fd_stream_t stream);
int fd_forecast_groups(const double *centers3, int n, double match_thresh, int32_t *ids, fd_stream_t stream);

typedef struct fd_forecast_buffers {
    double *center, *quat, *velocity;
    float *size;
    int32_t *fwd_idx, *fwd_ok, *bwd_idx, *bwd_ok, *match_idx;
    double *cv_centers;
    int32_t *status;
    int32_t *traj_kind, *traj_src, *traj_first, *traj_group, *n_traj;
} fd_forecast_buffers;
int fd_forecast_from_detections(const float *packed, const int32_t *counts, int B, int T, int post, int row_floats,
                                const double *records_dev, const double *time_dev, double reject_thresh, double match_thresh,
                                const fd_forecast_buffers *out, fd_stream_t stream);

int fd_nearest_rows(const double *library, int n_library, const double *queries, int n_queries, int dim, int32_t *idx, fd_stream_t stream);

typedef struct fd_index_level {
    int32_t D, H, W;
    int32_t ksize[3], stride[3], pad[3];
    uint64_t *words;
    int32_t *prefix;
    int32_t *coords;
    int64_t coords_rows;
} fd_index_level;
int fd_index_pyramid(const int32_t *coords, const int32_t *n_dev, int64_t n_max_per_sample, int B, int n_levels,
                     const fd_index_level *levels_host, int32_t *counts_dev, void *workspace, size_t workspace_bytes,
                     fd_stream_t stream);
int fd_index_pyramid_coords(int B, int n_levels, const fd_index_level *levels_host, fd_stream_t stream);

int fd_rows_place(const uint64_t *words, const int32_t *prefix, int B, int D, int H, int W, const int32_t *coords_in,
                  const int32_t *n_dev, int64_t n_max, const float *src, int c_src, void *dst, int c_dst, int dst_bf16,
                  fd_stream_t stream);

size_t fd_deform_adapt_packed_weight_bytes(int bf16);
int fd_deform_adapt_pack_weight(const float *w_cls_oihw_host, const float *w_reg_oihw_host, int bf16, void *wpacked_host);
int fd_deform_adapt_nhwc(const void *x, int B, int H, int W, int C, int bf16, const float *off_w, const float *off_b, const float *offsets,
                         const void *wpacked, void *y, fd_stream_t stream);

size_t fd_deform_adapt_backward_workspace_bytes(int B, int H, int W);
int fd_deform_adapt_backward(const float *x, const float *offsets, const float *w_cls_oihw, const float *w_reg_oihw, const float *y, const float *dy,
                             int B, int H, int W, int C, float *dx, float *doffsets, float *dw, void *workspace, size_t workspace_bytes,
                             fd_stream_t stream);
int fd_deform_adapt_pack_weight_device(const float *w_cls_oihw, const float *w_reg_oihw, void *wpacked, fd_stream_t stream);

size_t fd_spconv_wgrad_workspace_bytes(int K, int64_t n_out, int cin, int cout);
int fd_spconv_wgrad(const float *in_feats, int64_t n_in, const float *dy, const int32_t *nbr, int64_t nbr_stride, int K, int64_t n_out,
                    const int32_t *n_out_dev, int cin, int cout, float *dw, void *workspace, size_t workspace_bytes, fd_stream_t stream);
int fd_rulebook_transpose(const int32_t *nbr, int64_t nbr_stride, int K, int64_t n_out, const int32_t *n_out_dev, int64_t n_in, int32_t *inv,
                          int64_t inv_stride, fd_stream_t stream);
int fd_spconv_pack_weight_device(const float *w_kio, int K, int cin, int cout, int mode, void *wpacked, fd_stream_t stream);
int fd_dense_gather(const float *dense, int64_t stride_b, int64_t stride_c, int64_t stride_y, int64_t stride_x, int D, const int32_t *coords,
                    int64_t n_rows, const int32_t *n_dev, int c, float *feats, fd_stream_t stream);

size_t fd_spconv_wgrad_bf16_workspace_bytes(int K, int64_t n_out, int cin, int cout);
int fd_spconv_wgrad_bf16(const void *in_feats, int64_t n_in, const void *dy, const int32_t *nbr, int64_t nbr_stride, int K, int64_t n_out,
                         const int32_t *n_out_dev, int cin, int cout, float *dw, void *workspace, size_t workspace_bytes, fd_stream_t stream);
int fd_spconv_pack_weight_device_bf16(const float *w_kio, int K, int cin, int cout, int mode, void *wpacked, fd_stream_t stream);

int fd_conv2d_pack_weight_dev(const float *w_oihw, int cout, int cin, int ks, int mode, void *wpacked, fd_stream_t stream);
int fd_conv2d_wgrad_bf16_chunk(void);
size_t fd_conv2d_wgrad_bf16_workspace_bytes(int B, int H, int W, int cin, int cout, int ks);
int fd_conv2d_wgrad_bf16(const void *x, const void *dy, int B, int H, int W, int cin, int cout, int ks, void *workspace,
                         size_t workspace_bytes, float *dw, fd_stream_t stream);

typedef struct fd_head_tail_group {
    void *x;
    float *w;
    float *bias;
    void *y;
    int64_t x_stride;
    int cin;
    int k;
} fd_head_tail_group;
int fd_head_tail_bf16_max_groups(void);
int fd_head_tail_wgrad_bf16_chunk(void);
size_t fd_head_tail_wgrad_bf16_workspace_bytes(int B, int H, int W, int cin_sum);
int fd_head_tail_forward_bf16(const fd_head_tail_group *groups, int n_groups, int B, int H, int W, fd_stream_t stream);
int fd_head_tail_dgrad_bf16(const fd_head_tail_group *groups, int n_groups, int B, int H, int W, fd_stream_t stream);
int fd_head_tail_wgrad_bf16(const fd_head_tail_group *groups, int n_groups, int B, int H, int W, void *workspace, size_t workspace_bytes,
                            fd_stream_t stream);

#define FD_TARGETS_MAX_TASKS 16
typedef struct fd_targets_cfg {
    int H, W;
    int T, n_max, max_objs;
    int n_sets;
    int n_tasks;
    int task_classes[FD_TARGETS_MAX_TASKS];
    int radius_mult;
    int min_radius;
    float out_size_factor, voxel_x, voxel_y, pc_x, pc_y;
    double gaussian_overlap;
} fd_targets_cfg;
size_t fd_targets_workspace_bytes(int B, int T, int maps_per_step, int max_objs);
int fd_assign_targets(const float *boxes, const int32_t *counts, const int32_t *classes, const int32_t *trajectory, int B,
                      const fd_targets_cfg *cfg, float *hm, int64_t *ind, uint8_t *mask, int64_t *cat, float *anno_box,
                      float *gt_boxes_and_cls, int32_t *status, void *workspace, size_t workspace_bytes, fd_stream_t stream);

size_t fd_pillar_train_workspace_bytes(int64_t m, int max_points);
int fd_pillar_train_forward(const float *voxels, const int32_t *num_points, const int32_t *coors4, int64_t m, int max_points, int ndim,
                            int with_distance, float vx, float vy, float x_offset, float y_offset, const float *w1, const float *gamma1,
                            const float *beta1, int units1, float eps1, const float *w2, const float *gamma2, const float *beta2, int units2,
                            float eps2, float *out, float *mean1, float *var1, float *mean2, float *var2, void *workspace,
                            size_t workspace_bytes, fd_stream_t stream);
int fd_pillar_train_backward(const float *voxels, const int32_t *num_points, const int32_t *coors4, int64_t m, int max_points, int ndim,
                             int with_distance, float vx, float vy, float x_offset, float y_offset, const float *w1, const float *gamma1,
                             const float *beta1, int units1, const float *w2, const float *gamma2, const float *beta2, int units2,
                             const float *dout, float *dw1, float *dgamma1, float *dbeta1, float *dw2, float *dgamma2, float *dbeta2,
                             void *workspace, size_t workspace_bytes, fd_stream_t stream);

int fd_pillar_train_forward_dev(const float *voxels, const int32_t *num_points, const int32_t *coors4, const int32_t *seg_counts, int n_seg,
                                int64_t seg_stride, int max_points, int ndim, int with_distance, float vx, float vy, float x_offset,
                                float y_offset, const float *w1, const float *gamma1, const float *beta1, int units1, float eps1,
                                const float *w2, const float *gamma2, const float *beta2, int units2, float eps2, float *out, float *mean1,
                                float *var1, float *mean2, float *var2, void *workspace, size_t workspace_bytes, fd_stream_t stream);
int fd_pillar_train_backward_dev(const float *voxels, const int32_t *num_points, const int32_t *coors4, const int32_t *seg_counts, int n_seg,
                                 int64_t seg_stride, int max_points, int ndim, int with_distance, float vx, float vy, float x_offset,
                                 float y_offset, const float *w1, const float *gamma1, const float *beta1, int units1, const float *w2,
                                 const float *gamma2, const float *beta2, int units2, const float *dout, float *dw1, float *dgamma1,
                                 float *dbeta1, float *dw2, float *dgamma2, float *dbeta2, void *workspace, size_t workspace_bytes,
                                 fd_stream_t stream);
int fd_pillar_train_running_stats_dev(const float *mean, const float *var, int channels, double momentum, const int32_t *seg_counts, int n_seg,
                                      int64_t seg_stride, int max_points, float *running_mean, float *running_var,
                                      int64_t *num_batches_tracked, fd_stream_t stream);

#define FD_OPTIM_CHUNK 4096
#define FD_OPTIM_DECAY 1
#define FD_OPTIM_HAS_GRAD 2
typedef struct fd_optim_table {
    const void *params;
    const void *numel, *offset;
    const void *flags;
    void *step;
    void *coef;
    const void *chunks;
    void *partials;
    void *norm;
    float *grad, *exp_avg, *exp_avg_sq;
    int64_t total;
    int32_t n_tensors, n_chunks, chunk;
} fd_optim_table;
int fd_optim_chunk(void);
int fd_optim_zero_grad(const fd_optim_table *table, fd_stream_t stream);
int fd_optim_adam_step(const fd_optim_table *table, double lr, double beta1, double beta2, double eps, double wd, double max_norm,
                       fd_stream_t stream);
int fd_optim_adam_step_dev(const fd_optim_table *table, const double *hyper, int clip, const int32_t *skip, fd_stream_t stream);

#define FD_ROWS_COLSUM_CHUNK 512
int fd_rows_colsum_chunk(void);
size_t fd_rows_colsum_workspace_bytes(int64_t n, int C);
int fd_rows_colsum(const void *x, int64_t n, const int32_t *n_dev, int C, int dtype, float *out, void *workspace, size_t workspace_bytes,
                   fd_stream_t stream);
int fd_levels_overflow(const int32_t *counts, const int32_t *caps, int n_levels, int32_t *flag, fd_stream_t stream);

#define FD_AUGMENT_MAX_ROWS (1 << 28)
typedef struct fd_augment_record {
    int32_t flip_a, flip_b;
    float c, s, rot, scale;
    double tx, ty, tz;
} fd_augment_record;
int fd_augment_points(const float *src, int64_t n_rows, int ndim, const int32_t *perm, const fd_augment_record *rec, float *dst,
                      fd_stream_t stream);
int fd_augment_boxes(const float *boxes, const int32_t *counts, const fd_augment_record *recs, float *out, int B, int T, int n_max,
                     fd_stream_t stream);

#define FD_LOSS_CHUNK 2048
#define FD_LOSS_MAX_TASKS 16
#define FD_LOSS_MAX_STEPS 7
#define FD_LOSS_MAX_OBJS 2048
typedef struct fd_loss_cfg {
    int32_t B;
    int32_t H;
    int32_t W;
    int32_t M;
    int32_t n_tasks;
    int32_t dense;
    int32_t T;
    int32_t D;
    int32_t row_stride;
    int32_t col[14];
    double code_weights[14];
    double code_weights_forecast[14];
    double weight;
} fd_loss_cfg;
typedef struct fd_loss_task {
    const float *hm;
    const float *hm_target;
    const int64_t *ind;
    const int64_t *cat;
    const void *mask[7];
    const float *maps[7];
    const float *anno_box[7];
    int32_t C;
    float *sig;
    float *d_hm;
    float *d_maps[7];
} fd_loss_task;
int fd_loss_chunk(void);
size_t fd_centerhead_loss_terms(const fd_loss_cfg *cfg);
size_t fd_centerhead_loss_workspace_bytes(const fd_loss_cfg *cfg, int max_classes);
int fd_centerhead_loss_forward(const fd_loss_cfg *cfg, const fd_loss_task *tasks, float *terms, void *workspace, size_t workspace_bytes,
                               fd_stream_t stream);
int fd_centerhead_loss_backward(const fd_loss_cfg *cfg, const fd_loss_task *tasks, const float *terms, const float *go, void *workspace,
// ... 67 lines not shown
```

Measured before the change: 282.1.

## Precompute compacted per-chunk tap lists for f32 SubM convs on side stream

Adds a chunk-plan kernel that precomputes each 128-row chunk's compacted neighbor lists and per-tap counts once per rulebook. The f32 compact and c32 spconv kernels gain a PLAN variant that loads these lists directly, skipping the in-kernel compact_taps pass and one barrier per chunk. The plan is built on the side stream alongside rulebooks and cached on the nbr tensor, so the two SubM convs in each block reuse it. It costs an extra plan buffer, a build kernel, and more template instantiations. Training paths opt out.

```diff
diff --git a/futuredet_amd/backbones.py b/futuredet_amd/backbones.py
--- a/futuredet_amd/backbones.py
+++ b/futuredet_amd/backbones.py
@@ -211,6 +211,9 @@
                             r = hip_ops.ranges_for(nbr, cp, cp)
                             if r[0] is not None:
                                 made.append(r[0])
+                        if dt == torch.float32 and nbr.shape[0] == 27 and dst_l.n > 0 and \
+                                hip_ops._lib.load().fd_spconv_plan_wanted(cp, cp, 0):
+                            made.append(hip_ops.plan_for(nbr, dst_l.n, *hip_ops.row_split(nbr, dst_l.n, cp, cp))[0])
                 for t in made:
                     t.record_stream(main)
         x = feats0
diff --git a/futuredet_amd/csrc/fd_common.h b/futuredet_amd/csrc/fd_common.h
--- a/futuredet_amd/csrc/fd_common.h
+++ b/futuredet_amd/csrc/fd_common.h
@@ -28,6 +28,8 @@
     int cin, cout, dtype;
     void *out;
     hipStream_t stream;
+    const int *plan;
+    int64_t plan_stride;
 };
 
 constexpr int kSpconvMaxTaps = 27;
@@ -102,7 +104,7 @@
     X(kTuneSpconvRG, "spconv_rg") X(kTuneSpconvV1, "spconv_v1") X(kTuneConvNT, "conv_nt") X(kTuneV2RangesPerCU, "v2_ranges_per_cu") \
     X(kTuneSpconvC32, "spconv_c32") X(kTuneBf16GP, "bf16_gp") X(kTuneBf16RG, "bf16_rg") X(kTuneBf16Depth, "bf16_depth")        \
     X(kTuneBf16NW, "bf16_nw") X(kTuneBf16Win, "bf16_win") X(kTuneF32ResRG, "f32_res_rg") X(kTuneConvStrip, "conv_strip")       \
-    X(kTuneF32ResNW, "f32_res_nw")
+    X(kTuneF32ResNW, "f32_res_nw") X(kTuneSpconvPlan, "spconv_plan")
 #define FD_TUNE_ENUM(key, name) key,
 enum TuneKey { FD_TUNE_KNOBS(FD_TUNE_ENUM) kTuneCount };
 #undef FD_TUNE_ENUM
diff --git a/futuredet_amd/csrc/fd_spconv.hip b/futuredet_amd/csrc/fd_spconv.hip
--- a/futuredet_amd/csrc/fd_spconv.hip
+++ b/futuredet_amd/csrc/fd_spconv.hip
@@ -239,9 +239,10 @@
     return FD_OK;
 }
 
-extern "C" int fd_spconv_apply(const void *in_feats, int64_t n_in, const void *wpacked, const float *bias, const void *residual, int relu,
-                               const int32_t *nbr, int64_t nbr_stride, const int32_t *ranges, int n_ranges, int K, int64_t n_out,
-                               const int32_t *n_out_dev, int64_t n_expected, int cin, int cout, int dtype, void *out_feats, fd_stream_t stream) {
+namespace {
+int spconv_apply(const void *in_feats, int64_t n_in, const void *wpacked, const float *bias, const void *residual, int relu, const int32_t *nbr,
+                 int64_t nbr_stride, const int32_t *ranges, int n_ranges, int K, int64_t n_out, const int32_t *n_out_dev, int64_t n_expected, int cin,
+                 int cout, int dtype, void *out_feats, fd_stream_t stream, const int32_t *plan, int64_t plan_stride) {
     FD_REQUIRE(K >= 1 && K <= fd::kSpconvMaxTaps, "fd_spconv_apply: K must be in [1,27]");
     FD_REQUIRE(dtype == 0 || dtype == 1, "fd_spconv_apply: dtype must be 0 (f32) or 1 (bf16)");
     FD_REQUIRE(n_out >= 0 && n_out <= nbr_stride && n_out < (1ll << 31), "fd_spconv_apply: n_out out of range");
@@ -250,7 +251,7 @@
     if (n_out == 0) return FD_OK;
     FD_REQUIRE(in_feats && wpacked && nbr && out_feats, "fd_spconv_apply: null argument");
     const fd::SpconvCall c{in_feats, n_in, wpacked, bias, residual, relu, nbr, nbr_stride, ranges, n_ranges, K, (int)n_out, n_out_dev, n_expected,
-                           cin, cout, dtype, out_feats, fd::as_stream(stream)};
+                           cin, cout, dtype, out_feats, fd::as_stream(stream), plan, plan_stride};
     if (dtype == 0 && !fd::tuning(fd::kTuneSpconvV1) && cin == 16 && fd::tuning(fd::kTuneF32ResRG) >= 0) {
         if (fd::spconv_f32_res16_dispatch(c)) return fd::check_launch("fd_spconv_apply(f32 resident)");
     }
@@ -281,3 +282,24 @@
     }
     return fd::check_launch("fd_spconv_apply");
 }
+}
+
+extern "C" int fd_spconv_apply(const void *in_feats, int64_t n_in, const void *wpacked, const float *bias, const void *residual, int relu,
+                               const int32_t *nbr, int64_t nbr_stride, const int32_t *ranges, int n_ranges, int K, int64_t n_out,
+                               const int32_t *n_out_dev, int64_t n_expected, int cin, int cout, int dtype, void *out_feats, fd_stream_t stream) {
+    return spconv_apply(in_feats, n_in, wpacked, bias, residual, relu, nbr, nbr_stride, ranges, n_ranges, K, n_out, n_out_dev, n_expected, cin, cout,
+                        dtype, out_feats, stream, nullptr, 0);
+}
+
+extern "C" int fd_spconv_apply_plan(const void *in_feats, int64_t n_in, const void *wpacked, const float *bias, const void *residual, int relu,
+                                    const int32_t *nbr, int64_t nbr_stride, const int32_t *ranges, int n_ranges, int K, int64_t n_out,
+                                    const int32_t *n_out_dev, int64_t n_expected, int cin, int cout, int dtype, void *out_feats,
+                                    const int32_t *plan, int64_t plan_stride, fd_stream_t stream) {
+    if (plan) {
+        FD_REQUIRE(K == fd::kSpconvMaxTaps && dtype == 0 && cin == cout, "fd_spconv_apply_plan: a chunk plan belongs to an fp32 SubM layer (K = 27)");
+        FD_REQUIRE(plan_stride >= fd_spconv_plan_stride(n_out), "fd_spconv_apply_plan: plan_stride below fd_spconv_plan_stride(n_out)");
+        if (!fd_spconv_plan_wanted(cin, cout, dtype)) plan = nullptr;
+    }
+    return spconv_apply(in_feats, n_in, wpacked, bias, residual, relu, nbr, nbr_stride, ranges, n_ranges, K, n_out, n_out_dev, n_expected, cin, cout,
+                        dtype, out_feats, stream, plan, plan_stride);
+}
diff --git a/futuredet_amd/csrc/fd_spconv_c32.hip b/futuredet_amd/csrc/fd_spconv_c32.hip
--- a/futuredet_amd/csrc/fd_spconv_c32.hip
+++ b/futuredet_amd/csrc/fd_spconv_c32.hip
@@ -9,7 +9,7 @@
 constexpr sk::Layout L = sk::layout(TM, COUT, TS, 32);
 static_assert(((sk::kMaxTaps + TS - 1) / TS) * (TM / WR / 32) <= L.item_slot, "item list slot");
 
-template <int CIN, int DEPTH>
+template <int CIN, int DEPTH, bool PLAN>
 __global__ void __launch_bounds__(256) spconv_f32_c32(const float *__restrict__ in, const float4 *__restrict__ wp, const float *__restrict__ bias,
                                                       const float *__restrict__ residual, int relu, const int *__restrict__ nbr, int64_t nbr_stride,
                                                       int K, int n_out, const int *__restrict__ n_out_dev, float *__restrict__ out, unsigned in_bytes,
@@ -29,7 +29,8 @@
     if (r_begin >= r_end) return;
     sk::cut_chunks<TM>(r_begin, r_end, n_chunks, chunk_rows);
     int pre[sk::kSliceRegs<TM>];
-    sk::fetch_slice<TM>(pre, nbr, nbr_stride, K, r_begin);
+    const int k_fetch = PLAN ? sk::kPlanRows : K;
+    sk::fetch_slice<TM>(pre, nbr, nbr_stride, k_fetch, r_begin);
 
     const int ln = lane & 31, lh = lane >> 5;
     const int ts = wave, wr = 0;
@@ -40,11 +41,15 @@
     for (int chunk = 0; chunk < n_chunks; ++chunk) {
         int row0, n_rows;
         if (!sk::chunk_span(r_begin, r_end, chunk_rows, chunk, row0, n_rows)) break;
-        sk::stage_chunk<TM, COUT, TS, 32>(pre, s_list, s_pad, s_acc, bias, residual, K, row0, n_rows);
+        if constexpr (PLAN) {
+            sk::stage_plan_chunk<TM, COUT, TS, 32>(pre, s_list, s_cnt, s_pad, s_acc, bias, residual, row0, n_rows);
+        } else {
+            sk::stage_chunk<TM, COUT, TS, 32>(pre, s_list, s_pad, s_acc, bias, residual, K, row0, n_rows);
+            __syncthreads();
+            sk::compact_taps<TM, WR>(s_list, s_cnt, K);
+        }
         __syncthreads();
-        sk::compact_taps<TM, WR>(s_list, s_cnt, K);
-        __syncthreads();
-        if (chunk + 1 < n_chunks) sk::fetch_slice<TM>(pre, nbr, nbr_stride, K, row0 + chunk_rows);
+        if (chunk + 1 < n_chunks) sk::fetch_slice<TM>(pre, nbr, nbr_stride, k_fetch, row0 + chunk_rows);
         const int n_items = sk::build_items<TS, 32>(s_cnt, items, K, ts, wr);
 
         int k_r[DEPTH], row_r[DEPTH];
@@ -123,16 +128,16 @@
     }
 }
 
-template <int CIN, int DEPTH>
+template <int CIN, int DEPTH, bool PLAN>
 int launch_c32(const fd::SpconvCall &c) {
     const unsigned in_bytes = (unsigned)(c.n_in * CIN * 4);
     int n_ranges = c.n_ranges, rows_per = 0;
     if (!c.ranges) sk::equal_rows_split(c.n_out, TM, c.n_out_dev != nullptr, n_ranges, rows_per);
     static std::atomic<uint64_t> lds_set{0};
-    if (!fd::ensure_dynamic_lds(reinterpret_cast<const void *>(spconv_f32_c32<CIN, DEPTH>), (size_t)L.bytes, lds_set)) return 0;
+    if (!fd::ensure_dynamic_lds(reinterpret_cast<const void *>(spconv_f32_c32<CIN, DEPTH, PLAN>), (size_t)L.bytes, lds_set)) return 0;
     const void *wp = (const char *)c.wpacked + fd::spconv_weight_layout(c).c32.offset;
-    hipLaunchKernelGGL((spconv_f32_c32<CIN, DEPTH>), dim3((unsigned)n_ranges), dim3(256), (size_t)L.bytes, c.stream, (const float *)c.in, (const float4 *)wp,
-                       c.bias, (const float *)c.residual, c.relu, c.nbr, c.nbr_stride, c.K, c.n_out, c.n_out_dev, (float *)c.out, in_bytes, c.ranges, rows_per);
+    hipLaunchKernelGGL((spconv_f32_c32<CIN, DEPTH, PLAN>), dim3((unsigned)n_ranges), dim3(256), (size_t)L.bytes, c.stream, (const float *)c.in, (const float4 *)wp,
+                       c.bias, (const float *)c.residual, c.relu, PLAN ? c.plan : c.nbr, PLAN ? c.plan_stride : c.nbr_stride, c.K, c.n_out, c.n_out_dev, (float *)c.out, in_bytes, c.ranges, rows_per);
     return 1;
 }
 
@@ -142,6 +147,6 @@
 int spconv_f32_c32_dispatch(const SpconvCall &c) {
     if (c.cout != 32 || c.cin != 32) return 0;
     if (!sk::entries_fit(c.n_in, c.cin)) return 0;
-    return launch_c32<32, 3>(c);
+    return c.plan ? launch_c32<32, 3, true>(c) : launch_c32<32, 3, false>(c);
 }
 }
diff --git a/futuredet_amd/csrc/fd_spconv_chunk.h b/futuredet_amd/csrc/fd_spconv_chunk.h
--- a/futuredet_amd/csrc/fd_spconv_chunk.h
+++ b/futuredet_amd/csrc/fd_spconv_chunk.h
@@ -157,6 +157,34 @@
     if (tid < ITEM) s_pad[tid] = pad_entry(TM);
 }
 
+constexpr int kPlanRows = kMaxTaps + 1;
+constexpr int kPlanTM = 128;
+constexpr int kPlanCountWords = (kMaxTaps + 3) / 4;
+inline int64_t plan_stride_for(int64_t n_out) { return (n_out + 8 + 63) / 64 * 64; }
+
+template <int TM, int COUT, int TS, int ITEM>
+__device__ __forceinline__ void stage_plan_chunk(const int (&pre)[kSliceRegs<TM>], int *s_list, unsigned char *s_cnt, int *s_pad, float *s_acc,
+                                                 const float *bias, const float *residual, int row0, int n_rows) {
+    const int tid = threadIdx.x;
+    static_assert(TM == kPlanTM && 256 % TM == 0, "the plan is cut for 128-row chunks");
+    static_assert(kSliceRegs<TM> * 256 >= kMaxTaps * TM + kPlanCountWords, "the count words ride in the slice's last register");
+    const bool in_chunk = tid % TM < n_rows;
+#pragma unroll
+    for (int i = 0; i < kSliceRegs<TM>; ++i) {
+        const int t = tid + i * 256;
+        if (t < kMaxTaps * TM) {
+            s_list[t] = in_chunk ? pre[i] : pad_entry(TM);
+        } else if (t < kMaxTaps * TM + kPlanCountWords) {
+            const int k0 = (t - kMaxTaps * TM) * 4;
+#pragma unroll
+            for (int q = 0; q < 4; ++q)
+                if (k0 + q < kMaxTaps) s_cnt[(k0 + q) * 4] = (unsigned char)((unsigned)pre[i] >> (8 * q));
+        }
+    }
+    init_acc<TM, COUT, TS>(s_acc, bias, residual, row0, n_rows);
+    if (tid < ITEM) s_pad[tid] = pad_entry(TM);
+}
+
 template <int TM, int WR>
 __device__ __forceinline__ void compact_taps(int *s_list, unsigned char *s_cnt, int K) {
     const int lane = threadIdx.x & 63, wave = __builtin_amdgcn_readfirstlane(threadIdx.x >> 6);
diff --git a/futuredet_amd/csrc/fd_spconv_v2.hip b/futuredet_amd/csrc/fd_spconv_v2.hip
--- a/futuredet_amd/csrc/fd_spconv_v2.hip
+++ b/futuredet_amd/csrc/fd_spconv_v2.hip
@@ -25,7 +25,7 @@
 
 constexpr int tap_splits(int cout) { return (cout == 32 || cout == 64) ? 2 : 1; }
 
-template <int CIN, int COUT, int TM, int DEPTH>
+template <int CIN, int COUT, int TM, int DEPTH, bool PLAN>
 __global__ void __launch_bounds__(256) spconv_f32_compact(const float *__restrict__ in, const float4 *__restrict__ wp,
                                                           const float *__restrict__ bias, const float *__restrict__ residual, int relu,
                                                           const int *__restrict__ nbr, int64_t nbr_stride, int K, int n_out,
@@ -38,6 +38,7 @@
     constexpr int WR = 4 / (WC * TS);
     constexpr int NACC = NBW;
     static_assert((TM == 128 || TM == 64) && TM / WR >= 16, "local row uses 8 bits (0..TM, TM = scratch row)");
+    static_assert(!PLAN || (TM == sk::kPlanTM && WR == 1), "the chunk plan holds the lists of 128-row chunks with one row set");
     constexpr int kPad = sk::pad_entry(TM);
     constexpr sk::Layout L = sk::layout(TM, COUT, TS, 16);
     extern __shared__ __attribute__((aligned(16))) unsigned char smem[];
@@ -54,7 +55,8 @@
     FD_T(0);
     sk::cut_chunks<TM>(r_begin, r_end, n_chunks, chunk_rows);
     int pre[sk::kSliceRegs<TM>];
-    sk::fetch_slice<TM>(pre, nbr, nbr_stride, K, r_begin);
+    const int k_fetch = PLAN ? sk::kPlanRows : K;
+    sk::fetch_slice<TM>(pre, nbr, nbr_stride, k_fetch, r_begin);
 
     const int lrow = lane & 15, lq = lane >> 4;
     const int wc = wave % WC, wr = TS == 1 ? wave / WC : 0, ts = TS == 1 ? 0 : wave / WC;
@@ -67,13 +69,17 @@
     for (int chunk = 0; chunk < n_chunks; ++chunk) {
     int row0, n_rows;
     if (!sk::chunk_span(r_begin, r_end, chunk_rows, chunk, row0, n_rows)) break;
-    sk::stage_chunk<TM, COUT, TS, 16>(pre, s_list, s_pad, s_acc, bias, residual, K, row0, n_rows);
-    __syncthreads();
-    if (chunk == 0) FD_T(1);
-    sk::compact_taps<TM, WR>(s_list, s_cnt, K);
+    if constexpr (PLAN) {
+        sk::stage_plan_chunk<TM, COUT, TS, 16>(pre, s_list, s_cnt, s_pad, s_acc, bias, residual, row0, n_rows);
+    } else {
+        sk::stage_chunk<TM, COUT, TS, 16>(pre, s_list, s_pad, s_acc, bias, residual, K, row0, n_rows);
+        __syncthreads();
+        if (chunk == 0) FD_T(1);
+        sk::compact_taps<TM, WR>(s_list, s_cnt, K);
+    }
     __syncthreads();
     if (chunk == 0) FD_T(2);
-    if (chunk + 1 < n_chunks) sk::fetch_slice<TM>(pre, nbr, nbr_stride, K, row0 + chunk_rows);
+    if (chunk + 1 < n_chunks) sk::fetch_slice<TM>(pre, nbr, nbr_stride, k_fetch, row0 + chunk_rows);
     const int n_items = sk::build_items<TS, 16>(s_cnt, items, K, ts, wr);
 
     int k_r[DEPTH];
@@ -193,18 +199,22 @@
     return (cin == 64 && cout == 64 && tm == 128 && lds < 56 * 1024) ? (size_t)56 * 1024 : lds;
 }
 
-template <int CIN, int COUT, int TM, int DEPTH>
+template <int CIN, int COUT, int TM, int DEPTH, bool PLAN = false>
 int launch_compact(const fd::SpconvCall &c) {
+    if constexpr (!PLAN && CIN == COUT && COUT >= 32 && TM == sk::kPlanTM) {
+        if (c.plan) return launch_compact<CIN, COUT, TM, DEPTH, true>(c);
+    }
     const size_t lds_req = lds_request(CIN, COUT, TM);
     static std::atomic<uint64_t> lds_set{0};
-    auto kern = spconv_f32_compact<CIN, COUT, TM, DEPTH>;
+    auto kern = spconv_f32_compact<CIN, COUT, TM, DEPTH, PLAN>;
     if (!fd::ensure_dynamic_lds(reinterpret_cast<const void *>(kern), lds_req, lds_set)) return 0;
     const unsigned in_bytes = (unsigned)(c.n_in * CIN * 4);
     int n_ranges = c.n_ranges, rows_per = 0;
     if (!c.ranges) sk::equal_rows_split(c.n_out, TM, c.n_out_dev != nullptr, n_ranges, rows_per);
     const void *wp = (const char *)c.wpacked + fd::spconv_weight_layout(c).base.offset;
     hipLaunchKernelGGL(kern, dim3((unsigned)n_ranges), dim3(256), lds_req, c.stream, (const float *)c.in, (const float4 *)wp, c.bias,
-                       (const float *)c.residual, c.relu, c.nbr, c.nbr_stride, c.K, c.n_out, c.n_out_dev, (float *)c.out, in_bytes, c.ranges, rows_per);
+                       (const float *)c.residual, c.relu, PLAN ? c.plan : c.nbr, PLAN ? c.plan_stride : c.nbr_stride, c.K, c.n_out, c.n_out_dev,
+                       (float *)c.out, in_bytes, c.ranges, rows_per);
     return 1;
 }
 
@@ -333,6 +343,77 @@
     }
 }
 
+constexpr int kPlanSplit = 4;
+__global__ void __launch_bounds__(256) chunk_plan_kernel(const int *__restrict__ nbr, int64_t nbr_stride, int n_out, const int *__restrict__ n_out_dev,
+                                                         const int *__restrict__ ranges, int rows_per_range, int *__restrict__ plan, int64_t plan_stride) {
+    constexpr int TM = sk::kPlanTM, K = sk::kMaxTaps, NT = (K + 3) / 4, NH = TM / 64;
+    constexpr int kPad = sk::pad_entry(TM);
+    const int lane = threadIdx.x & 63, wave = __builtin_amdgcn_readfirstlane(threadIdx.x >> 6);
+    int r_begin, r_end, n_chunks, chunk_rows;
+    sk::resolve_range(n_out, n_out_dev, ranges, rows_per_range, r_begin, r_end);
+    if (r_begin < 0 || r_begin >= r_end) return;
+    sk::cut_chunks<TM>(r_begin, r_end, n_chunks, chunk_rows);
+    for (int chunk = blockIdx.y; chunk < n_chunks; chunk += kPlanSplit) {
+        int row0, n_rows;
+        if (!sk::chunk_span(r_begin, r_end, chunk_rows, chunk, row0, n_rows)) break;
+        int v[NT][NH];
+#pragma unroll
+        for (int j = 0; j < NT; ++j) {
+            const int k = wave + 4 * j < K ? wave + 4 * j : K - 1;
+#pragma unroll
+            for (int h = 0; h < NH; ++h) {
+                const int r = h * 64 + lane;
+                const int rr = r < n_rows ? r : n_rows - 1;
+                v[j][h] = nbr[(int64_t)k * nbr_stride + row0 + rr];
+                if (r >= n_rows) v[j][h] = -1;
+            }
+        }
+#pragma unroll
+        for (int j = 0; j < NT; ++j) {
+            const int k = wave + 4 * j;
+            if (k >= K) break;
+            int *list = plan + (int64_t)k * plan_stride + row0;
+            int count = 0;
+#pragma unroll
+            for (int h = 0; h < NH; ++h) {
+                const unsigned long long m = __ballot(v[j][h] >= 0);
+                const int pos = count + __popcll(m & ((1ull << lane) - 1ull));
+                if (v[j][h] >= 0) list[pos] = sk::pack_entry(v[j][h], h * 64 + lane);
+                count += __popcll(m);
+            }
+#pragma unroll
+            for (int h = 0; h < NH; ++h) {
+                const int p = h * 64 + lane;
+                if (p >= count && p < n_rows) list[p] = kPad;
+            }
+            if (lane == 0) reinterpret_cast<unsigned char *>(plan + (int64_t)K * plan_stride + row0)[k] = (unsigned char)count;
+        }
+    }
+}
+
+}
+
+extern "C" int64_t fd_spconv_plan_stride(int64_t n_out) { return n_out < 0 ? 0 : sk::plan_stride_for(n_out); }
+extern "C" size_t fd_spconv_plan_bytes(int64_t n_out) { return n_out < 0 ? 0 : sizeof(int32_t) * (size_t)sk::kPlanRows * (size_t)sk::plan_stride_for(n_out); }
+
+extern "C" int fd_spconv_plan_wanted(int cin, int cout, int dtype) {
+    if (dtype != 0 || cin != cout || fd::tuning(fd::kTuneSpconvV1) || fd::tuning(fd::kTuneSpconvPlan) < 0) return 0;
+    return cin == 32 || cin == 64 || cin == 128;
+}
+
+extern "C" int fd_spconv_plan_build(const int32_t *nbr, int64_t nbr_stride, int K, int64_t n_out, const int32_t *n_out_dev, const int32_t *ranges,
+                                    int n_ranges, int32_t *plan, int64_t plan_stride, fd_stream_t stream_) {
+    FD_REQUIRE(K == sk::kMaxTaps, "fd_spconv_plan_build: a chunk plan belongs to a SubM rulebook (K = 27)");
+    FD_REQUIRE(n_out >= 0 && n_out <= nbr_stride && n_out < (1ll << 31), "fd_spconv_plan_build: n_out out of range");
+    FD_REQUIRE(n_ranges >= 0 && (ranges == nullptr || n_ranges >= 1), "fd_spconv_plan_build: ranges needs n_ranges >= 1");
+    if (n_out == 0) return FD_OK;
+    FD_REQUIRE(nbr && plan, "fd_spconv_plan_build: null argument");
+    FD_REQUIRE(plan_stride >= sk::plan_stride_for(n_out), "fd_spconv_plan_build: plan_stride below fd_spconv_plan_stride(n_out)");
+    int rows_per = 0;
+    if (!ranges) sk::equal_rows_split((int)n_out, sk::kPlanTM, n_out_dev != nullptr, n_ranges, rows_per);
+    hipLaunchKernelGGL(chunk_plan_kernel, dim3((unsigned)n_ranges, kPlanSplit), dim3(256), 0, fd::as_stream(stream_), nbr, nbr_stride, (int)n_out,
+                       n_out_dev, ranges, rows_per, plan, plan_stride);
+    return fd::check_launch("fd_spconv_plan_build");
 }
 
 #ifdef FD_V2_TRACE
diff --git a/futuredet_amd/hip_ops.py b/futuredet_amd/hip_ops.py
--- a/futuredet_amd/hip_ops.py
+++ b/futuredet_amd/hip_ops.py
@@ -286,6 +286,33 @@
     return nbr.ranges
 
 
+def row_split(nbr, n_out, cin, cout, balanced=None):
+    L = _lib.load()
+    if balanced is None:
+        balanced = nbr.shape[0] == 27 and cin == cout and bool(L.fd_spconv_wants_balanced_ranges(cin, cout, 0))
+    if balanced == "tiles":
+        return None, 0
+    if balanced:
+        return ranges_for(nbr, cin, cout)
+    return None, int(L.fd_spconv_num_ranges(getattr(nbr, "n_expected", 0) or n_out, cin, cout, 0))
+
+
+def plan_for(nbr, n_out, ranges, n_ranges):
+    key = (ranges.data_ptr() if ranges is not None else 0, int(n_ranges), int(n_out))
+    plans = getattr(nbr, "plans", None)
+    if plans is None:
+        plans = nbr.plans = {}
+    if key not in plans:
+        L = _lib.load()
+        K, nstride = nbr.shape
+        pstride = int(L.fd_spconv_plan_stride(n_out))
+        plan = torch.empty((28, pstride), dtype=torch.int32, device=nbr.device)
+        check(L.fd_spconv_plan_build(_p(nbr), nstride, K, n_out, _p(getattr(nbr, "n_dev", None)), _p(ranges), int(n_ranges), _p(plan), pstride,
+                                     _stream()), "fd_spconv_plan_build")
+        plans[key] = (plan, pstride, ranges)
+    return plans[key][:2]
+
+
 def rows_permute(src, row_of, c_dst, dtype=torch.float32, n_rows=None, n_dev=None):
     L = _lib.load()
     src = _dev(src, "src", torch.float32)
@@ -406,7 +433,7 @@
     return feats
 
 
-def spconv_apply(feats, wpacked, bias, nbr, n_out, cout, residual=None, relu=False, out=None, balanced=None):
+def spconv_apply(feats, wpacked, bias, nbr, n_out, cout, residual=None, relu=False, out=None, balanced=None, plan=None):
     L = _lib.load()
     feats = _dev(feats, "feats")
     dt = _DT[feats.dtype]
@@ -417,17 +444,17 @@
         out = torch.empty((max(n_out, 1), out_cols), dtype=out_dtype, device=feats.device)[:n_out]
     if residual is not None:
         _dev(residual, "residual", out_dtype)
-    ranges, n_ranges = None, 0
     n_dev, n_expected = getattr(nbr, "n_dev", None), getattr(nbr, "n_expected", 0)
-    if dt == 0 and n_out > 0:
-        if balanced is None:
-            balanced = K == 27 and cin == cout and bool(L.fd_spconv_wants_balanced_ranges(cin, cout, 0))
-        if balanced == "tiles":
-            n_ranges = 0
-        elif balanced:
-            ranges, n_ranges = ranges_for(nbr, cin, cout)
-        else:
-            n_ranges = int(L.fd_spconv_num_ranges(n_expected or n_out, cin, cout, 0))
+    ranges, n_ranges = row_split(nbr, n_out, cin, cout, balanced) if dt == 0 and n_out > 0 else (None, 0)
+    if plan is None:
+        plan = dt == 0 and n_out > 0 and K == 27 and cin == cout and bool(L.fd_spconv_plan_wanted(cin, cout, 0))
+    if plan:
+        plan_t, pstride = plan_for(_dev(nbr, "nbr", torch.int32), n_out, ranges, n_ranges)
+        check(L.fd_spconv_apply_plan(_p(feats), feats.shape[0], _p(_dev(wpacked, "wpacked")), _p(bias), _p(residual), int(bool(relu)),
+                                     _p(nbr), nstride, _p(ranges), n_ranges, K, n_out, _p(n_dev), int(n_expected or 0),
+                                     cin, cout, dt, _p(out), _p(plan_t), pstride, _stream()),
+              "fd_spconv_apply_plan")
+        return out
     check(L.fd_spconv_apply(_p(feats), feats.shape[0], _p(_dev(wpacked, "wpacked")), _p(bias), _p(residual), int(bool(relu)),
                             _p(_dev(nbr, "nbr", torch.int32)), nstride, _p(ranges), n_ranges, K, n_out, _p(n_dev), int(n_expected or 0),
                             cin, cout, dt, _p(out), _stream()),
diff --git a/futuredet_amd/lib.py b/futuredet_amd/lib.py
--- a/futuredet_amd/lib.py
+++ b/futuredet_amd/lib.py
@@ -100,6 +100,12 @@
     "fd_spconv_wants_balanced_ranges": (c_int, [c_int, c_int, c_int]),
     "fd_spconv_ranges_workspace_bytes": (c_size_t, [c_i64]),
     "fd_spconv_ranges": (c_int, [c_void_p, c_i64, c_int, c_i64, c_void_p, c_int, c_void_p, c_void_p, c_size_t, c_void_p]),
+    "fd_spconv_plan_stride": (c_i64, [c_i64]),
+    "fd_spconv_plan_bytes": (c_size_t, [c_i64]),
+    "fd_spconv_plan_wanted": (c_int, [c_int, c_int, c_int]),
+    "fd_spconv_plan_build": (c_int, [c_void_p, c_i64, c_int, c_i64, c_void_p, c_void_p, c_int, c_void_p, c_i64, c_void_p]),
+    "fd_spconv_apply_plan": (c_int, [c_void_p, c_i64, c_void_p, c_void_p, c_void_p, c_int, c_void_p, c_i64, c_void_p, c_int, c_int, c_i64,
+                                     c_void_p, c_i64, c_int, c_int, c_int, c_void_p, c_void_p, c_i64, c_void_p]),
     "fd_densify": (c_int, [c_void_p, c_int, c_int, c_void_p, c_void_p, c_int, c_int, c_int, c_int, c_void_p, c_int, c_i64,
                            c_i64, c_i64, c_i64, c_i64, c_void_p]),
     "fd_conv2d_packed_weight_bytes": (c_size_t, [c_int, c_int, c_int]),
diff --git a/futuredet_amd/sparse.py b/futuredet_amd/sparse.py
--- a/futuredet_amd/sparse.py
+++ b/futuredet_amd/sparse.py
@@ -121,7 +121,7 @@
     @staticmethod
     def forward(ctx, feats, weight, bias, nbr, n_out, subm):
         wpk = hip_ops.pack_spconv_weight_device(weight, hip_ops.PACK_PLAIN, feats.dtype)
-        out = hip_ops.spconv_apply(feats, wpk, bias, nbr, n_out, weight.shape[2])
+        out = hip_ops.spconv_apply(feats, wpk, bias, nbr, n_out, weight.shape[2], plan=False)
         ctx.save_for_backward(feats, weight)
         ctx.nbr, ctx.n_out, ctx.subm, ctx.has_bias = nbr, n_out, subm, bias is not None
         return out
@@ -137,7 +137,7 @@
         if ctx.needs_input_grad[0]:
             if ctx.subm:
                 wt = hip_ops.pack_spconv_weight_device(weight, hip_ops.PACK_FLIPPED_TRANSPOSED, dt)
-                dx = hip_ops.spconv_apply(dy, wt, None, nbr, n_in, cin_p)
+                dx = hip_ops.spconv_apply(dy, wt, None, nbr, n_in, cin_p, plan=False)
             else:
                 inv = getattr(nbr, "inv", None)
                 if inv is None:
@@ -145,7 +145,7 @@
                     if getattr(nbr, "n_in_dev", None) is not None:
                         inv.n_dev, inv.n_expected = nbr.n_in_dev, nbr.n_in_expected
                 wt = hip_ops.pack_spconv_weight_device(weight, hip_ops.PACK_TRANSPOSED, dt)
-                dx = hip_ops.spconv_apply(dy, wt, None, inv, n_in, cin_p)
+                dx = hip_ops.spconv_apply(dy, wt, None, inv, n_in, cin_p, plan=False)
         if ctx.needs_input_grad[1]:
             dw = hip_ops.spconv_wgrad(feats, dy, nbr, n_out)
         if ctx.has_bias and ctx.needs_input_grad[2]:
diff --git a/include/futuredet_hip.h b/include/futuredet_hip.h
--- a/include/futuredet_hip.h
+++ b/include/futuredet_hip.h
@@ -57,6 +57,15 @@
 size_t fd_spconv_ranges_workspace_bytes(int64_t n_out);
 int fd_spconv_ranges(const int32_t *nbr, int64_t nbr_stride, int K, int64_t n_out, const int32_t *n_out_dev, int n_ranges,
                      int32_t *ranges , void *workspace, size_t workspace_bytes, fd_stream_t stream);
+int64_t fd_spconv_plan_stride(int64_t n_out);
+size_t fd_spconv_plan_bytes(int64_t n_out);
+int fd_spconv_plan_wanted(int cin, int cout, int dtype);
+int fd_spconv_plan_build(const int32_t *nbr, int64_t nbr_stride, int K, int64_t n_out, const int32_t *n_out_dev, const int32_t *ranges,
+                         int n_ranges, int32_t *plan, int64_t plan_stride, fd_stream_t stream);
+int fd_spconv_apply_plan(const void *in_feats, int64_t n_in, const void *wpacked, const float *bias, const void *residual, int relu,
+                         const int32_t *nbr, int64_t nbr_stride, const int32_t *ranges, int n_ranges, int K, int64_t n_out,
+                         const int32_t *n_out_dev, int64_t n_expected, int cin, int cout, int dtype, void *out_feats, const int32_t *plan,
+                         int64_t plan_stride, fd_stream_t stream);
 
 int fd_densify(const void *feats, int c, int dtype, const uint64_t *words, const int32_t *prefix, int B, int D,
                int H, int W, void *out, int out_dtype, int64_t stride_b, int64_t stride_c, int64_t stride_y,
```

Result: faster. 285.2 (median of 6 runs) (+1.1%).
